# andrei-ace/EdgeStyle

Measured on AMD Instinct MI355X. Metric: 512x512 try-on images/sec @ 50 DDIM steps (6-cond ControlNet), higher is better.
Workload: dtype f16; 1 GPU; BASELINE configs[1]: full 6-cond edgestyle_multicontrolnet + controllora, 512x512, 50 DDIM steps, CFG 7.5, batch=1/GPU, hipGraph-captured step, cond embedding + VAE decode included; images_per_gpu=1, ddim_steps=50, parallelism=dp1 (independent images, one RCCL gather)

## Files before the change

### edgestyle_amd/csrc/builder.hip

```cpp
#include <hip/hip_runtime.h>
#include <math.h>
#include <stdio.h>
#include <stdlib.h>
#include <string.h>

#include <algorithm>
#include <deque>
#include <functional>
#include <map>
#include <memory>
#include <stdexcept>
#include <string>
#include <thread>
#include <unordered_map>
#include <vector>

#include "../../include/edgestyle_hip.h"
#include "plan.h"

extern "C" void es_set_error(const char* msg);
extern "C" int es_plan_set_dry(int on);

namespace {

[[noreturn]] void fail(const std::string& m) { throw std::runtime_error(m); }
inline int cdiv(long long a, long long b) { return (int)((a + b - 1) / b); }
inline int round_up(int a, int b) { return (a + b - 1) / b * b; }
constexpr int BK = 64, BM = 128;
constexpr unsigned long long FAKE_HEAP = 1ull << 44, FAKE_WS = 1ull << 45;

void parallel_for(long long n, const std::function<void(long long, long long)>& fn) {
  unsigned nt = std::thread::hardware_concurrency();
  nt = nt < 1 ? 1 : (nt > 16 ? 16 : nt);
  if (n < 64 || nt == 1) { fn(0, n); return; }
  std::vector<std::thread> th;
  const long long step = (n + nt - 1) / nt;
  for (long long a = 0; a < n; a += step) th.emplace_back(fn, a, std::min(n, a + step));
  for (auto& t : th) t.join();
}

inline uint16_t f32_to_f16(float f) { _Float16 h = (_Float16)f; uint16_t u; memcpy(&u, &h, 2); return u; }
inline float f16_to_f32(uint16_t u) { _Float16 h; memcpy(&h, &u, 2); return (float)h; }
inline uint16_t f32_to_bf16(float f) {
  uint32_t u; memcpy(&u, &f, 4);
  if ((u & 0x7FFFFFFFu) > 0x7F800000u) return (uint16_t)((u >> 16) | 0x40);
  return (uint16_t)((u + 0x7FFFu + ((u >> 16) & 1u)) >> 16);
}
inline float bf16_to_f32(uint16_t h) { uint32_t u = (uint32_t)h << 16; float f; memcpy(&f, &u, 4); return f; }

struct Dict {
  std::unordered_map<std::string, const es_tensor*> m;
  std::string name;
  void init(const es_state_dict& sd, const char* nm) {
    name = nm;
    if (sd.count < 0 || (sd.count > 0 && !sd.tensors)) fail(std::string("es_load_weights: the ") + nm + " state dict has a count but no tensors");
    for (int i = 0; i < sd.count; ++i) {
      const es_tensor& t = sd.tensors[i];
      if (!t.key || !t.data || t.ndim < 1 || t.ndim > 4 || t.dtype < 0 || t.dtype > ES_F32) fail("es_load_weights: malformed tensor descriptor #" + std::to_string(i) + " in the " + name + " state dict");
      long long n = 1;
      for (int d = 0; d < t.ndim; ++d) { if (t.shape[d] < 1 || t.shape[d] > (1ll << 31)) n = -1; else if (n > 0) n *= t.shape[d]; if (n > (1ll << 33)) n = -1; }
      if (n < 0) fail(std::string("es_load_weights: implausible shape of '") + t.key + "' in the " + name + " state dict");
      m[t.key] = &t;
    }
  }
  const es_tensor* find(const std::string& k) const { auto it = m.find(k); return it == m.end() ? nullptr : it->second; }
};
long long numel(const es_tensor* t) { long long n = 1; for (int i = 0; i < t->ndim; ++i) n *= t->shape[i]; return n; }
bool on_device(const void* p) {
  hipPointerAttribute_t a;
  const bool dev = hipPointerGetAttributes(&a, p) == hipSuccess && a.type == hipMemoryTypeDevice;
  (void)hipGetLastError();
  return dev;
}
std::vector<float> to_f32(const es_tensor* t) {
// ... 125 lines not shown
  ~Blk() { if (heap) heap->release(off, bytes); }
};

struct T {
  unsigned long long p = 0;
  int n = 0, h = 0, w = 0, c = 0;
  long long ld = 0;
  int es = 2;
  std::shared_ptr<Blk> b;
  unsigned long long lo = 0;
  std::shared_ptr<Blk> lo_b;
  unsigned long long gnp = 0;
  std::shared_ptr<Blk> gnp_b;
  int gnp_groups = 0;
  explicit operator bool() const { return p != 0; }
  long long hw() const { return (long long)h * w; }
  long long numel() const { return (long long)n * h * w * c; }
  bool contig() const { return ld == c; }
  long long bstride() const { return hw() * ld; }
  size_t bytes() const { return (size_t)numel() * es; }
  T batch(int a, int cnt = -1) const {
    T t = *this;
    t.p += (unsigned long long)a * (unsigned long long)bstride() * es;
    if (t.lo) t.lo += (unsigned long long)a * (unsigned long long)bstride() * es;
    t.gnp = 0; t.gnp_b.reset(); t.gnp_groups = 0;
    t.n = cnt < 0 ? n - a : cnt;
    if (a < 0 || t.n < 0 || a + t.n > n) fail("builder: batch slice out of range");
    return t;
  }
  T chan(int c0, int cn) const {
    T t = *this;
    if (c0 < 0 || c0 + cn > c) fail("builder: channel slice out of range");
    t.p += (unsigned long long)c0 * es;
    t.lo = 0; t.lo_b.reset();
    t.gnp = 0; t.gnp_b.reset(); t.gnp_groups = 0;
    t.c = cn;
    return t;
  }
  T view(int n2, int h2, int w2, int c2) const {
    if (!contig() || (long long)n2 * h2 * w2 * c2 != numel()) fail("builder: view of a non-contiguous or differently sized tensor");
    T t = *this;
    t.n = n2; t.h = h2; t.w = w2; t.c = c2; t.ld = c2;
    return t;
  }
  void* ptr() const { return (void*)p; }
};

struct PW {
  unsigned long long w = 0, bias = 0, ln_colsum = 0;
  int cout = 0, cin = 0, ksize = 1, bn = 128, rows_padded = 0, kpad = 0, ctail = 0, korder = 0;
  bool geglu = false;
  float ln_eps = 1e-5f;
  const uint16_t* host_w = nullptr;
  long long w_numel() const { return (long long)rows_padded * kpad; }
};
using PWs = std::vector<const PW*>;
struct Norm { unsigned long long g = 0, b = 0; };

struct CA {
  int stride = 1, pad = -1;
  bool upsample = false;
  T x2, temb, residual, out, out_scale_dev;
  long long temb_stride = 0;
  int act = ES_ACT_NONE;
  float out_scale = 1.f;
  int out_h = 0, out_w = 0;
  std::vector<int> group_n;
  std::vector<T> tails;
  int x_rep = 1;
  bool wide = false;
  int gn_groups = 0;
};

#pragma clang fp contract(off)
constexpr double PLAN_T160 = 1.25, PLAN_ALONE = 0.9, PLAN_TFIX = 2.0, PLAN_RED_FIX = 12.0, PLAN_SLAB_BYTES_PER_UNIT = 4.0e6;
constexpr double PLAN_T320 = 2.3, PLAN_T320_FIX = 3.0;
constexpr double PLAN_T256 = 2.6, PLAN_T256_FIX = 6.0, PLAN_T256_GEGLU = 7.0, PLAN_LN_TK = 1.55, PLAN_T256_MARGIN = 0.93;
constexpr int PLAN_BIG_MIN_M = 2048, PLAN_BIG_MIN_NK = 16;
constexpr double PLAN_T64_ALONE = 0.5, PLAN_T64 = 0.16, PLAN_T64_LONG = 1.5;
constexpr int PLAN_SMALL_MAX_M = 16384, PLAN_MIN_SLICE = 12, PLAN_NK_NOSPLIT = 10, PLAN_RESIDENT = 512;

double plan_env(const char* name, double dflt) { const char* e = getenv(name); return e && *e ? atof(e) : dflt; }
bool plan_gemm(long long M, int rows_padded, int kpad, bool geglu, const int* bns, int nb, bool allow_split, int* o_bn, int* o_sk, int* o_st) {
  static const double PLAN_T320 = plan_env("ES_PLAN_T320", ::PLAN_T320), PLAN_T256_MARGIN = plan_env("ES_PLAN_T256_MARGIN", ::PLAN_T256_MARGIN);
  static const int PLAN_BIG_MIN_NK = (int)plan_env("ES_PLAN_BIG_MIN_NK", ::PLAN_BIG_MIN_NK);
  int others[8], no = 0;
  bool has256 = false;
  for (int bi = 0; bi < nb; ++bi) { if (bns[bi] == 256) has256 = true; else if (no < 8) others[no++] = bns[bi]; }
  if (has256) {
    const int nk = kpad / BK;
    int obn = 0, osk = 1, ost = 2;
    const bool have_other = no > 0 && plan_gemm(M, rows_padded, kpad, geglu, others, no, allow_split, &obn, &osk, &ost);
    if (rows_padded % 256) { if (!have_other) return false; *o_bn = obn; *o_sk = osk; *o_st = ost; return true; }
    const long long t256 = ((M + 255) / 256) * (rows_padded / 256);
    const double c256 = (double)((t256 + 255) / 256) * ((double)nk * PLAN_T256 + PLAN_T256_FIX + (geglu ? PLAN_T256_GEGLU : 0.0));
    bool take = !have_other;
    if (have_other && M >= PLAN_BIG_MIN_M && nk >= PLAN_BIG_MIN_NK && osk == 1 && obn != 64) {
      const long long to = ((M + BM - 1) / BM) * (rows_padded / obn);
      const double co = (double)((to + PLAN_RESIDENT - 1) / PLAN_RESIDENT) * ((double)nk * PLAN_LN_TK * (obn == 160 ? PLAN_T160 : 1.0) + PLAN_T256_FIX);
      take = c256 < PLAN_T256_MARGIN * co;
    }
    if (take) { *o_bn = 256; *o_sk = 1; *o_st = 2; } else { *o_bn = obn; *o_sk = osk; *o_st = ost; }
    return true;
  }
  if (geglu) { *o_bn = 128; *o_sk = 1; *o_st = 2; return true; }
  const int nk = kpad / BK;
// ... 16 lines not shown
      else if (bn == 64) {
        if (sk > 1 && wgs > PLAN_RESIDENT) continue;
        const double w = (double)wgs / (double)(PLAN_RESIDENT / 2);
        const double ex = std::max(0.0, w - 1.0);
        tk = (PLAN_T64_ALONE + PLAN_T64 * (ex * ex)) * (nk <= 40 ? 1.0 : PLAN_T64_LONG);
      } else tk = (bn == 160 ? PLAN_T160 : 1.0) * (wgs <= PLAN_RESIDENT / 2 ? PLAN_ALONE : 1.0);
      const double rounds = bn == 320 ? std::max((double)wgs / 256.0, 0.9) : (double)((wgs + resident - 1) / resident);
      double t = rounds * (((double)nk / (double)sk) * tk + (bn == 320 ? PLAN_T320_FIX : PLAN_TFIX));
      if (sk > 1) t += PLAN_RED_FIX + (double)sk * (double)M * (double)rows_padded * 8.0 / PLAN_SLAB_BYTES_PER_UNIT;
      if (!have || t < bt) { have = true; bt = t; bbn = bn; bsk = sk; bwgs = wgs; }
    }
  }
  if (!have) return false;
  *o_bn = bbn; *o_sk = bsk;
  if (bbn == 64) *o_st = (bwgs <= PLAN_RESIDENT && nk / bsk >= 6) ? 4 : 2;
  else *o_st = (bbn != 320 && bwgs <= PLAN_RESIDENT / 2 && nk / bsk >= 6) ? 4 : 2;
  return true;
}

constexpr int XS_TARGET_WGS = 256, XS_MIN_M = 8192;
bool xs_shape_fits(int ksize, int kpad, int cin, int ctail, int cout, bool geglu) {
  if (ksize != 1 || (kpad != 320 && kpad != 640) || cin != kpad || ctail) return false;
  const int ch = kpad == 320 ? 64 : 32;
  const int line = ch * (128 / (geglu ? ch : 2 * ch));
  return !(cout % line || cout < 4 * line);
}
bool xs_shape_ok(long long M, int ksize, int kpad, int cin, int ctail, int cout, bool geglu, long long min_m) {
  if (!xs_shape_fits(ksize, kpad, cin, ctail, cout, geglu)) return false;
  if (min_m && (M < min_m || (M < 4 * min_m && cout < (kpad == 320 ? 960 : 1920)))) return false;
  return true;
}
int choose_bn(int cout) { return (cout % 160 == 0 && cout % 128 != 0) ? 160 : 128; }

bool wide_stream(int dtype, const es_launch_knobs& k) { return k.wide_stream == 1 || (k.wide_stream < 0 && dtype == ES_BF16); }
bool gn_handover(long long hw, int c, int groups, const es_launch_knobs& k) {
  if (!k.gn_handover || groups < 1 || c % 8 || hw % 64 || c % groups || c / groups > 64) return false;
  return k.gn_handover == 2 || !es_group_norm_is_slab((int)hw, c, groups);
}
bool groups_tile_256(const es_launch_query& q) {
  for (int g = 0; g < std::min(q.n_counts, 4); ++g) if ((q.group_n[g] * q.hw) % 256) return false;
  return true;
}
bool launch_takes_xs(const es_launch_query& q, const es_launch_knobs& k) {
  const bool xs_res = !q.has_residual || (k.xs_residual && q.kpad == 320 && !q.geglu && !q.has_ln && q.residual_dense && !(q.wide && wide_stream(q.dtype, k)));
  if (!(q.ksize == 1 && q.stride == 1 && !q.upsample && !q.C2 && !q.has_temb && xs_res && !q.n_tails && q.x_rep == 1 && q.act == ES_ACT_NONE &&
        q.unit_scale && !q.force_splitk && !k.force_bn && k.xs_enabled)) return false;
  if (q.ngroups > 1 && (q.ngroups > 4 || !groups_tile_256(q) || !q.groups_agree)) return false;
  return xs_shape_ok(q.M, q.ksize, q.kpad, q.cin, q.ctail, q.cout, q.geglu != 0, k.xs_min_m);
}
bool launch_choose(const es_launch_query& q, const es_launch_knobs& k, es_launch_choice* o) {
  memset(o, 0, sizeof(*o));
  if (launch_takes_xs(q, k)) { o->route = ES_ROUTE_LINEAR_XS; return true; }
  const bool aligned = q.C1 % BK == 0 && q.C2 % BK == 0;
  const bool big_ok = k.big_tile && aligned && !q.geglu && !q.has_ln && groups_tile_256(q);
  const bool small_ok = k.small_tile && aligned && !q.geglu && k.force_waves != 8;
  const bool ln256_ok = k.big_tile_256 && (q.geglu || q.has_ln) && q.ksize == 1 && q.stride == 1 && !q.upsample && !q.C2 && !q.n_tails && !q.has_temb &&
                        q.x_rep == 1 && q.C1 % BK == 0 && q.rows_padded % 256 == 0 && q.cout % 8 == 0 && !(q.geglu && q.has_residual) && !q.wide &&
                        q.gn_groups == 0 && k.force_waves != 8 && groups_tile_256(q);
  int cand[5], nc = 0;
  if (ln256_ok) cand[nc++] = 256;
  if (big_ok) cand[nc++] = 320;
  cand[nc++] = 160; cand[nc++] = 128;
  if (small_ok) cand[nc++] = 64;
  if (k.force_bn) { cand[0] = k.force_bn; nc = 1; }
  const bool geglu = q.geglu != 0, allow_split = !q.has_ln;
  int bn, splitk, stages;
  if (!plan_gemm(q.M, q.rows_padded, q.kpad, geglu, cand, nc, allow_split, &bn, &splitk, &stages)) return false;
  if (bn == 320 && !k.force_bn && (q.force_splitk ? q.force_splitk : splitk) == 1 &&
      !es_conv_gemm8p_form_ok(geglu ? ES_ACT_GEGLU : q.act, q.cout, q.has_temb, q.hw, q.has_residual)) {
    const int at = (int)(std::find(cand, cand + nc, 320) - cand);
    std::copy(cand + at + 1, cand + nc, cand + at);
    if (!plan_gemm(q.M, q.rows_padded, q.kpad, geglu, cand, nc - 1, allow_split, &bn, &splitk, &stages)) return false;
  }
  if (stages == 4 && !k.deep_ring) stages = 2;
  if (q.force_splitk) { splitk = q.force_splitk; stages = q.stages; }
  else if (q.stages) stages = q.stages;
  if (!stages) stages = k.force_stages;
  o->bn = bn; o->splitk = splitk; o->stages = stages;
  if (k.force_waves) o->waves = k.force_waves;
  else if (k.eight_waves && q.ksize == 1 && q.M <= 65536 && aligned && bn != 64 && bn != 320 && bn != 256 && !(stages == 4 && bn != 128) && stages != 3) o->waves = 8;
  o->xcd_m_fastest = k.xcd_order < 0 ? (q.ngroups <= 1 && splitk == 1 && q.M <= 2048 && q.w_numel > q.src_numel) : k.xcd_order;
  const int cstore = geglu ? q.cout / 2 : q.cout;
  o->gn_partials = q.gn_groups > 0 && gn_handover(q.hw, cstore, q.gn_groups, k) && !geglu && !q.has_ln && q.cout / q.gn_groups <= (bn == 320 ? 160 : bn);
  o->wide = q.wide && q.has_residual && wide_stream(q.dtype, k) && cstore % 8 == 0 && !geglu;
  return true;
}
bool launch_gn_fold(const es_launch_query& q, int groups, const es_launch_knobs& k) {
  if (!(k.gn_fold && k.xs_enabled) || k.gn_handover || q.hw % 256 || groups < 1 || groups > 32) return false;
  if (q.geglu || q.has_ln || q.kpad % groups || !xs_shape_fits(q.ksize, q.kpad, q.cin, q.ctail, q.cout, false)) return false;
  if (q.M < (q.kpad == 320 ? 8192 : 32768)) return false;
  return !(q.ngroups > 1 && (q.ngroups > 4 || !groups_tile_256(q) || !q.groups_agree));
}
struct BuildEnv { es_launch_knobs knobs; bool chunk_major; };
BuildEnv read_build_env() {
  auto env = [](const char* name, const char* dflt) { const char* e = getenv(name); return std::string(e ? e : dflt); };
  const std::string ho = env("ES_GN_HANDOVER", "0"), ws = env("ES_WIDE_STREAM", "auto");
  BuildEnv b;
  b.chunk_major = env("ES_CHUNK_MAJOR", "0") == "1";
  es_launch_knobs& k = b.knobs;
  memset(&k, 0, sizeof(k));
  k.xs_enabled = k.big_tile = k.small_tile = k.eight_waves = k.deep_ring = 1; k.xs_min_m = XS_MIN_M; k.xcd_order = -1;
  k.xs_residual = env("ES_XS_RESIDUAL", "1") == "1"; k.big_tile_256 = env("ES_BIG_TILE_256", "1")[0] != '0'; k.gn_fold = env("ES_GN_FOLD", "1") == "1";
  k.gn_handover = ho == "all" ? 2 : ho == "1"; k.wide_stream = ws == "auto" ? -1 : ws == "1";
  return b;
}

struct Builder {
  Heap heap;
  unsigned long long ws_bytes = 0;
  int dt = ES_F16;
  const BuildEnv env = read_build_env();
  std::vector<std::pair<unsigned long long, std::vector<char>>> uploads;
  std::deque<PW> pws;
  std::map<std::string, const PW*> pack_cache;
  std::map<const void*, unsigned long long> vec_cache;
  std::map<std::pair<int, int>, unsigned long long> gn_partials, fusion_scratch;
  std::map<int, unsigned long long> zero_bias;

  T empty(int n, int h, int w, int c, int es = 2) {
    T t; t.n = n; t.h = h; t.w = w; t.c = c; t.ld = c; t.es = es;
    auto blk = std::make_shared<Blk>();
    blk->heap = &heap; blk->bytes = std::max<size_t>(t.bytes(), 1); blk->off = heap.alloc(blk->bytes);
    t.b = blk; t.p = FAKE_HEAP + blk->off;
    return t;
  }
  unsigned long long persistent(size_t bytes) { return FAKE_HEAP + heap.alloc(std::max<size_t>(bytes, 1)); }
  T persistent_t(int n, int h, int w, int c, int es = 2) {
    T t; t.n = n; t.h = h; t.w = w; t.c = c; t.ld = c; t.es = es;
    t.p = persistent(t.bytes());
    return t;
  }
  char* staged(unsigned long long addr, size_t bytes) {
    uploads.emplace_back(addr, std::vector<char>(bytes, 0));
    return uploads.back().second.data();
  }
  unsigned long long upload_f32(const std::vector<float>& v) {
    const unsigned long long a = persistent(v.size() * 4);
    memcpy(staged(a, v.size() * 4), v.data(), v.size() * 4);
    return a;
  }
  unsigned long long workspace(unsigned long long bytes) { ws_bytes = std::max(ws_bytes, bytes); return FAKE_WS; }
  void add_into(const T& a, const T& b, const T& out) {
    if (!a.contig() || !b.contig() || !out.contig() || a.numel() != b.numel() || a.numel() != out.numel()) fail("builder: add of non-contiguous or differently sized tensors");
    ok(es_add(a.ptr(), b.ptr(), out.ptr(), a.numel(), dt, nullptr), "es_add");
  }
  T add(const T& a, const T& b) {
    if (!a.contig() || !b.contig() || a.numel() != b.numel()) fail("builder: add of non-contiguous or differently sized tensors");
    T out = empty(a.n, a.h, a.w, a.c);
    ok(es_add(a.ptr(), b.ptr(), out.ptr(), a.numel(), dt, nullptr), "es_add");
    return out;
  }
  uint16_t enc(float f) const { return dt == ES_F16 ? f32_to_f16(f) : f32_to_bf16(f); }
  float dec(uint16_t u) const { return dt == ES_F16 ? f16_to_f32(u) : bf16_to_f32(u); }

  const PW* pack(const std::vector<float>& w, int cout, int cin, int k, const std::vector<float>* bias, bool geglu = false, int cin_pad = 0, int cout_pad = 0,
                 const std::vector<float>* tail = nullptr, int ctail = 0) {
    if ((long long)w.size() != (long long)cout * cin * k * k) fail("builder: weight size does not match its shape");
    const int cp = cin_pad ? cin_pad : round_up(cin, 8);
    if (cp < cin || cp % 8 || (cout_pad && cout_pad < cout)) fail("builder: channel padding smaller than the tensor");
    const int ktrue = k * k * cp + ctail;
    const int cout_eff = cout_pad ? cout_pad : cout;
    const int bn = geglu ? 128 : choose_bn(cout_eff);
    const int rows = round_up(cout_eff, bn);
    const int kpad = round_up(ktrue, BK);
    const int inner = cout / 2;
    if (geglu && inner % 16) fail("builder: GEGLU inner width must be a multiple of 16");
    pws.emplace_back();
    PW& p = pws.back();
    p.cout = cout_eff; p.cin = cp; p.ksize = k; p.bn = bn; p.rows_padded = rows; p.kpad = kpad; p.geglu = geglu; p.ctail = ctail;
    const bool chunk_major = env.chunk_major && k == 3 && cp % BK == 0;
    p.korder = chunk_major ? 1 : 0;
    p.w = persistent((size_t)rows * kpad * 2);
    uint16_t* dst = (uint16_t*)staged(p.w, (size_t)rows * kpad * 2);
    p.host_w = dst;
    auto src_row = [&](int r) { if (!geglu) return r; const int blk = r / 32, within = r % 32; return within < 16 ? blk * 16 + within : inner + blk * 16 + (within - 16); };
    parallel_for(cout, [&](long long a, long long b) {
      for (long long r = a; r < b; ++r) {
        const float* s = w.data() + (size_t)src_row((int)r) * cin * k * k;
        uint16_t* d = dst + (size_t)r * kpad;
        for (int t = 0; t < k * k; ++t)
          for (int ci = 0; ci < cin; ++ci)
            d[chunk_major ? ((ci / BK) * k * k + t) * BK + ci % BK : t * cp + ci] = enc(s[(size_t)ci * k * k + t]);
        if (tail) for (int j = 0; j < ctail; ++j) d[k * k * cp + j] = enc((*tail)[(size_t)r * ctail + j]);
      }
    });
    if (bias) {
      if ((int)bias->size() != cout) fail("builder: bias size does not match the weight");
      p.bias = persistent((size_t)rows * 4);
      float* bd = (float*)staged(p.bias, (size_t)rows * 4);
      for (int r = 0; r < cout; ++r) bd[r] = (*bias)[src_row(r)];
    }
    return &p;
  }
  const PW* pack_ln(const std::vector<float>& w, int rows, int C, const std::vector<float>* bias, const std::vector<float>& gamma, const std::vector<float>& beta,
                    float eps, bool geglu) {
    std::vector<float> wg((size_t)rows * C), fb((size_t)rows);
    parallel_for(rows, [&](long long a, long long b) {
      for (long long r = a; r < b; ++r) {
        double acc = 0.0;
        for (int j = 0; j < C; ++j) { wg[r * C + j] = w[r * C + j] * gamma[j]; acc += (double)w[r * C + j] * (double)beta[j]; }
        if (bias) acc += (double)(*bias)[r];
        fb[r] = (float)acc;
      }
    });
    PW* p = const_cast<PW*>(pack(wg, rows, C, 1, &fb, geglu));
    const uint16_t* pk = p->host_w;
    std::vector<float> cs((size_t)p->rows_padded);
    for (int r = 0; r < p->rows_padded; ++r) {
      double acc = 0.0;
      for (int j = 0; j < p->kpad; ++j) acc += (double)dec(pk[(size_t)r * p->kpad + j]);
      cs[r] = (float)acc;
    }
    p->ln_colsum = upload_f32(cs);
    p->ln_eps = eps;
    return p;
  }
  unsigned long long norm_vec(const Weights& W, const std::string& key, long long n) {
    const es_tensor* id = nullptr;
    std::vector<float> v = W.vec(key, n, &id);
    auto it = vec_cache.find(id->data);
    if (it != vec_cache.end()) return it->second;
    return vec_cache[id->data] = upload_f32(v);
  }
  Norm norm(const Weights& W, const std::string& p, long long n) { return {norm_vec(W, p + ".weight", n), norm_vec(W, p + ".bias", n)}; }

  const PW* conv(const Weights& W, const std::string& p, int cin_pad = 0, bool geglu = false, int cout_pad = 0) {
    const es_tensor* wt = W.get(p + ".weight");
    if (wt->ndim != 2 && wt->ndim != 4) fail("es_load_weights: '" + p + ".weight' is neither a Linear nor a Conv2d weight");
    const int cout = (int)wt->shape[0], cin = (int)wt->shape[1], k = wt->ndim == 4 ? (int)wt->shape[2] : 1;
    if (wt->ndim == 4 && (wt->shape[3] != k || (k != 1 && k != 3))) fail("es_load_weights: '" + p + ".weight': only 1x1 and 3x3 kernels");
    const es_tensor* bt = W.find(p + ".bias");
    std::string key;
    if (!W.lora(p)) {
      char buf[128];
      snprintf(buf, sizeof(buf), "%p|%p|%d|%d|%d", wt->data, bt ? bt->data : nullptr, (int)geglu, cin_pad, cout_pad);
      key = buf;
      auto it = pack_cache.find(key);
      if (it != pack_cache.end()) return it->second;
    }
    std::vector<float> w = W.matrix(p), b;
    if (bt) b = W.vec(p + ".bias", cout);
    const PW* pw = pack(w, cout, cin, k, bt ? &b : nullptr, geglu, cin_pad, cout_pad);
    if (!key.empty()) pack_cache[key] = pw;
    return pw;
  }
  void stack(const Weights& W, const std::vector<std::string>& ps, bool bias, std::vector<float>& w, std::vector<float>& b, int& rows, int& cols) {
    rows = 0; cols = -1;
    for (const auto& p : ps) {
      const es_tensor* t = W.get(p + ".weight");
      if (t->ndim != 2 || (cols >= 0 && t->shape[1] != cols)) fail("es_load_weights: '" + p + ".weight' does not stack with its neighbours");
      cols = (int)t->shape[1];
      std::vector<float> m = W.matrix(p);
      w.insert(w.end(), m.begin(), m.end());
      if (bias) { std::vector<float> v = W.vec(p + ".bias", t->shape[0]); b.insert(b.end(), v.begin(), v.end()); }
      rows += (int)t->shape[0];
    }
  }
  const PW* cat(const Weights& W, const std::vector<std::string>& ps, bool bias) {
    std::vector<float> w, b; int rows, cols;
    stack(W, ps, bias, w, b, rows, cols);
    return pack(w, rows, cols, 1, bias ? &b : nullptr);
  }
  const PW* cat_ln(const Weights& W, const std::vector<std::string>& ps, bool bias, const std::string& ln, bool geglu = false) {
    std::vector<float> w, b; int rows, cols;
    stack(W, ps, bias, w, b, rows, cols);
    return pack_ln(w, rows, cols, bias ? &b : nullptr, W.vec(ln + ".weight", cols), W.vec(ln + ".bias", cols), 1e-5f, geglu);
  }
  const PW* conv_tail(const Weights& W, const std::string& p, const std::string& pt) {
    const es_tensor* wt = W.get(p + ".weight");
    const es_tensor* tt = W.get(pt + ".weight");
    char buf[96];
    snprintf(buf, sizeof(buf), "%p|%p|tail", wt->data, tt->data);
    auto it = pack_cache.find(buf);
    if (it != pack_cache.end()) return it->second;
    const int cout = (int)wt->shape[0], cin = (int)wt->shape[1], k = (int)wt->shape[2], ct = (int)tt->shape[1];
    if (wt->ndim != 4 || cin % BK || ct % BK || tt->shape[0] != cout) fail("es_load_weights: conv2 + conv_shortcut fold needs 64-aligned channels ('" + p + "')");
    std::vector<float> w = W.matrix(p), tw = W.matrix(pt), b = W.vec(p + ".bias", cout), b2 = W.vec(pt + ".bias", cout);
    for (int i = 0; i < cout; ++i) b[i] = b[i] + b2[i];
    const PW* pw = pack(w, cout, cin, k, &b, false, 0, 0, &tw, ct);
    pack_cache[buf] = pw;
    return pw;
  }

  static void ok(int rc, const char* what) { if (rc) fail(std::string(what) + ": " + es_last_error()); }

  struct GnFront { unsigned long long part = 0; std::vector<Norm> nl; int groups = 0, nchunk = 0, hw = 0; float eps = 0.f; };
  T linear_xs(const T& x, const PWs& pl, long long M, const T& out, const std::vector<long long>& group_rows, const T& residual = T(),
              const GnFront* gn = nullptr) {
    const PW* pw = pl[0];
    const int K = pw->kpad, ch = K == 320 ? 64 : 32;
    const int pline = 128 / (pw->geglu ? ch : 2 * ch);
    const int total = pw->cout / ch, lines = total / pline;
    const long long rbs = (M + 255) / 256;
    const int want = (int)std::max<long long>(1, std::min<long long>(lines, XS_TARGET_WGS / rbs));
    const int lps = cdiv(lines, want), nslices = cdiv(lines, lps);
    es_xs_desc d;
    memset(&d, 0, sizeof(d));
    auto bias_of = [&](const PW* q) -> unsigned long long {
      if (q->bias) return q->bias;
      auto it = zero_bias.find(q->rows_padded);
      if (it != zero_bias.end()) return it->second;
      return zero_bias[q->rows_padded] = persistent((size_t)q->rows_padded * 4);
    };
    d.x = x.ptr(); d.out = out.ptr(); d.w = (const void*)pw->w; d.bias = (const float*)bias_of(pw);
    d.M = (int)M; d.K = K; d.Cout = pw->cout; d.rows_padded = pw->rows_padded; d.ldo = out.c;
    d.geglu = pw->geglu; d.ln = pw->ln_colsum != 0; d.ln_eps = pw->ln_eps;
    d.nslices = nslices; d.chunks_per_slice = lps * pline; d.dtype = dt;
    if (residual) d.residual = residual.ptr();
    if (gn) {
      d.gn_part = (const float*)gn->part; d.gn_groups = gn->groups; d.gn_nchunk = gn->nchunk; d.gn_hw = gn->hw; d.gn_eps = gn->eps;
      if (pl.size() > 1) {
        if (gn->nl.size() != pl.size()) fail("grouped linear_xs: one GroupNorm parameter set per weight group");
        for (size_t g = 0; g < pl.size(); ++g) { d.gn_gamma_g[g] = (const float*)gn->nl[g].g; d.gn_beta_g[g] = (const float*)gn->nl[g].b; }
      } else { d.gn_gamma = (const float*)gn->nl[0].g; d.gn_beta = (const float*)gn->nl[0].b; }
    }
    if (pl.size() > 1) {
      d.ngroups = (int)pl.size();
      long long acc = 0;
      for (size_t g = 0; g < pl.size(); ++g) {
        const PW* q = pl[g];
        if (q->rows_padded != pw->rows_padded || q->kpad != pw->kpad || q->cout != pw->cout || q->geglu != pw->geglu) fail("grouped linear_xs: weight geometry differs between groups");
        acc += group_rows[g] / 128;
        d.mt_end[g] = (int)acc; d.w_g[g] = (const void*)q->w; d.bias_g[g] = (const float*)bias_of(q);
      }
    }
    ok(es_linear_xs(&d, nullptr), "es_linear_xs");
    return out;
  }

  es_launch_query launch_query(const PWs& pl, long long M, long long hw, const CA& a, int C1, int C2, long long src_numel, bool residual_dense) const {
    const PW* pw = pl[0];
    es_launch_query q;
    memset(&q, 0, sizeof(q));
    q.M = M; q.hw = hw; q.w_numel = pw->w_numel(); q.src_numel = src_numel; q.ksize = pw->ksize; q.stride = a.stride; q.upsample = a.upsample; q.C1 = C1; q.C2 = C2;
    q.rows_padded = pw->rows_padded; q.kpad = pw->kpad; q.cin = pw->cin; q.ctail = pw->ctail; q.cout = pw->cout; q.geglu = pw->geglu; q.has_ln = pw->ln_colsum != 0;
    q.act = a.act; q.has_temb = (bool)a.temb; q.has_residual = (bool)a.residual; q.residual_dense = residual_dense; q.unit_scale = a.out_scale == 1.f && !a.out_scale_dev;
    q.n_tails = (int)a.tails.size(); q.x_rep = a.x_rep; q.wide = a.wide; q.dtype = dt; q.gn_groups = a.gn_groups;
    if (pl.size() > 1) {
      q.ngroups = (int)pl.size(); q.n_counts = (int)a.group_n.size(); q.groups_agree = 1;
      for (size_t g = 0; g < std::min<size_t>(a.group_n.size(), 4); ++g) q.group_n[g] = a.group_n[g];
      for (const PW* p : pl) if ((p->ln_colsum == 0) != (pw->ln_colsum == 0)) q.groups_agree = 0;
    }
    return q;
  }

  T conv_gemm(const T& x, const PWs& pl, const CA& a = CA()) {
    const PW* pw = pl[0];
    const bool grouped = pl.size() > 1;
    int N = x.n;
    const int H = x.h, Wd = x.w, C1 = x.c, nsrc = x.n;
    if (!x.contig()) fail("conv_gemm: the source must be contiguous");
    if (a.x_rep > 1) { if (a.x2 || !a.tails.empty()) fail("conv_gemm: x_rep needs a single source"); N *= a.x_rep; }
    const int C2 = a.x2 ? a.x2.c : 0;
    if (C1 + C2 != pw->cin) fail("conv_gemm: input channels " + std::to_string(C1) + "+" + std::to_string(C2) + " != packed " + std::to_string(pw->cin));
    int tsum = 0;
    for (const auto& t : a.tails) tsum += t.c;
    if (tsum != pw->ctail || a.tails.size() > 2) fail("conv_gemm: tail channels do not match the packed weights");
    const int k = pw->ksize, pad = a.pad < 0 ? (k == 3 ? 1 : 0) : a.pad;
    const int Hin = a.upsample ? H * 2 : H, Win = a.upsample ? Wd * 2 : Wd;
    const int Hout = a.out_h ? a.out_h : (Hin + 2 * pad - k) / a.stride + 1, Wout = a.out_w ? a.out_w : (Win + 2 * pad - k) / a.stride + 1;
    const int act_i = pw->geglu ? ES_ACT_GEGLU : a.act;
    const int cstore = pw->geglu ? pw->cout / 2 : pw->cout;
    T out = a.out ? a.out : empty(N, Hout, Wout, cstore);
    if (out.numel() != (long long)N * Hout * Wout * cstore || !out.contig()) fail("conv_gemm: output buffer of another size");
    const long long M = (long long)N * Hout * Wout, hw = (long long)Hout * Wout;
    const es_launch_query q = launch_query(pl, M, hw, a, C1, C2, x.numel() * a.x_rep + (a.x2 ? a.x2.numel() : 0),
                                           a.residual && a.residual.contig() && a.residual.numel() == M * cstore);
    es_launch_choice ch;
    if (!launch_choose(q, env.knobs, &ch)) fail("plan_gemm: rows_padded fits no N tile");
    if (ch.route == ES_ROUTE_LINEAR_XS) {
      std::vector<long long> rows;
      for (int n : a.group_n) rows.push_back(n * hw);
      T xo = out;
      linear_xs(x, grouped ? pl : PWs{pw}, M, xo, rows, a.residual);
      return out;
    }
    const int bn = ch.bn, splitk = ch.splitk;
    es_gemm_desc d;
    memset(&d, 0, sizeof(d));
    d.x = x.ptr(); d.x2 = a.x2 ? a.x2.ptr() : nullptr; d.w = (const void*)pw->w; d.bias = (const float*)pw->bias;
    d.temb = a.temb ? a.temb.ptr() : nullptr; d.residual = a.residual ? a.residual.ptr() : nullptr;
    d.out_scale_dev = a.out_scale_dev ? (const float*)a.out_scale_dev.ptr() : nullptr; d.out = out.ptr();
    d.N = N; d.Hsrc = H; d.Wsrc = Wd; d.C1 = C1; d.C2 = C2; d.Hout = Hout; d.Wout = Wout; d.Cout = pw->cout;
    d.rows_padded = pw->rows_padded; d.Kpad = pw->kpad; d.ksize = k; d.stride = a.stride; d.pad = pad; d.upsample = a.upsample;
    d.temb_stride = a.temb ? (int)a.temb_stride : 0;
    d.act = act_i; d.splitk = splitk; d.bn = bn; d.dtype = dt; d.out_scale = a.out_scale; d.stages = ch.stages;
    d.waves = ch.waves; d.xcd_m_fastest = ch.xcd_m_fastest;
    d.x_nmod = a.x_rep > 1 ? nsrc : 0;
    d.korder = pw->korder;
    if (ch.gn_partials) {
      T part = empty(N, (int)(2 * (hw / 64)), 1, a.gn_groups * 2, 4);
      d.gn_part = (float*)part.ptr(); d.gn_groups = a.gn_groups;
      out.gnp = part.p; out.gnp_b = part.b; out.gnp_groups = a.gn_groups;
    }
    if (ch.wide) {
      if (a.residual.lo) d.residual_lo = (const void*)a.residual.lo;
      T lo = empty(N, Hout, Wout, cstore);
      d.out_lo = lo.ptr();
      out.lo = lo.p; out.lo_b = lo.b;
    }
    if (splitk > 1) d.workspace = (float*)workspace((unsigned long long)splitk * M * pw->rows_padded * 4);
    if (pw->ln_colsum) {
      for (const PW* q : pl) if (!q->ln_colsum) fail("LayerNorm-folded weights need a plain linear launch (all groups folded)");
      if (a.x2 || k != 1) fail("LayerNorm-folded weights need a plain linear launch");
      d.ln_colsum = (const float*)pw->ln_colsum; d.ln_eps = pw->ln_eps;
    }
    if (!a.tails.empty()) {
      for (const auto& t : a.tails) if (t.n != N || t.h != Hout || t.w != Wout || !t.contig()) fail("conv_gemm: tail sources must be contiguous [N,Hout,Wout,C]");
      d.t1 = a.tails[0].ptr(); d.Ct1 = a.tails[0].c;
      if (a.tails.size() == 2) { d.t2 = a.tails[1].ptr(); d.Ct2 = a.tails[1].c; }
    }
    if (grouped) {
      const int gran = bn == 320 ? 256 : BM;
      int sum = 0;
      for (int n : a.group_n) { sum += n; if ((n * hw) % gran) fail("grouped conv_gemm: groups must cover N in whole tiles"); }
      if (pl.size() > 4 || a.group_n.size() != pl.size() || sum != N) fail("grouped conv_gemm: bad group table");
      d.ngroups = (int)pl.size();
      long long acc = 0;
      for (size_t g = 0; g < pl.size(); ++g) {
        const PW* q = pl[g];
// ... 215 lines not shown
    conv_in = B.conv(W, "conv_in", in_pad);
    t1 = B.conv(W, "time_embedding.linear_1"); t2 = B.conv(W, "time_embedding.linear_2");
    std::vector<std::string> names;
    for (int i = 0; i < c.nb; ++i) for (int j = 0; j < c.lpb; ++j) names.push_back("down_blocks." + std::to_string(i) + ".resnets." + std::to_string(j));
    names.push_back("mid_block.resnets.0"); names.push_back("mid_block.resnets.1");
    names.insert(names.end(), extra_resnets.begin(), extra_resnets.end());
    int o = 0;
    std::vector<std::string> tp;
    for (const auto& nm : names) { temb_offs[nm] = o; o += (int)W.shaped(nm + ".time_emb_proj.weight", {-1, 4 * c.ch[0]})->shape[0]; tp.push_back(nm + ".time_emb_proj"); }
    tproj = B.cat(W, tp, true);
    for (int i = 0; i < c.nb; ++i) {
      down.emplace_back();
      for (int j = 0; j < c.lpb; ++j) {
        const std::string r = "down_blocks." + std::to_string(i) + ".resnets." + std::to_string(j);
        int ti = -1;
        Resnet rs(B, W, r, c.groups, c.eps, temb_offs[r]);
        if (c.has_attn[i]) { tr.emplace_back(B, W, "down_blocks." + std::to_string(i) + ".attentions." + std::to_string(j), c.heads, c.groups); ti = (int)tr.size() - 1; }
        down.back().emplace_back(rs, ti);
      }
      downsample.push_back(i != c.nb - 1 ? B.conv(W, "down_blocks." + std::to_string(i) + ".downsamplers.0.conv") : nullptr);
    }
    mid0 = Resnet(B, W, "mid_block.resnets.0", c.groups, c.eps, temb_offs["mid_block.resnets.0"]);
    tr.emplace_back(B, W, "mid_block.attentions.0", c.heads, c.groups); mid_attn = (int)tr.size() - 1;
    mid1 = Resnet(B, W, "mid_block.resnets.1", c.groups, c.eps, temb_offs["mid_block.resnets.1"]);
    n_enc_tr = (int)tr.size();
  }
  int tproj_width() const { return tproj->cout; }
  T time_proj(Builder& B, const T& t, int n) const {
    T e = B.timestep_embedding(t, n, cfg.ch[0]);
    CA s; s.act = ES_ACT_SILU;
    e = B.linear(e, t1, s);
    e = B.linear(e, t2, s);
    return B.linear(e, tproj);
  }
};

struct UNet : Encoder {
  std::vector<std::vector<std::pair<Resnet, int>>> up;
  std::vector<const PW*> upsample;
  Norm norm_out; const PW* conv_out;
  void init(Builder& B, const Weights& W, const UCfg& c) {
    std::vector<std::string> extra;
    for (int i = 0; i < c.nb; ++i) for (int j = 0; j < c.lpb + 1; ++j) extra.push_back("up_blocks." + std::to_string(i) + ".resnets." + std::to_string(j));
    Encoder::init(B, W, c, extra);
    for (int i = 0; i < c.nb; ++i) {
      up.emplace_back();
      for (int j = 0; j < c.lpb + 1; ++j) {
        const std::string r = "up_blocks." + std::to_string(i) + ".resnets." + std::to_string(j);
        int ti = -1;
        Resnet rs(B, W, r, c.groups, c.eps, temb_offs[r]);
        if (c.has_attn[c.nb - 1 - i]) { tr.emplace_back(B, W, "up_blocks." + std::to_string(i) + ".attentions." + std::to_string(j), c.heads, c.groups); ti = (int)tr.size() - 1; }
        up.back().emplace_back(rs, ti);
      }
      upsample.push_back(i != c.nb - 1 ? B.conv(W, "up_blocks." + std::to_string(i) + ".upsamplers.0.conv") : nullptr);
    }
    W.shaped("conv_out.weight", {c.out_ch, c.ch[0], 3, 3});
    norm_out = B.norm(W, "conv_norm_out", c.ch[0]);
    conv_out = B.conv(W, "conv_out");
  }
};

struct ControlNet : Encoder {
  std::vector<const PW*> zero; const PW* zero_mid = nullptr;
  std::vector<const PW*> cond;
  bool uses_vae = false;
  void init(Builder& B, const Weights& W, const UCfg& c, bool uses_vae_) {
    Encoder::init(B, W, c, {});
    uses_vae = uses_vae_;
    std::vector<int> rc{c.ch[0]};
    for (int i = 0; i < c.nb; ++i) { for (int j = 0; j < c.lpb; ++j) rc.push_back(c.ch[i]); if (i != c.nb - 1) rc.push_back(c.ch[i]); }
    for (size_t i = 0; i < rc.size(); ++i) {
      W.shaped("controlnet_down_blocks." + std::to_string(i) + ".weight", {rc[i], rc[i], 1, 1});
      zero.push_back(B.conv(W, "controlnet_down_blocks." + std::to_string(i)));
    }
    W.shaped("controlnet_mid_block.weight", {c.ch[c.nb - 1], c.ch[c.nb - 1], 1, 1});
    zero_mid = B.conv(W, "controlnet_mid_block");
    if (!uses_vae) {
      const std::string p = "controlnet_cond_embedding";
      W.shaped(p + ".conv_in.weight", {c.ce[0], c.cond_ch, 3, 3});
      W.shaped(p + ".conv_out.weight", {c.ch[0], c.ce[c.nce - 1], 3, 3});
      cond.push_back(B.conv(W, p + ".conv_in", 8));
      for (int i = 0; i < 2 * (c.nce - 1); ++i) cond.push_back(B.conv(W, p + ".blocks." + std::to_string(i)));
      cond.push_back(B.conv(W, p + ".conv_out"));
    }
  }
  T embed_cond(Builder& B, const T& img) const {
    CA s; s.act = ES_ACT_SILU;
    T h = B.conv_gemm(img, cond[0], s);
    for (size_t i = 1; i + 1 < cond.size(); ++i) { CA a; a.act = ES_ACT_SILU; a.stride = ((i - 1) % 2 == 1) ? 2 : 1; h = B.conv_gemm(h, cond[i], a); }
    return B.conv_gemm(h, cond.back());
  }
};

struct FusionParams { unsigned long long w1, b1, g1, be1, w2, b2, g2, be2, w3, b3; int c, s; };

struct VAE {
  VCfg cfg; int lat_pad = 8;
  struct Mid { Resnet r0, r1; Norm gn; const PW *qkv, *o; };
  const PW *e_in, *e_out, *quant, *post_quant_scaled, *d_in, *d_out;
  std::vector<std::pair<std::vector<Resnet>, const PW*>> e_down, d_up;
  Mid e_mid, d_mid; Norm e_norm, d_norm;
  Mid mid(Builder& B, const Weights& W, const std::string& side) {
    const std::string a = side + ".mid_block.attentions.0";
    const int c = cfg.ch[cfg.nb - 1];
    Mid m;
    m.r0 = Resnet(B, W, side + ".mid_block.resnets.0", cfg.groups, cfg.eps, -1);
    m.gn = B.norm(W, a + ".group_norm", c);
    m.qkv = B.cat(W, {a + ".to_q", a + ".to_k", a + ".to_v"}, true);
    m.o = B.conv(W, a + ".to_out.0");
    m.r1 = Resnet(B, W, side + ".mid_block.resnets.1", cfg.groups, cfg.eps, -1);
    return m;
  }
  void init(Builder& B, const Weights& W, const VCfg& c) {
    cfg = c;
    lat_pad = round_up(c.latent, 8);
    const int n = c.nb;
    W.shaped("encoder.conv_in.weight", {c.ch[0], 3, 3, 3}); W.shaped("encoder.conv_out.weight", {2 * c.latent, c.ch[n - 1], 3, 3});
    W.shaped("quant_conv.weight", {2 * c.latent, 2 * c.latent, 1, 1}); W.shaped("post_quant_conv.weight", {c.latent, c.latent, 1, 1});
    W.shaped("decoder.conv_in.weight", {c.ch[n - 1], c.latent, 3, 3}); W.shaped("decoder.conv_out.weight", {3, c.ch[0], 3, 3});
    for (const char* side : {"encoder", "decoder"})
      for (const char* q : {".to_q", ".to_k", ".to_v", ".to_out.0"}) W.shaped(std::string(side) + ".mid_block.attentions.0" + q + ".weight", {c.ch[n - 1], c.ch[n - 1]});
    e_in = B.conv(W, "encoder.conv_in", 8);
    for (int i = 0; i < n; ++i) {
      std::vector<Resnet> rs;
      for (int j = 0; j < c.lpb; ++j) rs.emplace_back(B, W, "encoder.down_blocks." + std::to_string(i) + ".resnets." + std::to_string(j), c.groups, c.eps, -1);
      e_down.emplace_back(rs, i != n - 1 ? B.conv(W, "encoder.down_blocks." + std::to_string(i) + ".downsamplers.0.conv") : nullptr);
    }
    e_mid = mid(B, W, "encoder");
    e_norm = B.norm(W, "encoder.conv_norm_out", c.ch[n - 1]);
    e_out = B.conv(W, "encoder.conv_out");
    quant = B.conv(W, "quant_conv");
    {
      const es_tensor* wt = W.get("post_quant_conv.weight");
      std::vector<float> w = W.matrix("post_quant_conv"), b;
      for (auto& v : w) v = (float)((double)v / (double)c.scaling);
      const bool hb = W.has("post_quant_conv.bias");
      if (hb) b = W.vec("post_quant_conv.bias", wt->shape[0]);
      post_quant_scaled = B.pack(w, (int)wt->shape[0], (int)wt->shape[1], 1, hb ? &b : nullptr, false, lat_pad, 8);
    }
    d_in = B.conv(W, "decoder.conv_in", 8);
    d_mid = mid(B, W, "decoder");
    for (int i = 0; i < n; ++i) {
      std::vector<Resnet> rs;
      for (int j = 0; j < c.lpb + 1; ++j) rs.emplace_back(B, W, "decoder.up_blocks." + std::to_string(i) + ".resnets." + std::to_string(j), c.groups, c.eps, -1);
      d_up.emplace_back(rs, i != n - 1 ? B.conv(W, "decoder.up_blocks." + std::to_string(i) + ".upsamplers.0.conv") : nullptr);
    }
    d_norm = B.norm(W, "decoder.conv_norm_out", c.ch[0]);
    d_out = B.conv(W, "decoder.conv_out");
  }
  T run_mid(Builder& B, const Mid& m, T h) const {
    h = m.r0.run(B, h, T());
    const int N = h.n, H = h.h, Wd = h.w, C = h.c;
    T n = B.group_norm(h, m.gn, cfg.groups, cfg.eps, false).view(N, H * Wd, 1, C);
    T qkv = B.linear(n, m.qkv);
    T a = B.attention(qkv.chan(0, C), qkv.chan(C, C), qkv.chan(2 * C, C), 1);
    CA r; r.residual = h.view(N, H * Wd, 1, C);
    h = B.linear(a, m.o, r).view(N, H, Wd, C);
    return m.r1.run(B, h, T());
  }
  T encode_moments(Builder& B, const T& img) const {
    T h = B.conv_gemm(img, e_in);
    for (const auto& blk : e_down) {
      for (const auto& r : blk.first) h = r.run(B, h, T());
      if (blk.second) { CA a; a.stride = 2; a.pad = 0; a.out_h = h.h / 2; a.out_w = h.w / 2; h = B.conv_gemm(h, blk.second, a); }
    }
    h = run_mid(B, e_mid, h);
    h = B.group_norm(h, e_norm, cfg.groups, cfg.eps, true);
    h = B.conv_gemm(h, e_out);
    return B.conv_gemm(h, quant);
  }
  T decode(Builder& B, const T& z) const {
    T h = B.conv_gemm(z, post_quant_scaled);
    h = B.conv_gemm(h, d_in);
    h = run_mid(B, d_mid, h);
    for (const auto& blk : d_up) {
      for (const auto& r : blk.first) h = r.run(B, h, T());
      if (blk.second) { CA a; a.upsample = true; h = B.conv_gemm(h, blk.second, a); }
    }
    h = B.group_norm(h, d_norm, cfg.groups, cfg.eps, true);
    return B.conv_gemm(h, d_out);
  }
};

struct Model {
  Builder B;
  UCfg ucfg; VCfg vcfg;
  es_ctx_geometry geo;
  Dict d_unet, d_vae, d_fusion, d_cn[6];
  UNet unet;
  VAE vae;
  std::vector<std::unique_ptr<ControlNet>> nets;
  std::vector<int> net_of_cond;
  std::vector<std::pair<int, std::vector<int>>> groups;
  std::vector<FusionParams> fusion;
  std::vector<std::pair<int, int>> table;
  std::vector<const Encoder*> encs; std::vector<int> counts; int ntot = 0, width = 0, ncn = 0;
  int B_ = 1, N = 2, T_ = 50, h = 64, w = 64, nn = 6, kmax = 3;
  T latents, model_in, noise, ehs, step_idx, t_rows, scales_cur, t_table, scale_table, coef, ts_dev, image;
// ... 340 lines not shown
  void pack_fusion(const Weights& W) {
    for (size_t i = 0; i < table.size(); ++i) {
      const std::string p = i + 1 < table.size() ? "multi_controlnet_down_blocks." + std::to_string(i) : "multi_controlnet_mid_block";
      const int c = table[i].first, s = table[i].second, hw = s * s;
      FusionParams f; f.c = c; f.s = s;
      f.w1 = B.upload_f32(to_f32(W.shaped(p + ".first_conv.weight", {3 * c, 2, 1, 1})));
      f.b1 = B.upload_f32(to_f32(W.shaped(p + ".first_conv.bias", {3 * c})));
      f.w2 = B.upload_f32(to_f32(W.shaped(p + ".second_conv.weight", {c, 3, 1, 1})));
      f.b2 = B.upload_f32(to_f32(W.shaped(p + ".second_conv.bias", {c})));
      f.w3 = B.upload_f32(to_f32(W.shaped(p + ".third_conv.weight", {c, 1, 1, 1})));
      f.b3 = B.upload_f32(to_f32(W.shaped(p + ".third_conv.bias", {c})));
      auto plane = [&](const std::string& key, int per) {
        const std::vector<float> t = to_f32(W.shaped(key, {(long long)per * c, s, s}));
        const unsigned long long a = B.persistent((size_t)hw * c * per * 2);
        uint16_t* d = (uint16_t*)B.staged(a, (size_t)hw * c * per * 2);
        parallel_for(hw, [&](long long x0, long long x1) {
          for (long long px = x0; px < x1; ++px)
            for (int cc = 0; cc < c * per; ++cc) d[(size_t)px * c * per + cc] = B.enc(t[(size_t)cc * hw + px]);
        });
        return a;
      };
      f.g1 = plane(p + ".first_normalization.weight", 3); f.be1 = plane(p + ".first_normalization.bias", 3);
      f.g2 = plane(p + ".second_normalization.weight", 1); f.be2 = plane(p + ".second_normalization.bias", 1);
      fusion.push_back(f);
    }
  }
};

struct Recording {
  es_plan* p;
  explicit Recording(es_plan* pl) : p(pl) { if (es_plan_begin_record(p)) fail(std::string("es_load_weights: ") + es_last_error()); es_plan_set_dry(1); }
  ~Recording() { es_plan_set_dry(0); es_plan_end_record(p); }
};

}

extern "C" int es_plan_gemm_choice(long long M, int rows_padded, int kpad, int geglu, const int* bns, int n_bns, int allow_split, int* bn, int* splitk, int* stages) {
  if (!bns || n_bns < 1 || !bn || !splitk || !stages) { es_set_error("es_plan_gemm_choice: null argument"); return -1; }
  if (!plan_gemm(M, rows_padded, kpad, geglu != 0, bns, n_bns, allow_split != 0, bn, splitk, stages)) { es_set_error("es_plan_gemm_choice: rows_padded fits no N tile"); return -1; }
  return 0;
}
extern "C" int es_linear_xs_eligible(long long M, int ksize, int kpad, int cin, int ctail, int cout, int geglu) {
  return xs_shape_ok(M, ksize, kpad, cin, ctail, cout, geglu != 0, XS_MIN_M) ? 1 : 0;
}
extern "C" int es_launch_choose(const es_launch_query* q, const es_launch_knobs* k, es_launch_choice* out) {
  if (!q || !k || !out) { es_set_error("es_launch_choose: null argument"); return -1; }
  if (!launch_choose(*q, *k, out)) { es_set_error("es_launch_choose: rows_padded fits no N tile"); return -1; }
  return 0;
}
extern "C" int es_launch_route(const es_launch_query* q, const es_launch_knobs* k) { return q && k && launch_takes_xs(*q, *k) ? ES_ROUTE_LINEAR_XS : ES_ROUTE_CONV_GEMM; }
extern "C" int es_launch_gn_fold(const es_launch_query* q, int groups, const es_launch_knobs* k) { return q && k && launch_gn_fold(*q, groups, *k); }
extern "C" int es_launch_gn_handover(long long hw, int c, int groups, const es_launch_knobs* k) { return k && gn_handover(hw, c, groups, *k); }
extern "C" int es_launch_wide_stream(int dtype, const es_launch_knobs* k) { return k && wide_stream(dtype, *k); }

extern "C" int es_load_weights(const es_weights* wts, const es_model_config* mc, const es_ctx_geometry* g, int device, es_ctx** out) {
  if (!wts || !mc || !g || !out) { es_set_error("es_load_weights: null argument"); return -1; }
  es_ctx* ctx = nullptr;
  es_plan* plans[ES_PLAN_COUNT] = {};
  void* arena = nullptr;
  try {
    auto m = std::make_unique<Model>();
    Model& M = *m;
    Builder& B = M.B;
    if (mc->n_blocks < 2 || mc->n_blocks > 4 || mc->vae_n_blocks < 2 || mc->vae_n_blocks > 4) fail("es_load_weights: 2..4 resolution levels");
    if (g->n_conds != 6 && g->n_conds != 1) fail("es_load_weights: n_conds is 6 (the reference's fused multi-ControlNet model, MC:66-114) or 1 (a single ControlNet, PL:338-351)");
    if (g->n_conds == 1 && wts->n_controlnets != 1) fail("es_load_weights: a single-ControlNet context takes exactly one ControlNet");
    if (g->dtype != ES_F16 && g->dtype != ES_BF16) fail("es_load_weights: dtype must be ES_F16 or ES_BF16");
    if (g->B < 1 || g->h < 1 || g->w < 1 || g->n_steps < 1) fail("es_load_weights: bad geometry");
    if (wts->n_controlnets < 1 || wts->n_controlnets > 6) fail("es_load_weights: 1..6 distinct ControlNets");
    UCfg& u = M.ucfg;
    u.in_ch = mc->in_channels; u.out_ch = mc->out_channels; u.nb = mc->n_blocks; u.lpb = mc->layers_per_block; u.heads = mc->num_heads;
    u.cross = mc->cross_attention_dim; u.groups = mc->norm_num_groups; u.eps = mc->norm_eps; u.nce = mc->n_cond_embed; u.cond_ch = mc->conditioning_channels;
    for (int i = 0; i < 4; ++i) { u.ch[i] = mc->block_out_channels[i]; u.has_attn[i] = mc->down_has_attn[i]; u.ce[i] = mc->cond_embed_channels[i]; }
    VCfg& v = M.vcfg;
    v.nb = mc->vae_n_blocks; v.lpb = mc->vae_layers_per_block; v.latent = mc->vae_latent_channels; v.groups = mc->vae_norm_num_groups;
    v.eps = mc->vae_norm_eps; v.scaling = mc->vae_scaling_factor;
    for (int i = 0; i < 4; ++i) v.ch[i] = mc->vae_block_out_channels[i];
    if (u.in_ch != v.latent) fail("es_load_weights: the UNet's in_channels must equal the VAE's latent_channels");
    if (u.cond_ch != 3 || u.nce < 2 || u.nce > 4) fail("es_load_weights: conditioning embedding of 3 input channels, 2..4 widths");
    M.geo = *g;
    B.dt = g->dtype;
    M.B_ = g->B; M.N = g->cfg ? 2 * g->B : g->B; M.T_ = g->n_steps; M.h = g->h; M.w = g->w; M.nn = g->n_conds;
    M.guess = g->guess_mode != 0;
    M.Bc = M.guess ? g->B : M.N;
    const int N = M.N, TS = M.T_, h = g->h, w = g->w, Bn = g->B, NN = g->n_conds, Nc = M.Bc;
    if (!M.guess) {
      int cnt[6] = {};
      for (int p = 0; p < NN; ++p) {
        const int ni = wts->net_of_cond[p];
        if (ni < 0 || ni >= wts->n_controlnets) fail("es_load_weights: net_of_cond names a ControlNet that was not given");
        ++cnt[ni];
      }
      const int hw_min = (h >> (u.nb - 1)) * (w >> (u.nb - 1));
      for (int i = 0; i <= wts->n_controlnets; ++i) {
        const long long n = (i < wts->n_controlnets ? (long long)cnt[i] : 1) * N;
        if (n && (n * hw_min) % BM) fail("es_load_weights: the groups of the lockstep pass do not tile in 128-pixel units at this latent size (the Python host falls back to serial chains; this builder does not)");
      }
    }
    M.d_unet.init(wts->unet, "UNet"); M.d_vae.init(wts->vae, "VAE"); M.d_fusion.init(wts->fusion, "fusion");
    for (int i = 0; i < wts->n_controlnets; ++i) M.d_cn[i].init(wts->controlnet[i], ("ControlNet " + std::to_string(i)).c_str());
    Weights Wu; Wu.own = &M.d_unet; Wu.who = "UNet";
    Weights Wv; Wv.own = &M.d_vae; Wv.who = "VAE";
    Weights Wf; Wf.own = &M.d_fusion; Wf.who = "fusion";
    M.unet.init(B, Wu, u);
    M.vae.init(B, Wv, v);
    for (int i = 0; i < wts->n_controlnets; ++i) {
// ... 198 lines not shown
```

### edgestyle_amd/csrc/gemm_conv.hip

```cpp
#ifndef ES_WT_STORES
#define ES_WT_STORES 1
#endif
#include "common.h"
#include "../../include/edgestyle_hip.h"
#include "plan.h"

#ifndef ES_W_AUX
#define ES_W_AUX 0
#endif

int es_conv_gemm8p_launch(const es_gemm_desc& d, hipStream_t st);
bool es_conv_gemm8p_takes(const es_gemm_desc& d);

unsigned long long es_operand_limit_v = 0x7FFFFFFFull;

namespace {

constexpr int BK = 64;

#ifndef ES_ABLATE
#define ES_ABLATE 0
#endif
#ifndef ES_STAMPS
#define ES_STAMPS 0
#endif

typedef __attribute__((address_space(3))) void* lptr_t;

template <typename T>
ES_DEVICE void store_elems(T* o, const float* v, int n) {
  for (int r = 0; r < n; ++r) o[r] = from_f32<T>(v[r]);
}

template <int XI>
ES_DEVICE void row_offsets_fn(unsigned (&voff)[XI], const int (&iy0)[XI], const int (&ix0)[XI], const int (&nb)[XI],
                              const int tp, const int cs, const int chan, const int ksize, const int KK, const int pad,
                              const int Hin, const int Win, const int upsample, const int Wsrc) {
  int ky = 0, kx = 0;
  if (ksize == 3) { ky = (tp * 11) >> 5; kx = tp - ky * 3; }
  if (tp >= KK) { ky = pad; kx = pad; }
#pragma unroll
  for (int i = 0; i < XI; ++i) {
    const int iy = iy0[i] + ky, ix = ix0[i] + kx;
    const bool ok = (unsigned)iy < (unsigned)Hin && (unsigned)ix < (unsigned)Win;
    const int pix = nb[i] + (iy >> upsample) * Wsrc + (ix >> upsample);
    voff[i] = ok ? (unsigned)(((size_t)pix * cs + chan) * 2) : 0xFFFFFF00u;
  }
}

template <typename T, int BM, int BN, bool ALIGNED, int STAGES, int FM = 4 ,
          bool LN = false ,
          bool KO = false >
__global__ __launch_bounds__(BM * 8 / FM, (STAGES == 2 && BM == 128) ? (FM == 2 ? 4 : 2) : 1) void conv_gemm_kernel(
    const es_gemm_desc p, const int M, const int nk, const void* const tail1, const void* const tail2, const int tailC1,
    const int tailC2) {
  constexpr int BKT = BK;
  constexpr int RB = BKT * 2;
  constexpr int CPR = BKT / 8;
  constexpr int RPP = 1024 / RB;
  constexpr int WM = BM / (16 * FM);
  constexpr int NW = WM * 2;
  constexpr int NT = NW * 64;
  constexpr int XI = (BM / RPP) / NW;
  constexpr int FN = BN / 32;
  constexpr int WP = BN / RPP;
  constexpr int WI = (WP + NW - 1) / NW;
  constexpr int XT = BM * RB;
  constexpr int WT = BN * RB;
  static_assert((size_t)BM * (BN * 2 + 16) <= (size_t)STAGES * (BM + BN) * RB, "the epilogue tile must fit the stage ring");
  static_assert(LN || (size_t)BM * (BN * 2 + 16) + (size_t)(BM / 8 + BM / 64) * BN * 8 <= (size_t)STAGES * (BM + BN) * RB,
                "the GroupNorm-statistics scratch (gn_emit_partials) must fit behind the epilogue tile");
  constexpr int BNP = BN;
  constexpr int EROW = BNP * 2 + 16;
  constexpr int NI = XI + WI;
  extern __shared__ __attribute__((aligned(16))) char smem[];

  const int tid = threadIdx.x;
  const int lane = tid & 63;
  const int wave = __builtin_amdgcn_readfirstlane(tid >> 6);
  const int wm = wave % WM, wn = wave / WM;
  int tile_m, tile_n, z;
  {
    const int tm = (M + BM - 1) / BM, tn = p.rows_padded / BN;
    const int nwg = gridDim.x, b = blockIdx.x;
    const int q = nwg >> 3, r = nwg & 7, xcd = b & 7;
    const int w = (xcd < r ? xcd * (q + 1) : r * (q + 1) + (xcd - r) * q) + (b >> 3);
    const float inv_tm = __builtin_amdgcn_rcpf((float)tm), inv_tn = __builtin_amdgcn_rcpf((float)tn);
    if (p.xcd_m_fastest) { const int t = fast_div(w, tm, inv_tm); tile_m = w - t * tm; z = fast_div(t, tn, inv_tn); tile_n = t - z * tn; }
    else                 { const int t = fast_div(w, tn, inv_tn); tile_n = w - t * tn; z = fast_div(t, tm, inv_tm); tile_m = t - z * tm; }
  }
#if ES_STAMPS
  const int sblk = blockIdx.x == 40 ? 0 : (blockIdx.x == 333 ? 1 : -1);
  auto stamp = [&](int ks, int what) __attribute__((always_inline)) {
    if (p.prof && sblk >= 0 && lane == 0 && wave < 4 && ks >= 8 && ks < 16)
      p.prof[((sblk * 4 + wave) * 8 + (ks - 8)) * 4 + what] = __builtin_amdgcn_s_memtime();
  };
  auto pstamp = [&](int what) __attribute__((always_inline)) {
    if (p.prof && tid == 0 && (blockIdx.x == 0 || blockIdx.x == gridDim.x - 1))
      p.prof[256 + (blockIdx.x == 0 ? 0 : 1) * 8 + what] = __builtin_amdgcn_s_memtime();
  };
  pstamp(0);
#else
  if (p.prof && tid == 0) atomicMin(p.prof, (unsigned long long)__builtin_amdgcn_s_memrealtime());
#endif

  int ks0 = 0, ks1 = nk;
  if (p.splitk > 1) {
    const float inv_sk = __builtin_amdgcn_rcpf((float)p.splitk);
    ks0 = fast_div(nk * z, p.splitk, inv_sk);
    ks1 = fast_div(nk * (z + 1), p.splitk, inv_sk);
  }

  const int lrow = lane / CPR;
  const int lslot = lane % CPR;
  const int kc = lslot ^ (lrow & 7);
  const int Ctot = p.C1 + p.C2;
  const int KK = p.ksize * p.ksize;
  const int pC1 = p.C1, pC2 = p.C2, pCt1 = tailC1, pCt2 = tailC2;
  const bool has_tail = tail1 != nullptr;
  const int Ctail = has_tail ? pCt1 + pCt2 : 0;
  const int Ktrue = KK * Ctot + Ctail;
  const int Hin = p.Hsrc << p.upsample, Win = p.Wsrc << p.upsample;
  const int HWout = p.Hout * p.Wout;

  constexpr unsigned OOB = 0xFFFFFF00u;
  int iy0[XI], ix0[XI], nb[XI];
  const bool small_m = M < (1 << 24);
  const float inv_hw = __builtin_amdgcn_rcpf((float)HWout), inv_w = __builtin_amdgcn_rcpf((float)p.Wout);
#pragma unroll
  for (int i = 0; i < XI; ++i) {
    const int m = tile_m * BM + RPP * (wave * XI + i) + lrow;
    iy0[i] = -(1 << 20); ix0[i] = -(1 << 20); nb[i] = 0;
    if (m < M) {
      int n, oy, ox;
      if (HWout == 1) {
        n = m; oy = 0; ox = 0;
      } else if (small_m) {
        n = fast_div(m, HWout, inv_hw);
        const int rem = m - n * HWout;
        oy = fast_div(rem, p.Wout, inv_w);
        ox = rem - oy * p.Wout;
      } else {
        n = m / HWout;
        const int rem = m - n * HWout;
        oy = rem / p.Wout; ox = rem - oy * p.Wout;
      }
      iy0[i] = oy * p.stride - p.pad;
      ix0[i] = ox * p.stride - p.pad;
      if (p.x_nmod) n -= (n / p.x_nmod) * p.x_nmod;
      nb[i] = n * p.Hsrc * p.Wsrc;
    }
  }
  int pix0[KO ? XI : 1];
  unsigned tmask[KO ? XI : 1];
  if constexpr (KO) {
#pragma unroll
    for (int i = 0; i < XI; ++i) {
      const int ay = iy0[i], ax = ix0[i];
      unsigned vy = 0, vx = 0;
#pragma unroll
      for (int k = 0; k < 3; ++k) {
        vy |= ((unsigned)(ay + k) < (unsigned)Hin ? 1u : 0u) << k;
        vx |= ((unsigned)(ax + k) < (unsigned)Win ? 1u : 0u) << k;
      }
      unsigned mk = ((vy & 1) ? vx : 0u) | ((vy & 2) ? vx << 3 : 0u) | ((vy & 4) ? vx << 6 : 0u);
      mk |= ay > -(1 << 19) ? 1u << 9 : 0u;
      mk |= (unsigned)(ay & p.upsample) << 10 | (unsigned)(ax & p.upsample) << 11;
      tmask[i] = mk;
      pix0[i] = nb[i] + (ay >> p.upsample) * p.Wsrc + (ax >> p.upsample);
    }
  }
  int grp = 0;
  if (p.ngroups > 1) {
    const int t128 = (tile_m * BM) / 128;
    grp = (t128 >= p.mt_end[0]) + (t128 >= p.mt_end[1]) + (t128 >= p.mt_end[2]);
  }
  const void* wsel = p.ngroups > 1 ? p.w_g[grp] : p.w;
  const float* bsel = p.ngroups > 1 ? p.bias_g[grp] : p.bias;
  const float* lnsel = LN ? (p.ngroups > 1 ? p.ln_colsum_g[grp] : p.ln_colsum) : nullptr;
  const auto rW = __builtin_amdgcn_make_buffer_rsrc(
      (void*)wsel, (short)0, (int)((size_t)p.rows_padded * p.Kpad * 2), 0x00020000);
  const int Nsrc = p.x_nmod ? p.x_nmod : p.N;
  const auto rX1 = __builtin_amdgcn_make_buffer_rsrc(
      (void*)p.x, (short)0, (int)((size_t)Nsrc * p.Hsrc * p.Wsrc * p.C1 * 2), 0x00020000);
  const void* const pt1 = tail1 ? tail1 : p.x;
  const void* const pt2 = tail2 ? tail2 : p.x;
  const void* const px = p.x;
  const void* const px2 = p.x2 ? p.x2 : p.x;
  const int nX1 = (int)((size_t)Nsrc * p.Hsrc * p.Wsrc * pC1 * 2);
  const int nX2 = (int)((size_t)Nsrc * p.Hsrc * p.Wsrc * (p.x2 ? pC2 : pC1) * 2);
  const int nT1 = has_tail ? (int)((size_t)p.N * p.Hout * p.Wout * pCt1 * 2) : 0;
  const int nT2 = tail2 ? (int)((size_t)p.N * p.Hout * p.Wout * pCt2 * 2) : 0;
  unsigned woff[WI];
#pragma unroll
  for (int i = 0; i < WI; ++i) {
    const int piece = wave * WI + i;
    woff[i] = piece < WP ? (unsigned)(((size_t)(tile_n * BN + RPP * piece + lrow) * p.Kpad + kc * 8) * 2) : OOB;
  }

  int tap, cpos;
  {
    const int kg = ks0 * BKT + (ALIGNED ? 0 : kc * 8);
    tap = kg == 0 ? 0 : fast_div(kg, Ctot, __builtin_amdgcn_rcpf((float)Ctot));
    cpos = kg - tap * Ctot;
    if (ALIGNED && tap >= KK) { tap = KK; cpos = kg - KK * Ctot; }
    if constexpr (KO) {
      const int kt = (KK * Ctot) / BKT;
      if (ks0 >= kt) { tap = KK; cpos = (ks0 - kt) * BKT; }
      else { const int ch = fast_div(ks0, 9, 1.0f / 9.0f); tap = ks0 - ch * 9; cpos = ch * BKT; }
    }
  }
  unsigned voff[XI];
#pragma unroll
  for (int i = 0; i < XI; ++i) voff[i] = OOB;
  const void* xbase = p.x;
  int xrec = 0, soff_x = 0, seg_left = 0;
  const int ks_tail = (KK * Ctot) / BKT;
  const int pk_ksize = p.ksize, pk_pad = p.pad, pk_up = p.upsample, pk_wsrc = p.Wsrc;
#define row_offsets(tp, cs, chan) \
  row_offsets_fn<XI>(voff, iy0, ix0, nb, (tp), (cs), (chan), pk_ksize, KK, pk_pad, Hin, Win, pk_up, pk_wsrc)
  auto issue_tile = [&](int ks, int stage) __attribute__((always_inline)) {
    char* xs = smem + stage * (XT + WT);
    char* ws = xs + XT;
    const int soff_w = ks * RB;
#pragma unroll
    for (int i = 0; i < WI; ++i)
      if (!(ES_ABLATE & 32) && wave * WI + i < WP)
        __builtin_amdgcn_raw_ptr_buffer_load_lds(rW, (lptr_t)(ws + (wave * WI + i) * 1024), 16,
                                                 (ES_ABLATE & 64) ? (int)OOB : (int)woff[i], soff_w, 0, ES_W_AUX);
    if constexpr ((ES_ABLATE & 16) != 0) {
    } else if constexpr (ALIGNED) {
      bool fast = false;
      if constexpr (!KO) fast = seg_left > 0;
      if (fast) {
        soff_x += 128; --seg_left;
      } else {
      const bool tail = KO ? ks >= ks_tail : tap >= KK;
      int q0 = pC1, q1 = pC2, q2 = pCt1, q3 = pCt2;
      asm("" : "+s"(q0), "+s"(q1), "+s"(q2), "+s"(q3));
      const int c1 = tail ? q2 : q0;
      const int second = cpos >= c1 ? 1 : 0;
      const int cs = second ? (tail ? q3 : q1) : c1;
      const int cc = second ? cpos - c1 : cpos;
      if constexpr (KO) {
        int ky = (tap * 11) >> 5, kx = tap - ky * 3;
        if (tail) { ky = pk_pad; kx = pk_pad; }
        const unsigned tb = 1u << tap, cs2 = (unsigned)cs * 2u;
        const int dsc = ky * pk_wsrc + kx;
#pragma unroll
        for (int i = 0; i < XI; ++i) {
          int pix = pix0[i] + dsc;
          if (pk_up) pix = pix0[i] + ((int)(((tmask[i] >> 10) & 1) + ky) >> 1) * pk_wsrc + ((int)(((tmask[i] >> 11) & 1) + kx) >> 1);
          voff[i] = (tmask[i] & tb) ? __umul24((unsigned)pix, cs2) + (unsigned)(kc * 16) : 0xFFFFFF00u;
        }
      } else {
        row_offsets(tap, cs, kc * 8);
      }
#if ES_ABLATE & 64
#pragma unroll
      for (int i = 0; i < XI; ++i) voff[i] = OOB;
#endif
      const void *b0 = px, *b1 = px2, *b2 = pt1, *b3 = pt2;
      int n0 = nX1, n1 = nX2, n2 = nT1, n3 = nT2;
      asm("" : "+s"(b0), "+s"(b1), "+s"(b2), "+s"(b3), "+s"(n0), "+s"(n1), "+s"(n2), "+s"(n3));
      xbase = tail ? (second ? b3 : b2) : (second ? b1 : b0);
      xrec = tail ? (second ? n3 : n2) : (second ? n1 : n0);
      soff_x = cc * 2;
      if constexpr (KO) {
        if (tap < KK) {
          if (++tap == KK) { cpos += BKT; if (cpos >= Ctot) cpos = 0; else tap = 0; }
        } else {
          cpos += BKT;
        }
// ... 122 lines not shown
      wa1[i] = as_vec8<T>(*(const u32x4*)(ws + row * 128 + (((4 + fq) ^ (row & 7)) << 4)));
    }
    }
#ifndef ES_LN_NOGRAM
#define ES_LN_NOGRAM 0
#endif
    if constexpr (LN && !ES_LN_NOGRAM) {
#pragma unroll
      for (int jj = 0; jj < LNH; ++jj) {
        const auto f0 = wn ? xa0[LNH + jj] : xa0[jj];
        const auto f1 = wn ? xa1[LNH + jj] : xa1[jj];
        ln_gram[jj] = mfma16(f0, f0, ln_gram[jj]);
        ln_gram[jj] = mfma16(f1, f1, ln_gram[jj]);
        ln_sum[jj] = mfma16(ln_ones, f0, ln_sum[jj]);
        ln_sum[jj] = mfma16(ln_ones, f1, ln_sum[jj]);
      }
    }
    do_mfmas();
#if ES_STAMPS
    stamp(ks - ks0, 3);
#endif
    istage = istage + 1 == STAGES ? 0 : istage + 1;
    stage = stage + 1 == STAGES ? 0 : stage + 1;
  }

#if ES_STAMPS
  pstamp(3);
#endif
  const int prow = wm * (16 * FM) + frow;
  const int pcol = wn * (BN / 2) + fq * 4;
  if (p.splitk > 1) {
    float* wsp = p.workspace + (size_t)z * M * p.rows_padded;
#pragma unroll
    for (int j = 0; j < FM; ++j) {
      const int m = tile_m * BM + prow + j * 16;
      if (m < M) {
#pragma unroll
        for (int i = 0; i < FN; ++i)
          store16(wsp + (size_t)m * p.rows_padded + tile_n * BN + pcol + i * 16, __builtin_bit_cast(u32x4, acc[i][j]));
      }
    }
#if !ES_STAMPS
    if (p.prof && tid == 0) atomicMax(p.prof + 1, (unsigned long long)__builtin_amdgcn_s_memrealtime());
#endif
    return;
  }

  const bool geglu = p.act == ES_ACT_GEGLU;
  const int Cstore = geglu ? p.Cout / 2 : p.Cout;
  float scale = p.out_scale;
  if (p.out_scale_dev) scale *= *p.out_scale_dev;
  char* et = smem;
  T* outp = (T*)p.out;
  const T* resp = (const T*)p.residual;
  constexpr int RPF = (BM * (BN / 8) + NT - 1) / NT;
  u32x4 rpre[RPF];
  const bool vec_store = (Cstore & 7) == 0;
  {
    if (resp && vec_store) {
      const int CH = (geglu ? BN / 2 : BN) / 8;
      const float inv_ch = __builtin_amdgcn_rcpf((float)CH);
      const int c_tile = tile_n * (geglu ? BN / 2 : BN);
#pragma unroll
      for (int k = 0; k < RPF; ++k) {
        const int idx = tid + k * NT;
        const int row = fast_div(idx, CH, inv_ch), ch = idx - row * CH;
        const int m = tile_m * BM + row, c = c_tile + ch * 8;
        rpre[k] = u32x4{0u, 0u, 0u, 0u};
        if (idx < BM * CH && m < M && c < Cstore) rpre[k] = *(const u32x4*)(resp + (size_t)m * Cstore + c);
      }
    }
  }
  float* rowstat = (float*)(smem + (size_t)STAGES * (XT + WT) - BM * 8);
  {
    __syncthreads();
    if constexpr (LN) {
#pragma unroll
      for (int i = 0; i < FN; ++i) lncs[i] = *(const f32x4*)(lnsel + tile_n * BN + wn * (BN / 2) + fq * 4 + i * 16);
#pragma unroll
      for (int jj = 0; jj < LNH; ++jj) {
        const float dq = fq == (frow >> 2) ? ln_gram[jj][frow & 3] : 0.f;
        const float q_ = xor32_sum(xor16_sum(dq));
        if (fq == 0) {
          const int row = wm * (16 * FM) + ((wn ? LNH : 0) + jj) * 16 + frow;
          const float inv_c = 1.0f / (float)p.C1;
          const float mean = ln_sum[jj][0] * inv_c;
          float var = q_ * inv_c - mean * mean;
          var = var < 0.f ? 0.f : var;
          rowstat[row * 2] = mean;
          rowstat[row * 2 + 1] = rsqrtf(var + p.ln_eps);
        }
      }
      __syncthreads();
    }
    const bool tuni = !LN && p.temb && (HWout % BM) == 0;
    if (!geglu && p.act == ES_ACT_NONE && (!p.temb || tuni)) {
      f32x4 tvv[LN ? 1 : FN];
#pragma unroll
      for (int i = 0; i < (LN ? 1 : FN); ++i) tvv[i] = f32x4{0.f, 0.f, 0.f, 0.f};
      if (tuni) {
        const int m0 = tile_m * BM < M ? tile_m * BM : M - 1;
        const T* trow = (const T*)p.temb + (size_t)(m0 / HWout) * p.temb_stride;
#pragma unroll
        for (int i = 0; i < (LN ? 0 : FN); ++i) {
          const int c = tile_n * BN + pcol + i * 16;
          if (c + 3 < p.Cout) {
// ... 42 lines not shown
                  ag = ln_rstd * (ag - ln_mean * lncs[i + 1][r]);
                }
                const float hv = ah + bias[i][r], gv = ag + bias[i + 1][r];
                pk[r] = from_f32<T>(hv * gelu_f(gv) * scale);
              }
              *(typename Traits<T>::vec4*)(et + (prow + j * 16) * EROW + ((wn * (BN / 2) + i * 16) / 2 + fq * 4) * 2) = pk;
            }
          }
        } else {
#pragma unroll
          for (int i = 0; i < FN; ++i) {
            const int c = tile_n * BN + pcol + i * 16;
            float tv[4] = {0.f, 0.f, 0.f, 0.f};
            if (p.temb && c < p.Cout) {
              const T* tp = (const T*)p.temb + (size_t)n * p.temb_stride + c;
              if (c + 3 < p.Cout) {
                const auto t4 = *(const typename Traits<T>::vec4*)tp;
#pragma unroll
                for (int r = 0; r < 4; ++r) tv[r] = to_f32(t4[r]);
              } else {
                for (int r = 0; r < 4 && c + r < p.Cout; ++r) tv[r] = to_f32(tp[r]);
              }
            }
            typename Traits<T>::vec4 pk;
#pragma unroll
            for (int r = 0; r < 4; ++r) {
              float a = acc[i][j][r];
              if constexpr (LN) a = ln_rstd * (a - ln_mean * lncs[i][r]);
              float x = a + bias[i][r] + tv[r];
              if (p.act == ES_ACT_SILU) x = silu_f(x);
              pk[r] = from_f32<T>(x * scale);
            }
            *(typename Traits<T>::vec4*)(et + (prow + j * 16) * EROW + (pcol + i * 16) * 2) = pk;
          }
        }
      }
    }
    __syncthreads();

    const int BNo = geglu ? BN / 2 : BNP;
    const int c_tile = tile_n * (geglu ? BN / 2 : BN);
    if (vec_store) {
      const int CH = BNo / 8;
      const float inv_ch = __builtin_amdgcn_rcpf((float)CH);
      auto store_rows = [&](auto mode_c) __attribute__((always_inline)) {
        constexpr int MODE = decltype(mode_c)::value;
#pragma unroll
        for (int k = 0; k < RPF; ++k) {
          const int idx = tid + k * NT;
          const int row = fast_div(idx, CH, inv_ch), ch = idx - row * CH;
          const int m = tile_m * BM + row, c = c_tile + ch * 8;
          if (idx < BM * CH && m < M && c < Cstore) {
            auto v = as_vec8<T>(*(const u32x4*)(et + row * EROW + ch * 16));
            const size_t o = (size_t)m * Cstore + c;
            if constexpr (MODE >= 2) {
              const auto rv = as_vec8<T>(rpre[k]);
              typename Traits<T>::vec8 lv, lo;
              if constexpr (MODE == 3) lv = as_vec8<T>(*(const u32x4*)((const T*)p.residual_lo + o));
#pragma unroll
              for (int e = 0; e < 8; ++e) {
                float sum = to_f32(v[e]) + to_f32(rv[e]);
                if constexpr (MODE == 3) sum += to_f32(lv[e]);
                v[e] = from_f32<T>(sum);
                lo[e] = from_f32<T>(sum - to_f32(v[e]));
              }
              store16((T*)p.out_lo + o, __builtin_bit_cast(u32x4, lo));
            } else if constexpr (MODE == 1) {
              const auto rv = as_vec8<T>(rpre[k]);
#pragma unroll
              for (int e = 0; e < 8; ++e) v[e] = from_f32<T>(to_f32(v[e]) + to_f32(rv[e]));
            }
            store16(outp + o, __builtin_bit_cast(u32x4, v));
            if (p.gn_part) *(u32x4*)(et + row * EROW + ch * 16) = __builtin_bit_cast(u32x4, v);
          }
        }
      };
      if (p.out_lo) { if (p.residual_lo) store_rows(std::integral_constant<int, 3>{}); else store_rows(std::integral_constant<int, 2>{}); }
      else if (resp) store_rows(std::integral_constant<int, 1>{});
      else store_rows(std::integral_constant<int, 0>{});
      if (p.gn_part) {
        __syncthreads();
        gn_emit_partials<T, NT>(et, EROW, BM, BNo, (float*)(et + BM * EROW), p.gn_part, tile_m * BM, M, c_tile, Cstore, HWout, p.gn_groups, tid);
      }
    } else {
      const float inv_bno = __builtin_amdgcn_rcpf((float)BNo);
      for (int idx = tid; idx < BM * BNo; idx += NT) {
        const int row = fast_div(idx, BNo, inv_bno), cc = idx - row * BNo;
        const int m = tile_m * BM + row, c = c_tile + cc;
        if (m < M && c < Cstore) {
          float x = to_f32(*(const T*)(et + row * EROW + cc * 2));
          if (resp) x += to_f32(resp[(size_t)m * Cstore + c]);
          outp[(size_t)m * Cstore + c] = from_f32<T>(x);
        }
      }
    }
  }
#if !ES_STAMPS
  if (p.prof && tid == 0) atomicMax(p.prof + 1, (unsigned long long)__builtin_amdgcn_s_memrealtime());
#else
  pstamp(4);
#endif
}

template <typename T>
__global__ __launch_bounds__(256) void splitk_reduce_kernel(const es_gemm_desc p, const int M) {
  const int oct = p.rows_padded / 8;
  const int idx = blockIdx.x * 256 + threadIdx.x;
  if (idx >= M * oct) return;
  const bool small = M * oct < (1 << 24);
  const int m = div_any(idx, oct, 1.0f / (float)oct, small);
  const int c0 = (idx - m * oct) * 8;
  if (c0 >= p.Cout) return;
  const int nv = p.Cout - c0 < 8 ? p.Cout - c0 : 8;
  const bool full = nv == 8 && (p.Cout & 7) == 0;
  const int n = div_any(m, p.Hout * p.Wout, 1.0f / (float)(p.Hout * p.Wout), small);
  const float* bsel = p.bias;
  if (p.ngroups > 1) {
    const int tm = m >> 7;
    bsel = p.bias_g[(tm >= p.mt_end[0]) + (tm >= p.mt_end[1]) + (tm >= p.mt_end[2])];
  }
  float bv[8] = {0.f, 0.f, 0.f, 0.f, 0.f, 0.f, 0.f, 0.f}, tv[8] = {0.f, 0.f, 0.f, 0.f, 0.f, 0.f, 0.f, 0.f};
  float rv[8] = {0.f, 0.f, 0.f, 0.f, 0.f, 0.f, 0.f, 0.f};
  if (bsel) {
    const f32x4 b0 = *(const f32x4*)(bsel + c0), b1 = *(const f32x4*)(bsel + c0 + 4);
#pragma unroll
    for (int r = 0; r < 4; ++r) { bv[r] = b0[r]; bv[4 + r] = b1[r]; }
  }
  if (p.temb) {
    const T* tp = (const T*)p.temb + (size_t)n * p.temb_stride + c0;
    if (full && (p.temb_stride & 7) == 0 && (((size_t)p.temb) & 15) == 0) {
      const auto t8 = as_vec8<T>(*(const u32x4*)tp);
#pragma unroll
      for (int r = 0; r < 8; ++r) tv[r] = to_f32(t8[r]);
    } else {
      for (int r = 0; r < nv; ++r) tv[r] = to_f32(tp[r]);
    }
  }
  if (p.residual) {
    const T* rp = (const T*)p.residual + (size_t)m * p.Cout + c0;
    if (full) {
      const auto r8 = as_vec8<T>(*(const u32x4*)rp);
#pragma unroll
      for (int r = 0; r < 8; ++r) rv[r] = to_f32(r8[r]);
    } else {
      for (int r = 0; r < nv; ++r) rv[r] = to_f32(rp[r]);
    }
  }
  float scale = p.out_scale;
  if (p.out_scale_dev) scale *= *p.out_scale_dev;
  f32x4 s0 = {0.f, 0.f, 0.f, 0.f}, s1 = {0.f, 0.f, 0.f, 0.f};
  const size_t zstride = (size_t)M * p.rows_padded;
  const float* w = p.workspace + (size_t)m * p.rows_padded + c0;
  int z = 0;
  for (; z + 4 <= p.splitk; z += 4) {
    f32x4 a[4], b[4];
#pragma unroll
    for (int u = 0; u < 4; ++u) { a[u] = *(const f32x4*)(w + (z + u) * zstride); b[u] = *(const f32x4*)(w + (z + u) * zstride + 4); }
#pragma unroll
    for (int u = 0; u < 4; ++u) { s0 += a[u]; s1 += b[u]; }
  }
  for (; z < p.splitk; ++z) {
    s0 += *(const f32x4*)(w + z * zstride);
    s1 += *(const f32x4*)(w + z * zstride + 4);
  }
  float v[8] = {s0[0], s0[1], s0[2], s0[3], s1[0], s1[1], s1[2], s1[3]};
#pragma unroll
  for (int r = 0; r < 8; ++r) {
    float x = v[r] + bv[r] + tv[r];
    if (p.act == ES_ACT_SILU) x = silu_f(x);
    x = to_f32(from_f32<T>(x * scale));
    v[r] = x + rv[r];
  }
  T* o = (T*)p.out + (size_t)m * p.Cout + c0;
  if (full && p.out_lo) {
    typename Traits<T>::vec8 pk, lo;
    if (p.residual_lo) {
      const auto l8 = as_vec8<T>(*(const u32x4*)((const T*)p.residual_lo + (size_t)m * p.Cout + c0));
#pragma unroll
      for (int r = 0; r < 8; ++r) v[r] += to_f32(l8[r]);
    }
#pragma unroll
    for (int r = 0; r < 8; ++r) { pk[r] = from_f32<T>(v[r]); lo[r] = from_f32<T>(v[r] - to_f32(pk[r])); }
    store16(o, __builtin_bit_cast(u32x4, pk));
    store16((T*)p.out_lo + (size_t)m * p.Cout + c0, __builtin_bit_cast(u32x4, lo));
  } else if (full) {
    typename Traits<T>::vec8 pk;
#pragma unroll
    for (int r = 0; r < 8; ++r) pk[r] = from_f32<T>(v[r]);
    store16(o, __builtin_bit_cast(u32x4, pk));
  } else {
    store_elems<T>(o, v, nv);
  }
}

template <typename T, int CB>
__global__ __launch_bounds__(64 * (CB / 8)) void splitk_reduce_gn_kernel(const es_gemm_desc p, const int M) {
  constexpr int OCT = CB / 8, NTH = 64 * OCT, ITEMS = 1, EROW = CB * 2 + 16;
  __shared__ __attribute__((aligned(16))) char smem[64 * EROW + (8 + 1) * CB * 8];
  const int tid = threadIdx.x;
  const int nct = p.rows_padded / CB;
  const int mb = blockIdx.x / nct, ct = blockIdx.x - mb * nct;
  const int HW = p.Hout * p.Wout;
  float scale = p.out_scale;
  if (p.out_scale_dev) scale *= *p.out_scale_dev;
  const size_t zstride = (size_t)M * p.rows_padded;
#pragma unroll
  for (int it = 0; it < ITEMS; ++it) {
    const int idx = tid + it * NTH;
    const int row = idx / OCT, o = idx - row * OCT;
    const int m = mb * 64 + row, c0 = ct * CB + o * 8;
    u32x4 res = {0u, 0u, 0u, 0u};
    if (c0 < p.Cout) {
      const int n = m / HW;
      const float* bsel = p.bias;
      if (p.ngroups > 1) {
        const int tm = m >> 7;
        bsel = p.bias_g[(tm >= p.mt_end[0]) + (tm >= p.mt_end[1]) + (tm >= p.mt_end[2])];
      }
      float bv[8] = {0.f, 0.f, 0.f, 0.f, 0.f, 0.f, 0.f, 0.f}, tv[8] = {0.f, 0.f, 0.f, 0.f, 0.f, 0.f, 0.f, 0.f};
      float rv[8] = {0.f, 0.f, 0.f, 0.f, 0.f, 0.f, 0.f, 0.f};
      if (bsel) {
        const f32x4 b0 = *(const f32x4*)(bsel + c0), b1 = *(const f32x4*)(bsel + c0 + 4);
#pragma unroll
        for (int r = 0; r < 4; ++r) { bv[r] = b0[r]; bv[4 + r] = b1[r]; }
      }
      if (p.temb) {
// ... 20 lines not shown
        for (int u = 0; u < 4; ++u) { a[u] = *(const f32x4*)(w + (z + u) * zstride); b[u] = *(const f32x4*)(w + (z + u) * zstride + 4); }
#pragma unroll
        for (int u = 0; u < 4; ++u) { s0 += a[u]; s1 += b[u]; }
      }
      for (; z < p.splitk; ++z) {
        s0 += *(const f32x4*)(w + z * zstride);
        s1 += *(const f32x4*)(w + z * zstride + 4);
      }
      float v[8] = {s0[0], s0[1], s0[2], s0[3], s1[0], s1[1], s1[2], s1[3]};
#pragma unroll
      for (int r = 0; r < 8; ++r) {
        float x = v[r] + bv[r] + tv[r];
        if (p.act == ES_ACT_SILU) x = silu_f(x);
        x = to_f32(from_f32<T>(x * scale));
        v[r] = x + rv[r];
      }
      typename Traits<T>::vec8 pk, lo;
      if (p.out_lo) {
        if (p.residual_lo) {
          const auto l8 = as_vec8<T>(*(const u32x4*)((const T*)p.residual_lo + (size_t)m * p.Cout + c0));
#pragma unroll
          for (int r = 0; r < 8; ++r) v[r] += to_f32(l8[r]);
        }
#pragma unroll
        for (int r = 0; r < 8; ++r) { pk[r] = from_f32<T>(v[r]); lo[r] = from_f32<T>(v[r] - to_f32(pk[r])); }
        store16((T*)p.out_lo + (size_t)m * p.Cout + c0, __builtin_bit_cast(u32x4, lo));
      } else {
#pragma unroll
        for (int r = 0; r < 8; ++r) pk[r] = from_f32<T>(v[r]);
      }
      res = __builtin_bit_cast(u32x4, pk);
      store16((T*)p.out + (size_t)m * p.Cout + c0, res);
    }
    *(u32x4*)(smem + row * EROW + o * 16) = res;
  }
  __syncthreads();
  gn_emit_partials<T, NTH>(smem, EROW, 64, CB, (float*)(smem + 64 * EROW), p.gn_part, mb * 64, M, ct * CB, p.Cout, HW, p.gn_groups, tid);
}

template <typename T>
int launch(const es_gemm_desc& d0, hipStream_t st) {
  es_gemm_desc d = d0;
  if (d.bn == 320 && !es_conv_gemm8p_takes(d)) { d.bn = 160; d.stages = 2; }
  if (d.bn == 256 && !es_conv_gemm8p_takes(d)) { d.bn = 128; d.stages = 2; }
  const int M = d.N * d.Hout * d.Wout;
  const int nk = d.Kpad / BK;
  const int Ctot = d.C1 + d.C2;
  const bool aligned = (Ctot % BK == 0) && (d.C1 % BK == 0);
  const int tn = d.rows_padded / d.bn;
  const int bm = d.bn == 64 ? 64 : 128;
  dim3 grid(((M + bm - 1) / bm) * tn * d.splitk);
  int stages = d.stages;
  if (stages == 0) stages = 2;
#define ES_LAUNCH_F(BMV, BNV, AL, ST, FMV)                                                                  \
  do {                                                                                                      \
    if (AL && d.korder) ES_LAUNCH_K(BMV, BNV, AL, ST, FMV, AL);                                             \
    else ES_LAUNCH_K(BMV, BNV, AL, ST, FMV, false);                                                         \
  } while (0)
#define ES_LAUNCH_K(BMV, BNV, AL, ST, FMV, KOV)                                                             \
  do {                                                                                                      \
    auto kfn = conv_gemm_kernel<T, BMV, BNV, AL, ST, FMV, false, KOV>;                                      \
    const size_t lds = (size_t)ST * (BMV + BNV) * BK * 2;                                                   \
    static bool attr_set = false;                                                                           \
    if (!attr_set) {                                                                                        \
      (void)hipFuncSetAttribute((const void*)kfn, hipFuncAttributeMaxDynamicSharedMemorySize, (int)lds);    \
      attr_set = true;                                                                                      \
    }                                                                                                       \
    hipLaunchKernelGGL(kfn, grid, dim3(BMV * 8 / FMV), lds, st, d, M, nk, d.t1, d.t2, d.Ct1, d.Ct2);                                  \
  } while (0)
#define ES_LAUNCH_LN(BMV, BNV, ST, FMV)                                                                      \
  do {                                                                                                      \
    auto kfn = conv_gemm_kernel<T, BMV, BNV, true, ST, FMV, true>;                                          \
    const size_t lds = (size_t)ST * (BMV + BNV) * BK * 2;                                                   \
    static bool attr_set = false;                                                                           \
    if (!attr_set) {                                                                                        \
      (void)hipFuncSetAttribute((const void*)kfn, hipFuncAttributeMaxDynamicSharedMemorySize, (int)lds);    \
      attr_set = true;                                                                                      \
    }                                                                                                       \
    hipLaunchKernelGGL(kfn, grid, dim3(BMV * 8 / FMV), lds, st, d, M, nk, d.t1, d.t2, d.Ct1, d.Ct2);                                  \
  } while (0)
#define ES_LAUNCH(BMV, BNV, AL, ST) ES_LAUNCH_F(BMV, BNV, AL, ST, 4)
#define ES_LAUNCH_ST(BNV)                                                                                   \
  do {                                                                                                      \
    if (d.waves == 8 && stages == 4 && BNV == 128) ES_LAUNCH_F(128, 128, true, 4, 2);                       \
    else if (d.waves == 8) ES_LAUNCH_F(128, BNV, true, 2, 2);                                               \
    else if (stages == 2) ES_LAUNCH(128, BNV, true, 2);                                                     \
    else if (stages == 3) ES_LAUNCH(128, BNV, true, 3);                                                     \
    else ES_LAUNCH(128, BNV, true, 4);                                                                      \
  } while (0)
  if (d.bn == 256) { if (es_conv_gemm8p_launch(d, st)) return -2; }
  else if (d.ln_colsum) {
    const bool w8 = d.waves == 8;
    if (d.bn == 64)            { if (stages == 4) ES_LAUNCH_LN(64, 64, 4, 2); else ES_LAUNCH_LN(64, 64, 2, 2); }
    else if (d.bn == 128 && w8) { if (stages == 4) ES_LAUNCH_LN(128, 128, 4, 2); else ES_LAUNCH_LN(128, 128, 2, 2); }
    else if (d.bn == 128)       { if (stages == 4) ES_LAUNCH_LN(128, 128, 4, 4); else ES_LAUNCH_LN(128, 128, 2, 4); }
    else if (w8)                { ES_LAUNCH_LN(128, 160, 2, 2); }
    else                        { if (stages == 4) ES_LAUNCH_LN(128, 160, 4, 4); else ES_LAUNCH_LN(128, 160, 2, 4); }
  }
  else if (d.bn == 64)  { if (stages == 4) ES_LAUNCH_F(64, 64, true, 4, 2); else ES_LAUNCH_F(64, 64, true, 2, 2); }
  else if (d.bn == 320) { if (es_conv_gemm8p_launch(d, st)) return -2; }
  else if (d.bn == 128) { if (aligned) ES_LAUNCH_ST(128); else ES_LAUNCH(128, 128, false, 2); }
  else                  { if (aligned) ES_LAUNCH_ST(160); else ES_LAUNCH(128, 160, false, 2); }
#undef ES_LAUNCH_ST
#undef ES_LAUNCH
#undef ES_LAUNCH_F
#undef ES_LAUNCH_K
#undef ES_LAUNCH_LN
  if (d.splitk > 1 && d.gn_part) {
    const int cb = (d.bn == 320 || d.bn == 160) ? 80 : (d.bn == 128 ? 128 : 64);
    dim3 grid((unsigned)((M / 64) * (d.rows_padded / cb)));
    if (cb == 80) hipLaunchKernelGGL((splitk_reduce_gn_kernel<T, 80>), grid, dim3(64 * 10), 0, st, d, M);
    else if (cb == 128) hipLaunchKernelGGL((splitk_reduce_gn_kernel<T, 128>), grid, dim3(64 * 16), 0, st, d, M);
    else hipLaunchKernelGGL((splitk_reduce_gn_kernel<T, 64>), grid, dim3(64 * 8), 0, st, d, M);
  } else if (d.splitk > 1) {
// ... 67 lines not shown
    }
    g0 = g1;
  }
  return 0;
}

}

extern "C" void es_set_error(const char* msg);

extern "C" unsigned long long es_set_operand_limit(unsigned long long bytes) {
  const unsigned long long prev = es_operand_limit_v;
  es_operand_limit_v = bytes && bytes < 0x7FFFFFFFull ? bytes : 0x7FFFFFFFull;
  return prev;
}

extern "C" size_t es_conv_gemm_workspace_bytes(const es_gemm_desc* d) {
  if (d->splitk <= 1) return 0;
  return (size_t)d->splitk * d->N * d->Hout * d->Wout * d->rows_padded * sizeof(float);
}

extern "C" int es_conv_gemm(const es_gemm_desc* d, void* stream) {
  const int Ctot = d->C1 + d->C2;
  const int Ktrue = d->ksize * d->ksize * Ctot + (d->t1 ? d->Ct1 + d->Ct2 : 0);
  if (!d->x || !d->out || (d->ngroups <= 1 && !d->w)) { es_set_error("es_conv_gemm: null pointer"); return -1; }
  if (d->ngroups > 4) { es_set_error("es_conv_gemm: at most 4 groups"); return -1; }
  if (d->ngroups > 1) {
    const int tm = (d->N * d->Hout * d->Wout + 127) / 128;
    for (int g = 0; g < d->ngroups; ++g)
      if (!d->w_g[g] || d->mt_end[g] <= (g ? d->mt_end[g - 1] : 0)) { es_set_error("es_conv_gemm: bad group table"); return -1; }
    if (d->mt_end[d->ngroups - 1] != tm || (d->N * d->Hout * d->Wout) % 128) { es_set_error("es_conv_gemm: groups must tile M in whole 128-pixel tiles"); return -1; }
    if (d->bn == 320 || d->bn == 256)
      for (int g = 0; g < d->ngroups; ++g)
        if (d->mt_end[g] & 1) { es_set_error("es_conv_gemm: 256-pixel tiles need groups of whole 256-pixel tiles"); return -1; }
  }
  if (d->bn != 64 && d->bn != 128 && d->bn != 160 && d->bn != 320 && d->bn != 256) { es_set_error("es_conv_gemm: bn must be 64, 128, 160, 256 or 320"); return -1; }
  if (d->bn == 256 && (d->C1 % BK || d->C2 % BK || (d->stages != 0 && d->stages != 2) || d->waves == 8 || d->korder || d->temb)) {
    es_set_error("es_conv_gemm: bn=256 is the 256-pixel phase-interleaved tile of the LayerNorm-folded / GEGLU linear layers: 64-aligned channels, 2 stages, tap-major K, no time embedding"); return -1; }
  if (d->bn == 64 && (d->C1 % BK || d->C2 % BK || d->stages == 3 || d->waves == 8 || d->act == ES_ACT_GEGLU)) {
    es_set_error("es_conv_gemm: bn=64 is the 64x64 tile: 64-aligned channels, 2 or 4 stages, no GEGLU"); return -1; }
  if (d->bn == 320 && (d->C1 % BK || d->C2 % BK || (d->stages != 0 && d->stages != 2) || d->act == ES_ACT_GEGLU || d->waves == 8)) {
    es_set_error("es_conv_gemm: bn=320 is the 256-pixel phase-interleaved tile: 64-aligned channels, 2 stages, no GEGLU"); return -1; }
  if (d->rows_padded % d->bn || d->rows_padded < d->Cout) { es_set_error("es_conv_gemm: bad rows_padded"); return -1; }
  if (d->Kpad % BK || d->Kpad < Ktrue) { es_set_error("es_conv_gemm: bad Kpad"); return -1; }
  if (d->C1 % 8 || d->C2 % 8 || (d->C2 && !d->x2)) { es_set_error("es_conv_gemm: channels must be multiples of 8"); return -1; }
  if (d->C2 && (d->C1 % BK || d->C2 % BK)) { es_set_error("es_conv_gemm: concatenated sources need C1, C2 multiples of 64"); return -1; }
  if ((size_t)d->rows_padded * d->Kpad * 2 >= 0x7FFFFFFFull) { es_set_error("es_conv_gemm: weights larger than 2 GiB (32-bit buffer offsets)"); return -1; }
  if (d->N < 1 || d->Hout < 1 || d->Wout < 1 || d->Cout < 1) { es_set_error("es_conv_gemm: empty problem"); return -1; }
  const bool chunked = oversize(*d);
  if (chunked) {
    const char* why = nullptr;
    if (launch_in_chunks(*d, nullptr, &why, true)) { es_set_error(why); return -1; }
  }
  if (d->ksize != 1 && d->ksize != 3) { es_set_error("es_conv_gemm: ksize must be 1 or 3"); return -1; }
  if (d->t1 && (d->stride != 1 || d->upsample || d->C1 % BK || d->C2 % BK || d->Ct1 % BK || d->Ct2 % BK || d->Ct1 < BK ||
                (d->Ct2 && !d->t2) || d->ln_colsum || d->Hout != d->Hsrc || d->Wout != d->Wsrc ||
                false)) {
    es_set_error("es_conv_gemm: 1x1 tail sources need stride 1, no upsample, same-size output, 64-aligned channels"); return -1; }
  if (!d->t1 && (d->t2 || d->Ct1 || d->Ct2)) { es_set_error("es_conv_gemm: tail fields set without t1"); return -1; }
  if (d->x_nmod < 0 || (d->x_nmod && (d->x2 || d->t1 || d->x_nmod > d->N))) { es_set_error("es_conv_gemm: x_nmod needs a single source and 0 < x_nmod <= N"); return -1; }
  if (d->out_lo && (!d->residual || (d->Cout & 7) || d->act == ES_ACT_GEGLU)) {
    es_set_error("es_conv_gemm: out_lo (wide residual stream) needs a residual and an output width that is a multiple of 8"); return -1; }
  if (d->residual_lo && !d->out_lo) { es_set_error("es_conv_gemm: residual_lo without out_lo"); return -1; }
  if (d->gn_part) {
    const int hw = d->Hout * d->Wout;
    if (d->gn_groups < 1 || d->Cout % d->gn_groups || (d->Cout & 7) || hw % 64 || d->act == ES_ACT_GEGLU || d->ln_colsum ||
        d->Cout / d->gn_groups > (d->bn == 320 ? 160 : d->bn) || (d->splitk > 1 && d->Cout / d->gn_groups > 64)) {
      es_set_error("es_conv_gemm: gn_part needs H*W % 64 == 0, Cout % 8 == 0 and whole GroupNorm groups no wider than the N tile"); return -1; }
  }
  if (d->korder != 0 && (d->korder != 1 || d->ksize != 3 || d->C1 % BK || d->C2 % BK || d->ln_colsum)) {
    es_set_error("es_conv_gemm: korder 1 (chunk-major K) needs ksize 3 and 64-aligned C1, C2"); return -1; }
  if (d->splitk < 1 || d->splitk > d->Kpad / BK) { es_set_error("es_conv_gemm: bad splitk"); return -1; }
  if (d->splitk > 1 && (!d->workspace || d->act == ES_ACT_GEGLU)) { es_set_error("es_conv_gemm: splitk needs workspace and no GEGLU"); return -1; }
  if (d->act == ES_ACT_GEGLU && ((d->bn != 128 && d->bn != 256) || d->Cout % 32)) { es_set_error("es_conv_gemm: GEGLU needs bn=128 | 256, Cout%32==0"); return -1; }
  if (d->stages != 0 && (d->stages < 2 || d->stages > 4)) { es_set_error("es_conv_gemm: stages must be 0 (auto), 2, 3 or 4"); return -1; }
  if (d->waves != 0 && d->waves != 4 && d->waves != 8) { es_set_error("es_conv_gemm: waves must be 0 (auto), 4 or 8"); return -1; }
  if (d->ln_colsum && (d->ksize != 1 || d->stride != 1 || d->C2 || d->C1 % BK || d->Kpad != d->C1 || d->splitk != 1 ||
                       d->bn == 320 || d->upsample || d->temb || d->stages == 3)) {
    es_set_error("es_conv_gemm: LayerNorm fold needs a plain linear layer: ksize 1, one source, K = C1 (multiple of 64), splitk 1, bn 64|128|160"); return -1; }
  if (d->ln_colsum && d->ngroups > 1)
    for (int g = 0; g < d->ngroups; ++g)
      if (!d->ln_colsum_g[g]) { es_set_error("es_conv_gemm: grouped LayerNorm fold needs ln_colsum_g for every group"); return -1; }
  if (d->waves == 8 && (d->bn == 320 || d->C1 % BK || d->C2 % BK || d->stages == 3 ||
                        (d->stages == 4 && d->bn != 128))) {
    es_set_error("es_conv_gemm: waves=8 is the 128-pixel tile on 8 waves: 64-aligned channels, 2 stages (4 with bn=128)"); return -1; }
  ES_PLAN_RECORD(ES_OP_CONV_GEMM, d, sizeof(*d));
  hipStream_t st = (hipStream_t)stream;
  es_gemm_desc dd = *d;
  for (int g = dd.ngroups > 1 ? dd.ngroups : 0; g < 4; ++g) dd.mt_end[g] = 0x7FFFFFFF;
  if (chunked) {
    const char* why = "es_conv_gemm: launch failed";
    const int rc = launch_in_chunks(*d, st, &why, false);
    if (rc) es_set_error(why);
    return rc;
  }
  int rc = dd.dtype == ES_F16 ? launch<f16>(dd, st) : launch<bf16>(dd, st);
  if (rc) es_set_error("es_conv_gemm: launch failed");
  return rc;
}
```

### edgestyle_amd/engine.py

```python
import os
import weakref
from typing import Dict, List, Optional, Sequence, Tuple

import torch

from . import lib as L
from . import ops
from .config import UNetConfig, VAEConfig

SD = Dict[str, torch.Tensor]


def fold_lora(sd: SD) -> SD:
    out = {k: v for k, v in sd.items() if ".lora_layer." not in k}
    for k in sd:
        if k.endswith(".lora_layer.down.weight"):
            base = k[: -len(".lora_layer.down.weight")]
            up = sd[base + ".lora_layer.up.weight"].double()
            out[base + ".weight"] = (sd[base + ".weight"].double() + up @ sd[k].double()).float()
    return out


_PACK_CACHE = {}


class _Packer:

    def __init__(self, sd: SD, dtype, device):
        self.sd, self.dtype, self.device = sd, dtype, device

    def t(self, key):
        return self.sd[key].to(self.device, torch.float32)

    def conv(self, p: str, cin_pad: Optional[int] = None, geglu=False, cout_pad=None) -> ops.PackedWeight:
        w = self.sd[p + ".weight"]
        b = self.sd.get(p + ".bias")
        key = (id(w), None if b is None else id(b), str(self.dtype), str(self.device), geglu, cin_pad, cout_pad)
        hit = _PACK_CACHE.get(key)
        if hit is not None and hit[0]() is w and (b is None or hit[1]() is b):
            return hit[2]
        pw = ops.pack_weight(self.t(p + ".weight"), None if b is None else b.to(self.device), self.dtype,
                             self.device, geglu=geglu, cin_pad=cin_pad, cout_pad=cout_pad)
        _PACK_CACHE[key] = (weakref.ref(w), None if b is None else weakref.ref(b), pw)
        return pw

    def conv_tail(self, p: str, pt: str) -> ops.PackedWeight:
        w, wt = self.sd[p + ".weight"], self.sd[pt + ".weight"]
        key = (id(w), id(wt), str(self.dtype), str(self.device), "tail")
        hit = _PACK_CACHE.get(key)
        if hit is not None and hit[0]() is w and hit[1]() is wt:
            return hit[2]
        pw = ops.pack_weight_tail(self.t(p + ".weight"), self.t(pt + ".weight"), self.t(p + ".bias") + self.t(pt + ".bias"),
                                  self.dtype, self.device)
        _PACK_CACHE[key] = (weakref.ref(w), weakref.ref(wt), pw)
        return pw

    def cat(self, ps: Sequence[str], bias: bool) -> ops.PackedWeight:
        w = torch.cat([self.t(p + ".weight") for p in ps], 0)
        b = torch.cat([self.t(p + ".bias") for p in ps], 0) if bias else None
        return ops.pack_weight(w, b, self.dtype, self.device)

    def norm(self, p: str) -> Tuple[torch.Tensor, torch.Tensor]:
        return self.t(p + ".weight").contiguous(), self.t(p + ".bias").contiguous()

    def cat_ln(self, ps: Sequence[str], bias: bool, ln: str, geglu: bool = False) -> ops.PackedWeight:
        w = torch.cat([self.t(p + ".weight") for p in ps], 0)
        b = torch.cat([self.t(p + ".bias") for p in ps], 0) if bias else None
        return ops.pack_weight_ln(w, b, self.t(ln + ".weight"), self.t(ln + ".bias"), 1e-5, self.dtype, self.device,
                                  geglu=geglu)


SHORTCUT_FOLD = os.environ.get("ES_SHORTCUT_FOLD", "1") == "1"
FFO_FOLD = os.environ.get("ES_FFO_FOLD", "1") == "1"
LN_FOLD = os.environ.get("ES_LN_FOLD", "1") in ("1", "qk")
LN_FOLD_FF = os.environ.get("ES_LN_FOLD", "1") == "1"


class Resnet:
    def __init__(self, pk: _Packer, p: str, groups: int, eps: float, temb_off: Optional[int]):
        self.n1, self.n2 = pk.norm(p + ".norm1"), pk.norm(p + ".norm2")
        self.conv1, self.conv2 = pk.conv(p + ".conv1"), pk.conv(p + ".conv2")
        self.short = pk.conv(p + ".conv_shortcut") if (p + ".conv_shortcut.weight") in pk.sd else None
        self.groups, self.eps, self.temb_off = groups, eps, temb_off
        self.cout = self.conv1.cout
        self.conv2s = None
        w2, ws_ = pk.sd[p + ".conv2.weight"], pk.sd.get(p + ".conv_shortcut.weight")
        if SHORTCUT_FOLD and ws_ is not None and w2.shape[1] % 64 == 0 and ws_.shape[1] % 64 == 0:
            self.conv2s = pk.conv_tail(p + ".conv2", p + ".conv_shortcut")

    def __call__(self, x, tproj, x2=None):
        h = ops.group_norm(x, self.n1[0], self.n1[1], self.groups, self.eps, True, x2=x2)
        temb = None if self.temb_off is None else tproj[:, self.temb_off:]
        h = ops.conv_gemm(h, self.conv1, temb=temb, gn_groups=self.groups)
        h = ops.group_norm(h, self.n2[0], self.n2[1], self.groups, self.eps, True)
        if self.conv2s is not None and (x2 is None or (x.shape[3] % 64 == 0 and x2.shape[3] % 64 == 0)):
            return ops.conv_gemm(h, self.conv2s, tail=(x, x2), gn_groups=self.groups)
# ... 89 lines not shown
        out = [a for blk in self.down for (_, a) in blk if a is not None]
        return out + [self.mid_attn]

    def context(self, ehs, outs: Optional[List[torch.Tensor]] = None) -> List[torch.Tensor]:
        tr = self.transformers()
        if outs is not None and outs[0].shape[0] == ehs.shape[0]:
            return [t.context(ehs, o) for t, o in zip(tr, outs)]
        return [t.context(ehs) for t in tr]

    def time_proj(self, t_dev: torch.Tensor, step_idx: Optional[torch.Tensor] = None) -> torch.Tensor:
        e = ops.timestep_embedding(t_dev, self.cfg.block_out_channels[0], self.dtype)
        e = ops.linear(e, self.t1, act=L.ACT_SILU)
        e = ops.linear(e, self.t2, act=L.ACT_SILU)
        return ops.linear(e, self.tproj)

    @property
    def tproj_width(self) -> int:
        return self.tproj.cout

    def run(self, h, tproj, ctx: List[torch.Tensor]):
        skips = [h]
        ci = 0
        for i, blk in enumerate(self.down):
            for r, a in blk:
                h = r(h, tproj)
                if a is not None:
                    h = a(h, ctx[ci]); ci += 1
                skips.append(h)
            if self.downsample[i] is not None:
                h = ops.conv_gemm(h, self.downsample[i], stride=2, gn_groups=self.cfg.norm_num_groups)
                skips.append(h)
        h = self.mid0(h, tproj)
        h = self.mid_attn(h, ctx[ci])
        h = self.mid1(h, tproj)
        return skips, h


class UNet(Encoder):
    def __init__(self, sd: SD, cfg: UNetConfig, dtype, device):
        n = len(cfg.block_out_channels)
        extra = [f"up_blocks.{i}.resnets.{j}" for i in range(n) for j in range(cfg.layers_per_block + 1)]
        super().__init__(sd, cfg, dtype, device, extra_resnets=extra)
        pk, g, eps, heads = self.pk, cfg.norm_num_groups, cfg.norm_eps, cfg.num_heads
        self.up: List[List[Tuple[Resnet, Optional[Transformer]]]] = []
        self.upsample: List[Optional[ops.PackedWeight]] = []
        for i in range(n):
            blk = []
            for j in range(cfg.layers_per_block + 1):
                nm = f"up_blocks.{i}.resnets.{j}"
                r = Resnet(pk, nm, g, eps, self.temb_offs[nm])
                a = Transformer(pk, f"up_blocks.{i}.attentions.{j}", heads, g) if cfg.up_has_attn[i] else None
                blk.append((r, a))
            self.up.append(blk)
            self.upsample.append(pk.conv(f"up_blocks.{i}.upsamplers.0.conv") if i != n - 1 else None)
        self.norm_out = pk.norm("conv_norm_out")
        self.conv_out = pk.conv("conv_out")
        del self.pk

    def transformers(self):
        return super().transformers() + [a for blk in self.up for (_, a) in blk if a is not None]

    def encode(self, x, tproj, ctx):
        h = ops.conv_gemm(x, self.conv_in, gn_groups=self.cfg.norm_num_groups)
        return self.run(h, tproj, ctx)

    def forward(self, x, tproj, ctx, down_res: Optional[Sequence] = None, mid_res=None, out=None, encoded=None,
                presummed: bool = False):
        skips, h = encoded if encoded is not None else self.encode(x, tproj, ctx)
        skips = list(skips)
        if presummed:
            skips = [r.reshape(s.shape) for s, r in zip(skips, down_res)]
            h = mid_res.reshape(h.shape)
        else:
            if down_res is not None:
                skips = [ops.add(s, r.reshape(s.shape)) for s, r in zip(skips, down_res)]
            if mid_res is not None:
                h = ops.add(h, mid_res.reshape(h.shape))
        ci = len(super().transformers())
        cfg = self.cfg
        for i, blk in enumerate(self.up):
            for r, a in blk:
                h = r(h, tproj, x2=skips.pop())
                if a is not None:
                    h = a(h, ctx[ci]); ci += 1
            if self.upsample[i] is not None:
                h = ops.conv_gemm(h, self.upsample[i], upsample=True)
        h = ops.group_norm(h, self.norm_out[0], self.norm_out[1], cfg.norm_num_groups, cfg.norm_eps, True)
        return ops.conv_gemm(h, self.conv_out, out=out)


class ControlNet(Encoder):

    def __init__(self, sd: SD, cfg: UNetConfig, dtype, device, uses_vae: bool = False):
        super().__init__(sd, cfg, dtype, device)
        pk = self.pk
        table = cfg.residual_table()
        self.zero = [pk.conv(f"controlnet_down_blocks.{i}") for i in range(len(table) - 1)]
        self.zero_mid = pk.conv("controlnet_mid_block")
        self.uses_vae = uses_vae
        self.cond = None
        if not uses_vae and "controlnet_cond_embedding.conv_in.weight" in pk.sd:
            ce = cfg.conditioning_embedding_out_channels
            p = "controlnet_cond_embedding"
            self.cond = [pk.conv(p + ".conv_in", cin_pad=8)]
            self.cond += [pk.conv(f"{p}.blocks.{i}") for i in range(2 * (len(ce) - 1))]
            self.cond.append(pk.conv(p + ".conv_out"))
        del self.pk
# ... 32 lines not shown
            p = f"multi_controlnet_down_blocks.{i}" if i < len(self.table) - 1 else "multi_controlnet_mid_block"
            self.params.append(ops.pack_fusion_params(sd, p, dtype, device))

    def forward(self, res_per_net: Sequence[Sequence[torch.Tensor]], bs: Sequence[Sequence[int]], N: int,
                scales: Sequence[float], scales_dev=None, addends=None, first_level: int = 0):
        nl = len(res_per_net[0])
        table = self.table[first_level:first_level + nl]
        blocks = [([res_per_net[i][k] for i in range(6)], [bs[i][k] for i in range(6)], self.params[first_level + k], s * s, c)
                  for k, (c, s) in enumerate(table)]
        outs = ops.fusion_blocks(blocks, N, scales, scales_dev, addends=addends, first_block=first_level)
        return [o.reshape(N, s, s, c) for o, (c, s) in zip(outs, table)]


class VAE:
    def __init__(self, sd: SD, cfg: VAEConfig, dtype, device, decoder: bool = True, encoder: bool = True):
        self.cfg, self.dtype, self.device = cfg, dtype, device
        pk = _Packer(sd, dtype, device)
        g, eps = cfg.norm_num_groups, cfg.norm_eps
        ch = cfg.block_out_channels
        n = len(ch)
        self.lat_pad = (cfg.latent_channels + 7) // 8 * 8

        def mid(side):
            a = f"{side}.mid_block.attentions.0"
            return dict(r0=Resnet(pk, f"{side}.mid_block.resnets.0", g, eps, None),
                        gn=pk.norm(a + ".group_norm"),
                        qkv=pk.cat([a + ".to_q", a + ".to_k", a + ".to_v"], bias=True),
                        o=pk.conv(a + ".to_out.0"),
                        r1=Resnet(pk, f"{side}.mid_block.resnets.1", g, eps, None))
        if encoder:
            self.e_in = pk.conv("encoder.conv_in", cin_pad=8)
            self.e_down = []
            for i in range(n):
                rs = [Resnet(pk, f"encoder.down_blocks.{i}.resnets.{j}", g, eps, None)
                      for j in range(cfg.layers_per_block)]
                ds = pk.conv(f"encoder.down_blocks.{i}.downsamplers.0.conv") if i != n - 1 else None
                self.e_down.append((rs, ds))
            self.e_mid = mid("encoder")
            self.e_norm = pk.norm("encoder.conv_norm_out")
            self.e_out = pk.conv("encoder.conv_out")
            self.quant = pk.conv("quant_conv")
        if decoder:
            self.post_quant = pk.conv("post_quant_conv", cin_pad=self.lat_pad, cout_pad=8)
            b = sd.get("post_quant_conv.bias")
            self.post_quant_scaled = ops.pack_weight(
                (pk.t("post_quant_conv.weight").double() / cfg.scaling_factor).float(), None if b is None else b.to(device), dtype,
                device, cin_pad=self.lat_pad, cout_pad=8)
            self.d_in = pk.conv("decoder.conv_in", cin_pad=8)
            self.d_mid = mid("decoder")
            self.d_up = []
            for i in range(n):
                rs = [Resnet(pk, f"decoder.up_blocks.{i}.resnets.{j}", g, eps, None)
                      for j in range(cfg.layers_per_block + 1)]
                us = pk.conv(f"decoder.up_blocks.{i}.upsamplers.0.conv") if i != n - 1 else None
                self.d_up.append((rs, us))
            self.d_norm = pk.norm("decoder.conv_norm_out")
            self.d_out = pk.conv("decoder.conv_out")

    def _mid(self, m, h):
        cfg = self.cfg
        h = m["r0"](h, None)
        N, H, W, C = h.shape
        n = ops.group_norm(h, m["gn"][0], m["gn"][1], cfg.norm_num_groups, cfg.norm_eps, False).reshape(N, H * W, C)
        qkv = ops.linear(n, m["qkv"])
        a = ops.attention(qkv[:, :, :C], qkv[:, :, C:2 * C], qkv[:, :, 2 * C:], 1)
        h = ops.linear(a, m["o"], residual=h.reshape(N, H * W, C)).reshape(N, H, W, C)
        return m["r1"](h, None)

    def encode_moments(self, img):
        cfg = self.cfg
        h = ops.conv_gemm(img, self.e_in)
        for rs, ds in self.e_down:
            for r in rs:
                h = r(h, None)
            if ds is not None:
                h = ops.conv_gemm(h, ds, stride=2, pad=0, out_hw=(h.shape[1] // 2, h.shape[2] // 2))
        h = self._mid(self.e_mid, h)
        h = ops.group_norm(h, self.e_norm[0], self.e_norm[1], cfg.norm_num_groups, cfg.norm_eps, True)
        h = ops.conv_gemm(h, self.e_out)
        return ops.conv_gemm(h, self.quant)

    def decode(self, z, unscaled_latents: bool = False):
        cfg = self.cfg
        h = ops.conv_gemm(z, self.post_quant_scaled if unscaled_latents else self.post_quant)
        h = ops.conv_gemm(h, self.d_in)
        h = self._mid(self.d_mid, h)
        for rs, us in self.d_up:
            for r in rs:
                h = r(h, None)
            if us is not None:
                h = ops.conv_gemm(h, us, upsample=True)
        h = ops.group_norm(h, self.d_norm[0], self.d_norm[1], cfg.norm_num_groups, cfg.norm_eps, True)
        return ops.conv_gemm(h, self.d_out)


class GroupedEncoder:

    def __init__(self, encoders: Sequence[Encoder], counts: Sequence[int]):
        self.encs, self.counts = list(encoders), list(counts)
        e0 = self.encs[0]
        self.cfg = e0.cfg
        for e in self.encs[1:]:
            if e.cfg.block_out_channels != e0.cfg.block_out_channels or e.cfg.layers_per_block != e0.cfg.layers_per_block:
                raise L.EdgeStyleHipError("grouped encoders must share the architecture")
        self.ntot = sum(self.counts)
        self.width = max(e.tproj_width for e in self.encs)

# ... 69 lines not shown
```

### edgestyle_amd/lib.py

```python
import ctypes as C
import os

_HERE = os.path.dirname(os.path.abspath(__file__))
LIB_PATH = os.environ.get("ES_HIP_LIB") or os.path.join(_HERE, "lib", "libedgestyle_hip.so")

ES_F16, ES_BF16, ES_F32 = 0, 1, 2
ABI_VERSION = 7
ACT_NONE, ACT_SILU, ACT_GEGLU = 0, 1, 2


class GemmDesc(C.Structure):
    _fields_ = [
        ("x", C.c_void_p), ("x2", C.c_void_p), ("w", C.c_void_p), ("bias", C.c_void_p), ("temb", C.c_void_p),
        ("residual", C.c_void_p), ("out_scale_dev", C.c_void_p), ("out", C.c_void_p), ("workspace", C.c_void_p),
        ("prof", C.c_void_p),
        ("N", C.c_int32), ("Hsrc", C.c_int32), ("Wsrc", C.c_int32), ("C1", C.c_int32), ("C2", C.c_int32),
        ("Hout", C.c_int32), ("Wout", C.c_int32), ("Cout", C.c_int32),
        ("rows_padded", C.c_int32), ("Kpad", C.c_int32),
        ("ksize", C.c_int32), ("stride", C.c_int32), ("pad", C.c_int32),
        ("upsample", C.c_int32), ("temb_stride", C.c_int32), ("act", C.c_int32), ("splitk", C.c_int32),
        ("bn", C.c_int32), ("dtype", C.c_int32),
        ("ngroups", C.c_int32), ("mt_end", C.c_int32 * 4), ("w_g", C.c_void_p * 4), ("bias_g", C.c_void_p * 4),
        ("stages", C.c_int32), ("xcd_m_fastest", C.c_int32), ("waves", C.c_int32),
        ("out_scale", C.c_float),
        ("ln_colsum", C.c_void_p), ("ln_colsum_g", C.c_void_p * 4), ("ln_eps", C.c_float),
        ("t1", C.c_void_p), ("t2", C.c_void_p), ("Ct1", C.c_int32), ("Ct2", C.c_int32),
        ("x_nmod", C.c_int32), ("korder", C.c_int32), ("residual_lo", C.c_void_p), ("out_lo", C.c_void_p),
        ("gn_part", C.c_void_p), ("gn_groups", C.c_int32),
    ]


class XsDesc(C.Structure):
    _fields_ = [
        ("x", C.c_void_p), ("out", C.c_void_p), ("w", C.c_void_p), ("bias", C.c_void_p),
        ("w_g", C.c_void_p * 4), ("bias_g", C.c_void_p * 4), ("prof", C.c_void_p),
        ("mt_end", C.c_int32 * 4), ("ngroups", C.c_int32),
        ("M", C.c_int32), ("K", C.c_int32), ("Cout", C.c_int32), ("rows_padded", C.c_int32),
        ("ldo", C.c_int32), ("geglu", C.c_int32), ("ln", C.c_int32), ("ln_eps", C.c_float),
        ("nslices", C.c_int32), ("chunks_per_slice", C.c_int32), ("dtype", C.c_int32),
        ("residual", C.c_void_p),
        ("gn_part", C.c_void_p), ("gn_gamma", C.c_void_p), ("gn_beta", C.c_void_p), ("gn_gamma_g", C.c_void_p * 4), ("gn_beta_g", C.c_void_p * 4),
        ("gn_groups", C.c_int32), ("gn_nchunk", C.c_int32), ("gn_hw", C.c_int32), ("gn_eps", C.c_float),
    ]


class CtxGeometry(C.Structure):
    _fields_ = [("B", C.c_int32), ("cfg", C.c_int32), ("h", C.c_int32), ("w", C.c_int32),
                ("latent_channels", C.c_int32), ("latent_pad", C.c_int32), ("n_conds", C.c_int32),
                ("n_steps", C.c_int32), ("dtype", C.c_int32), ("guess_mode", C.c_int32)]


PLAN_STEP_GENERIC, PLAN_PREP, PLAN_STEP, PLAN_DECODE, PLAN_CONDS, PLAN_STEP_UNET = 0, 1, 2, 3, 4, 5
PLAN_COUNT = 6
(BUF_SAMPLE, BUF_T_ROWS, BUF_EHS, BUF_COND0, BUF_COND1, BUF_COND2, BUF_COND3, BUF_COND4, BUF_COND5, BUF_SCALES, BUF_NOISE,
 BUF_LATENTS, BUF_STEP_IDX, BUF_T_TABLE, BUF_SCALE_TABLE, BUF_COEF, BUF_TIMESTEPS, BUF_IMAGE) = range(18)
BUF_COND_IMG0, BUF_COND_NOISE0 = 18, 24
BUF_HIST0, BUF_COUNT = 30, 33
SCHED_DDIM, SCHED_UNIPC = 0, 1
OP_CONV_GEMM, OP_LINEAR_XS, OP_ATTENTION = 1, 2, 3


class AttnDesc(C.Structure):
    _fields_ = [
        ("q", C.c_void_p), ("k", C.c_void_p), ("v", C.c_void_p), ("o", C.c_void_p),
        ("N", C.c_int32), ("heads", C.c_int32), ("Sq", C.c_int32), ("Skv", C.c_int32), ("d", C.c_int32),
        ("ldq", C.c_int32), ("ldk", C.c_int32), ("ldv", C.c_int32), ("ldo", C.c_int32),
        ("bsq", C.c_int64), ("bsk", C.c_int64), ("bsv", C.c_int64), ("bso", C.c_int64),
        ("scale", C.c_float), ("dtype", C.c_int32),
    ]


class GnDesc(C.Structure):
    _fields_ = [
        ("x", C.c_void_p), ("x2", C.c_void_p), ("out", C.c_void_p),
        ("gamma", C.c_void_p), ("beta", C.c_void_p), ("partials", C.c_void_p),
        ("N", C.c_int32), ("HW", C.c_int32), ("C1", C.c_int32), ("C2", C.c_int32), ("groups", C.c_int32),
        ("eps", C.c_float), ("silu", C.c_int32), ("dtype", C.c_int32),
        ("ngroups", C.c_int32), ("n_end", C.c_int32 * 4), ("gamma_g", C.c_void_p * 4), ("beta_g", C.c_void_p * 4),
        ("ext_chunks", C.c_int32), ("stats_only", C.c_int32),
    ]

# ... 23 lines not shown
class ImageU8(C.Structure):
    _fields_ = [("data", C.c_void_p), ("height", C.c_int32), ("width", C.c_int32), ("channels", C.c_int32), ("row_stride", C.c_int64)]


class Philox(C.Structure):
    _fields_ = [("seed", C.c_uint64), ("offset", C.c_uint64)]


class RandnDesc(C.Structure):
    _fields_ = [("seed", C.c_uint64), ("offset", C.c_uint64), ("numel", C.c_int64), ("blocks", C.c_int32), ("scale", C.c_float),
                ("round_dtype", C.c_int32), ("N", C.c_int64), ("C", C.c_int64), ("HW", C.c_int64), ("Cstride", C.c_int64)]


class TextConfig(C.Structure):
    _fields_ = [(n, C.c_int32) for n in ("vocab_size", "hidden", "heads", "layers", "intermediate", "max_positions")] + \
        [("ln_eps", C.c_float), ("act", C.c_int32)]


class Tensor(C.Structure):
    _fields_ = [("key", C.c_char_p), ("data", C.c_void_p), ("shape", C.c_int64 * 4), ("ndim", C.c_int32), ("dtype", C.c_int32)]


class StateDict(C.Structure):
    _fields_ = [("tensors", C.POINTER(Tensor)), ("count", C.c_int32)]


NET_CONTROLNET, NET_CONTROL_LORA_VAE, NET_CONTROL_LORA = 0, 1, 2


class Weights(C.Structure):
    _fields_ = [("unet", StateDict), ("vae", StateDict), ("fusion", StateDict), ("controlnet", StateDict * 6),
                ("controlnet_kind", C.c_int32 * 6), ("n_controlnets", C.c_int32), ("net_of_cond", C.c_int32 * 6)]


class ModelConfig(C.Structure):
    _fields_ = [("in_channels", C.c_int32), ("out_channels", C.c_int32),
                ("n_blocks", C.c_int32), ("block_out_channels", C.c_int32 * 4), ("down_has_attn", C.c_int32 * 4),
                ("layers_per_block", C.c_int32), ("num_heads", C.c_int32), ("cross_attention_dim", C.c_int32),
                ("norm_num_groups", C.c_int32), ("norm_eps", C.c_float),
                ("n_cond_embed", C.c_int32), ("cond_embed_channels", C.c_int32 * 4), ("conditioning_channels", C.c_int32),
                ("text_tokens", C.c_int32),
                ("vae_n_blocks", C.c_int32), ("vae_block_out_channels", C.c_int32 * 4), ("vae_layers_per_block", C.c_int32),
                ("vae_latent_channels", C.c_int32), ("vae_norm_num_groups", C.c_int32),
                ("vae_norm_eps", C.c_float), ("vae_scaling_factor", C.c_float)]


_I32 = C.c_int32


class LaunchQuery(C.Structure):
    _fields_ = [(n, C.c_longlong) for n in ("M", "hw", "w_numel", "src_numel")] + \
        [(n, _I32) for n in ("ksize", "stride", "upsample", "C1", "C2", "rows_padded", "kpad", "cin", "ctail", "cout", "geglu", "has_ln", "act",
                             "has_temb", "has_residual", "residual_dense", "unit_scale", "n_tails", "x_rep", "wide", "dtype", "gn_groups",
                             "ngroups", "n_counts")] + [("group_n", _I32 * 4)] + [(n, _I32) for n in ("groups_agree", "force_splitk", "stages")]


class LaunchKnobs(C.Structure):
    _fields_ = [(n, _I32) for n in ("xs_enabled", "xs_residual", "xs_min_m", "big_tile", "big_tile_256", "small_tile", "eight_waves", "deep_ring",
                                    "gn_handover", "wide_stream", "gn_fold", "force_bn", "force_waves", "force_stages", "xcd_order")]


class LaunchChoice(C.Structure):
    _fields_ = [(n, _I32) for n in ("route", "bn", "splitk", "stages", "waves", "xcd_m_fastest", "gn_partials", "wide")]


ROUTE_CONV_GEMM, ROUTE_LINEAR_XS = 0, 1
XS_FORM_KC_MASK, XS_FORM_GEGLU, XS_FORM_LN, XS_FORM_RES, XS_FORM_PP, XS_FORM_GN = 0xFF, 0x100, 0x200, 0x400, 0x800, 0x1000
GN_FORM_SLAB, GN_FORM_TWO_LAUNCHES = 1, 2
GN_ROUTE_FIELDS = ("form", "gpb", "slots", "cpt", "ppb", "nchunk", "ps", "lanes", "blocks", "ipt", "general", "lds")

_P, _I, _F, _L = C.c_void_p, C.c_int, C.c_float, C.c_int64
SYMBOLS = {
    "es_abi_version": (C.c_int, []),
    "es_set_operand_limit": (C.c_ulonglong, [C.c_ulonglong]),
    "es_last_error": (C.c_char_p, []),
    "es_sizeof_desc": (C.c_size_t, [_I]),
    "es_conv_gemm": (C.c_int, [C.POINTER(GemmDesc), _P]),
    "es_conv_gemm_workspace_bytes": (C.c_size_t, [C.POINTER(GemmDesc)]),
    "es_linear_xs": (C.c_int, [C.POINTER(XsDesc), _P]),
    "es_linear_xs_set_pp": (C.c_int, [_I]),
    "es_linear_xs_last_form": (C.c_int, []),
    "es_attention": (C.c_int, [C.POINTER(AttnDesc), _P]),
    "es_attention_set_kvres": (C.c_int, [_I]),
    "es_attention_last_kernel": (C.c_int, []),
    "es_group_norm": (C.c_int, [C.POINTER(GnDesc), _P]),
    "es_group_norm_partials_bytes": (C.c_size_t, [_I, _I]),
    "es_group_norm_is_slab": (C.c_int, [_I, _I, _I]),
    "es_group_norm_chunks": (C.c_int, [_I]),
    "es_group_norm_route": (C.c_int, [C.POINTER(GnDesc), C.POINTER(C.c_int32)]),
    "es_layer_norm_route": (C.c_int, [_I]),
    "es_layer_norm": (C.c_int, [_P, _P, _P, _P, _I, _I, _F, _I, _P]),
    "es_fusion_block": (C.c_int, [C.POINTER(FusionDesc), _P]),
    "es_fusion_scratch_bytes": (C.c_size_t, [_I]),
    "es_fusion_blocks": (C.c_int, [C.POINTER(FusionDesc), _I, _P]),
    "es_timestep_embedding": (C.c_int, [_P, _P, _I, _I, _I, _P]),
    "es_cfg_ddim_step": (C.c_int, [_P, _P, _P, _P, _P, _F, _I, _I, _I, _I, _I, _I, _I, _P]),
    "es_cfg_unipc_step": (C.c_int, [_P, _P, _P, _P, _P, _P, _P, _P, _F, _I, _I, _I, _I, _I, _I, _I, _P]),
    "es_nchw_f32_to_nhwc": (C.c_int, [_P, _P, _I, _I, _I, _I, _I, _P]),
    "es_nhwc_to_nchw_f32": (C.c_int, [_P, _P, _I, _I, _I, _I, _F, _F, _I, _I, _P]),
    "es_add": (C.c_int, [_P, _P, _P, _L, _I, _P]),
    "es_vae_sample": (C.c_int, [_P, _P, _P, _I, _I, _I, _I, _F, _I, _P]),
    "es_incr": (C.c_int, [_P, _P]),
    "es_clock_probe": (C.c_int, [_P, C.c_uint, _P]),
    "es_gather_row": (C.c_int, [_P, _P, _P, _I, _I, _P]),
    "es_layer_norm_grouped": (C.c_int, [C.POINTER(LnDesc), _P]),
    "es_latents_to_input": (C.c_int, [_P, _P, _I, _I, _I, _I, _I, _I, _P]),
    "es_memcpy": (C.c_int, [_P, _P, C.c_size_t, _P]),
    "es_memcpy2d": (C.c_int, [_P, C.c_size_t, _P, C.c_size_t, C.c_size_t, C.c_size_t, _P]),
    "es_fill_f32": (C.c_int, [_P, _F, C.c_size_t, _P]),
    "es_plan_create": (_P, []),
    "es_plan_destroy": (None, [_P]),
    "es_plan_begin_record": (C.c_int, [_P]),
    "es_plan_end_record": (C.c_int, [_P]),
    "es_plan_size": (C.c_int, [_P]),
    "es_plan_count": (C.c_int, [_P, _I]),
    "es_plan_launch": (C.c_int, [_P, _P]),
    "es_ctx_create": (C.c_int, [_I, C.POINTER(_P)]),
    "es_ctx_destroy": (None, [_P]),
    "es_ctx_set_geometry": (C.c_int, [_P, C.POINTER(CtxGeometry)]),
    "es_ctx_set_plan": (C.c_int, [_P, _I, _P]),
    "es_ctx_bind": (C.c_int, [_P, _I, _P, C.c_size_t]),
    "es_ctx_buffer": (_P, [_P, _I, C.POINTER(C.c_size_t)]),
    "es_ctx_arena_bytes": (C.c_size_t, [_P]),
    "es_ctx_set_options": (C.c_int, [_P, C.POINTER(C.c_float), _F, _F, _I]),
    "es_ctx_set_scheduler": (C.c_int, [_P, _I]),
    "es_ctx_set_alphas_cumprod_f64": (C.c_int, [_P, C.POINTER(C.c_double), _I]),
    "es_unipc_coef_table": (C.c_int, [C.POINTER(C.c_double), _I, C.POINTER(C.c_float), _I, C.POINTER(C.c_float)]),
    "es_ctx_set_alphas_cumprod": (C.c_int, [_P, C.POINTER(C.c_float), _I]),
    "es_ctx_plan_size": (C.c_int, [_P, _I]),
    "es_ctx_plan": (_P, [_P, _I]),
    "es_ctx_load": (C.c_int, [C.c_char_p, _I, C.POINTER(_P)]),
    "es_ctx_save": (C.c_int, [_P, C.c_char_p]),
    "es_plan_export": (C.c_size_t, [_P, _P, C.c_size_t]),
    "es_plan_import": (_P, [_P, C.c_size_t]),
    "es_plan_pointer_fields": (C.c_int, [_I, C.POINTER(C.c_int32), C.POINTER(C.c_int32), _I, C.POINTER(C.c_int32)]),
    "es_ctx_launch_plan": (C.c_int, [_P, _I, C.POINTER(C.c_float), _P]),
    "es_ddim_coef_table": (C.c_int, [C.POINTER(C.c_float), _I, C.POINTER(C.c_float), _I, C.POINTER(C.c_float)]),
    "es_denoise_step": (C.c_int, [_P, _P, _F, _P, C.POINTER(_P), C.POINTER(C.c_float), _P, _P]),
    "es_denoise_loop": (C.c_int, [_P, _P, _P, _F, C.POINTER(C.c_float), _I, _P]),
    "es_vae_decode": (C.c_int, [_P, _P, _P, _P]),
    "es_prepare_conds": (C.c_int, [_P, C.POINTER(_P), C.POINTER(_P), _P]),
    "es_load_weights": (C.c_int, [C.POINTER(Weights), C.POINTER(ModelConfig), C.POINTER(CtxGeometry), _I, C.POINTER(_P)]),
    "es_plan_gemm_choice": (C.c_int, [C.c_longlong, _I, _I, _I, C.POINTER(C.c_int), _I, _I, C.POINTER(C.c_int), C.POINTER(C.c_int),
                                      C.POINTER(C.c_int)]),
    "es_linear_xs_eligible": (C.c_int, [C.c_longlong, _I, _I, _I, _I, _I, _I]),
    "es_launch_choose": (C.c_int, [C.POINTER(LaunchQuery), C.POINTER(LaunchKnobs), C.POINTER(LaunchChoice)]),
    "es_launch_route": (C.c_int, [C.POINTER(LaunchQuery), C.POINTER(LaunchKnobs)]),
    "es_launch_gn_fold": (C.c_int, [C.POINTER(LaunchQuery), _I, C.POINTER(LaunchKnobs)]),
    "es_launch_gn_handover": (C.c_int, [C.c_longlong, _I, _I, C.POINTER(LaunchKnobs)]),
    "es_launch_wide_stream": (C.c_int, [_I, C.POINTER(LaunchKnobs)]),
    "es_conv_gemm8p_form_ok": (C.c_int, [_I, _I, _I, C.c_longlong, _I]),
    "es_ctx_graph_hazard": (C.c_int, []),
    "es_plan_set_dry": (C.c_int, [_I]),
    "es_image_fit": (C.c_int, [_I, _I, _I, C.POINTER(C.c_int32)]),
    "es_image_resize_coeffs": (C.c_int, [_I, _I, C.POINTER(C.c_int32), C.POINTER(C.c_int32), C.POINTER(C.c_int32), _I]),
    "es_image_resize_workspace_bytes": (C.c_size_t, [C.POINTER(ImageU8), _I, _I]),
    "es_image_resize_u8": (C.c_int, [C.POINTER(ImageU8), _I, _P, _I, _P, C.c_size_t, _P]),
    "es_image_u8_to_f32": (C.c_int, [_P, _P, _I, _I, _I, _I, _P]),
    "es_image_f32_to_u8": (C.c_int, [_P, _P, _I, _I, _I, _P]),
    "es_prepare_conds_u8": (C.c_int, [_P, C.POINTER(ImageU8), C.POINTER(C.c_int32), C.POINTER(_P), _P, C.c_size_t, _P]),
    "es_vae_decode_u8": (C.c_int, [_P, _P, _P, _P]),
    "es_philox4x32_10": (C.c_int, [C.POINTER(C.c_uint32), C.POINTER(C.c_uint32), C.POINTER(C.c_uint32)]),
    "es_philox_block_cap": (C.c_int, [_I]),
    "es_philox_blocks": (C.c_int, [_L, _I]),
    "es_philox_advance": (_L, [_L, _I]),
    "es_randn": (C.c_int, [_P, C.POINTER(RandnDesc), _P]),
    "es_randn_host": (C.c_int, [_P, C.POINTER(RandnDesc)]),
    "es_ctx_draw_latents": (C.c_int, [_P, C.POINTER(Philox), _I, _F, _I, _P, _P]),
    "es_ctx_draw_cond_noise": (C.c_int, [_P, C.POINTER(Philox), _I, _P]),
    "es_attention_causal": (C.c_int, [C.POINTER(AttnDesc), _P]),
    "es_text_embed": (C.c_int, [_P, _P, _P, _P, _I, _I, _I, _I, _I, _P]),
    "es_text_encoder_create": (C.c_int, [C.POINTER(StateDict), C.POINTER(TextConfig), _I, _I, _I, C.POINTER(_P)]),
    "es_text_encoder_destroy": (None, [_P]),
    "es_text_encoder_arena_bytes": (C.c_size_t, [_P]),
    "es_text_encode": (C.c_int, [_P, _P, _I, _P, _P]),
}

_lib = None


FUSION_MAX_BATCH = 13


class EdgeStyleHipError(RuntimeError):
    pass


def load():
    global _lib
    if _lib is not None:
        return _lib
    if not os.path.exists(LIB_PATH):
        raise EdgeStyleHipError(
            f"{LIB_PATH} not found: build it with `python -c 'import __graft_entry__ as g; g.build()'` "
            "(hipcc --offload-arch=gfx950). There is no CPU fallback for the product path.")
    lib = C.CDLL(LIB_PATH)
    for name, (res, args) in SYMBOLS.items():
        fn = getattr(lib, name)
        fn.restype = res
        fn.argtypes = args
    if lib.es_abi_version() != ABI_VERSION:
# ... 22 lines not shown
```

### edgestyle_amd/ops.py

```python
import ctypes as C
import math
import os as _os
from dataclasses import dataclass
from typing import Optional, Sequence

import torch

from . import lib as L

_DT = {torch.float16: L.ES_F16, torch.bfloat16: L.ES_BF16}
LANE = 0


class lane:

    def __init__(self, i: int):
        self.i = i

    def __enter__(self):
        global LANE
        self.prev, LANE = LANE, self.i

    def __exit__(self, *a):
        global LANE
        LANE = self.prev


XCD_ORDER = -1
DEEP_RING = _os.environ.get("ES_DEEP_RING", "1") == "1"
FORCE_BN = 0
FORCE_STAGES = 0
FORCE_WAVES = 0
EIGHT_WAVES = _os.environ.get("ES_EIGHT_WAVES", "1") == "1"
SMALL_TILE = _os.environ.get("ES_SMALL_TILE", "1") == "1"
PROFILE = None


class Profiler:

    def __init__(self, device, capacity: int = 8192, stamps: bool = True):
        self.slots = torch.empty((capacity, 2), dtype=torch.int64, device=device)
        self.meta = []
        self.stamps = stamps
        self.descs = []
        self.reset()

    def reset(self):
        self.slots[:, 0] = 1 << 62
        self.slots[:, 1] = 0

    def next(self, meta) -> int:
        i = len(self.meta)
        if i >= self.slots.shape[0]:
            raise L.EdgeStyleHipError("Profiler capacity exceeded")
        self.meta.append(meta)
        return self.slots[i].data_ptr() if self.stamps else 0

    def replay_gemms(self, only_ksize: int = 0):
        lib = L.load()
        for d in self.descs:
            if only_ksize and (isinstance(d, L.XsDesc) or int(d.ksize) != only_ksize):
                continue
            fn = lib.es_linear_xs if isinstance(d, L.XsDesc) else lib.es_conv_gemm
            L.check(fn(C.byref(d), _stream()), "GEMM replay")

    def results(self, first: int = 0):
        s = self.slots[first:len(self.meta)].cpu().tolist()
        return [(m, (e - b) * 1e-8) for m, (b, e) in zip(self.meta[first:], s) if e > 0]
BK = 64
BM = 128


def _stream():
    return C.c_void_p(torch.cuda.current_stream().cuda_stream)


def _ptr(t: Optional[torch.Tensor]):
    return None if t is None else C.c_void_p(t.data_ptr())


def _dt(t: torch.Tensor) -> int:
    try:
        return _DT[t.dtype]
    except KeyError:
        raise L.EdgeStyleHipError(f"unsupported dtype {t.dtype}: the HIP path computes in fp16 or bf16")


@dataclass
class PackedWeight:
    w: torch.Tensor
    bias: Optional[torch.Tensor]
    cout: int
    cin: int
    ksize: int
    bn: int
    geglu: bool = False
    ln_colsum: Optional[torch.Tensor] = None
    ln_eps: float = 1e-5
    ctail: int = 0
    korder: int = 0

    @property
    def rows_padded(self):
        return self.w.shape[0]

    @property
    def kpad(self):
        return self.w.shape[1]


def choose_bn(cout: int) -> int:
    return 160 if (cout % 160 == 0 and cout % 128 != 0) else 128


CHUNK_MAJOR = _os.environ.get("ES_CHUNK_MAJOR", "0") == "1"


def choose_korder(k: int, cin_padded: int) -> int:
    return 1 if (CHUNK_MAJOR and k == 3 and cin_padded % BK == 0) else 0


def _chunk_major(w: torch.Tensor, k: int, cin: int) -> torch.Tensor:
    cout = w.shape[0]
    return w.reshape(cout, k * k, cin // BK, BK).permute(0, 2, 1, 3).reshape(cout, k * k * cin)


def pack_weight(weight: torch.Tensor, bias: Optional[torch.Tensor], dtype, device, geglu: bool = False,
                cin_pad: Optional[int] = None, cout_pad: Optional[int] = None) -> PackedWeight:
    if weight.dim() == 2:
        weight = weight[:, :, None, None]
    weight = weight.to(device=device, dtype=torch.float32)
    cout, cin, k, _ = weight.shape
    cp = cin_pad or ((cin + 7) // 8 * 8)
    w = weight.permute(0, 2, 3, 1)
    if cp != cin:
        w = torch.nn.functional.pad(w, (0, cp - cin))
    w = w.reshape(cout, k * k * cp)
    korder = choose_korder(k, cp)
    if korder:
        w = _chunk_major(w, k, cp)
    b = None if bias is None else bias.to(device=device, dtype=torch.float32)
    if geglu:
        inner = cout // 2
        assert inner % 16 == 0
        idx = torch.arange(cout, device=device)
        blk, within = idx // 32, idx % 32
        src = torch.where(within < 16, blk * 16 + within, inner + blk * 16 + (within - 16))
        w = w[src]
        if b is not None:
            b = b[src]
    cout_eff = cout_pad or cout
    bn = 128 if geglu else choose_bn(cout_eff)
    rows = (cout_eff + bn - 1) // bn * bn
    ktrue = w.shape[1]
    kpad = (ktrue + BK - 1) // BK * BK
    wp = torch.zeros(rows, kpad, dtype=dtype, device=device)
    wp[:cout, :ktrue] = w.to(dtype)
    bp = None
    if b is not None:
        bp = torch.zeros(rows, dtype=torch.float32, device=device)
        bp[:cout] = b
    return PackedWeight(wp, bp, cout_eff, cp, k, bn, geglu, korder=korder)


def pack_weight_tail(weight: torch.Tensor, tail_weight: torch.Tensor, bias: Optional[torch.Tensor], dtype, device) -> PackedWeight:
    weight = weight.to(device=device, dtype=torch.float32)
    tw = tail_weight.to(device=device, dtype=torch.float32).reshape(tail_weight.shape[0], -1)
    cout, cin, k, _ = weight.shape
    if cin % BK or tw.shape[1] % BK or tw.shape[0] != cout:
        raise L.EdgeStyleHipError("pack_weight_tail: conv and tail channels must be multiples of 64, equal Cout")
    korder = choose_korder(k, cin)
    wm = weight.permute(0, 2, 3, 1).reshape(cout, k * k * cin)
    w = torch.cat([_chunk_major(wm, k, cin) if korder else wm, tw], 1)
    bn = choose_bn(cout)
    rows = (cout + bn - 1) // bn * bn
    wp = torch.zeros(rows, w.shape[1], dtype=dtype, device=device)
    wp[:cout] = w.to(dtype)
    bp = None
    if bias is not None:
        bp = torch.zeros(rows, dtype=torch.float32, device=device)
        bp[:cout] = bias.to(device=device, dtype=torch.float32)
    return PackedWeight(wp, bp, cout, cin, k, bn, False, ctail=tw.shape[1], korder=korder)


def pack_weight_ln(weight: torch.Tensor, bias: Optional[torch.Tensor], gamma: torch.Tensor, beta: torch.Tensor,
                   eps: float, dtype, device, geglu: bool = False) -> PackedWeight:
    w = weight.to(device=device, dtype=torch.float32)
    if w.dim() == 4:
        w = w[:, :, 0, 0]
    g = gamma.to(device=device, dtype=torch.float32)
    b = beta.to(device=device, dtype=torch.float32)
    fb = w.double() @ b.double()
    if bias is not None:
        fb = fb + bias.to(device=device, dtype=torch.float64)
    pw = pack_weight(w * g[None, :], fb.float(), dtype, device, geglu=geglu)
    pw.ln_colsum = pw.w.double().sum(dim=1).float().contiguous()
    pw.ln_eps = float(eps)
    return pw


_workspace = {}
_workspace_retired = []


def _get_workspace(nbytes: int, device) -> torch.Tensor:
    device = (device, LANE)
    ws = _workspace.get(device)
    if ws is None or ws.numel() * 4 < nbytes:
        if torch.cuda.is_current_stream_capturing():
            raise L.EdgeStyleHipError("split-K workspace too small during graph capture; run one eager warm-up first")
        if ws is not None:
            _workspace_retired.append(ws)
        ws = torch.empty(max(nbytes // 4, 1 << 22), dtype=torch.float32, device=device[0])
        _workspace[device] = ws
    return ws


PLAN_T160, PLAN_ALONE, PLAN_TFIX, PLAN_RED_FIX, PLAN_SLAB_BYTES_PER_UNIT = 1.25, 0.9, 2.0, 12.0, 4.0e6
PLAN_T320, PLAN_BIG_MIN_M, PLAN_T320_FIX, PLAN_BIG_MIN_NK = 2.3, 2048, 3.0, 16
PLAN_T256, PLAN_T256_FIX, PLAN_T256_GEGLU, PLAN_LN_TK, PLAN_T256_MARGIN = 2.6, 6.0, 7.0, 1.55, 0.93
PLAN_T64_ALONE, PLAN_T64, PLAN_T64_LONG, PLAN_SMALL_MAX_M = 0.5, 0.16, 1.5, 16384
BIG_TILE = _os.environ.get("ES_BIG_TILE", "1") == "1"
BIG_TILE_256 = _os.environ.get("ES_BIG_TILE_256", "1") != "0"
PLAN_MIN_SLICE, PLAN_NK_NOSPLIT, PLAN_RESIDENT = 12, 10, 512


def plan_gemm(M: int, rows_padded: int, kpad: int, geglu: bool = False, bns=(160, 128, 64), allow_split: bool = True):
    arr = (C.c_int * len(bns))(*[int(b) for b in bns])
    bn, sk, st = C.c_int(), C.c_int(), C.c_int()
    if L.load().es_plan_gemm_choice(int(M), int(rows_padded), int(kpad), int(bool(geglu)), arr, len(bns), int(bool(allow_split)),
                                    C.byref(bn), C.byref(sk), C.byref(st)) != 0:
        raise L.EdgeStyleHipError(f"plan_gemm: rows_padded {rows_padded} fits no N tile")
    stages = st.value
    if stages == 4 and not (DEEP_RING and LANE == 0):
        stages = 2
# ... 53 lines not shown
            rounds = max(wgs / 256.0, 0.9) if bn == 320 else float(-(-wgs // resident))
            t = rounds * ((nk / sk) * tk + (PLAN_T320_FIX if bn == 320 else PLAN_TFIX))
            if sk > 1:
                t += PLAN_RED_FIX + sk * M * rows_padded * 8.0 / PLAN_SLAB_BYTES_PER_UNIT
            if best is None or t < best[0]:
                best = (t, bn, sk, wgs)
    if best is None:
        raise L.EdgeStyleHipError(f"plan_gemm: rows_padded {rows_padded} fits no N tile")
    _, bn, sk, wgs = best
    if bn == 64:
        stages = 4 if (DEEP_RING and LANE == 0 and wgs <= PLAN_RESIDENT and nk // sk >= 6) else 2
    else:
        stages = 4 if (bn != 320 and DEEP_RING and LANE == 0 and wgs <= PLAN_RESIDENT // 2 and nk // sk >= 6) else 2
    return bn, sk, stages


def choose_launch_bn(M: int, pw: "PackedWeight") -> int:
    return plan_gemm(M, pw.rows_padded, pw.kpad, pw.geglu)[0]


def choose_splitk(M: int, rows_padded: int, bn: int, kpad: int) -> int:
    return plan_gemm(M, rows_padded, kpad, bns=(bn,))[1]


def plan_launch(M: int, pw: "PackedWeight", bn: int):
    _, sk, st = plan_gemm(M, pw.rows_padded, pw.kpad, pw.geglu, bns=(bn,))
    return sk, st


XS_ENABLED = _os.environ.get("ES_XS", "1") == "1"
XS_RESIDUAL = _os.environ.get("ES_XS_RESIDUAL", "1") == "1"
XS_TARGET_WGS = 256
XS_FORCE_SLICES = 0
XS_MIN_M = int(_os.environ.get("ES_XS_MIN_M", "8192"))
_zero_bias = {}


def xs_shape_reference(M: int, pw: "PackedWeight", min_m: int) -> bool:
    if pw.ksize != 1 or pw.kpad not in (320, 640) or pw.cin != pw.kpad or pw.ctail:
        return False
    ch = 64 if pw.kpad == 320 else 32
    line = ch * (128 // (ch if pw.geglu else 2 * ch))
    if pw.cout % line or pw.cout < 4 * line:
        return False
    if min_m and (M < min_m or (M < 4 * min_m and pw.cout < (960 if pw.kpad == 320 else 1920))):
        return False
    return True


def launch_knobs(**over) -> "L.LaunchKnobs":
    kn = dict(xs_enabled=XS_ENABLED, xs_residual=XS_RESIDUAL, xs_min_m=XS_MIN_M, big_tile=BIG_TILE, big_tile_256=BIG_TILE_256,
              small_tile=SMALL_TILE, eight_waves=EIGHT_WAVES, deep_ring=DEEP_RING and LANE == 0,
              gn_handover=(2 if GN_HANDOVER_ALL else 1) if GN_HANDOVER else 0, wide_stream={"auto": -1, "1": 1}.get(WIDE_STREAM, 0),
              gn_fold=GN_FOLD, force_bn=FORCE_BN, force_waves=FORCE_WAVES, force_stages=FORCE_STAGES, xcd_order=XCD_ORDER)
    return L.LaunchKnobs(**{k: int(v) for k, v in dict(kn, **over).items()})


def launch_query(M: int, hw: int, pw: "PackedWeight", pws=None, group_n=None, **facts) -> "L.LaunchQuery":
    q = L.LaunchQuery(M=M, hw=hw, w_numel=pw.w.numel(), ksize=pw.ksize, stride=1, rows_padded=pw.rows_padded, kpad=pw.kpad, cin=pw.cin,
                      ctail=pw.ctail, cout=pw.cout, geglu=pw.geglu, has_ln=pw.ln_colsum is not None, residual_dense=1, unit_scale=1, x_rep=1)
    for name, v in facts.items():
        setattr(q, name, int(v))
    if pws is not None:
        q.ngroups, q.groups_agree = len(pws), all((p.ln_colsum is None) == (pw.ln_colsum is None) for p in pws)
    if group_n is not None:
        q.n_counts = len(group_n)
        q.group_n[:] = (list(group_n) + [0] * 4)[:4]
    return q


def xs_eligible(M: int, pw: "PackedWeight", pws, group_n, hw: int) -> bool:
    return L.load().es_launch_route(C.byref(launch_query(M, hw, pw, pws, group_n)), C.byref(launch_knobs(force_bn=0))) == L.ROUTE_LINEAR_XS


def linear_xs(x: torch.Tensor, pw, M: int, out: torch.Tensor, group_rows=None, residual: Optional[torch.Tensor] = None,
              gn: Optional[dict] = None) -> torch.Tensor:
    def bad(msg):
        return L.EdgeStyleHipError("linear_xs: " + msg)
    pws = None
    if isinstance(pw, (list, tuple)):
        pws = list(pw) if len(pw) > 1 else None
        pw = pw[0]
    cstore = pw.cout // 2 if pw.geglu else pw.cout
    if x.dtype not in (torch.float16, torch.bfloat16):
        raise bad(f"x must be fp16 or bf16, not {x.dtype}")
    for name, t in (("out", out), ("residual", residual)):
        if t is not None and (t.dtype != x.dtype or t.device != x.device):
            raise bad(f"{name} is {t.dtype} on {t.device}, x is {x.dtype} on {x.device}")
    if M < 1 or x.dim() != 2 or tuple(x.shape) != (M, pw.kpad) or not x.is_contiguous():
        raise bad(f"x must be a contiguous [M, K] = [{M}, {pw.kpad}] (got shape {tuple(x.shape)}, strides {x.stride()})")
    if x.device.type != "meta" and x.data_ptr() % 16:
        raise bad("x must start at a multiple of 16 bytes (16-byte vector loads)")
    for name, t in (("out", out), ("residual", residual)):
        if t is None:
            continue
        if t.dim() != 2 or tuple(t.shape) != (M, cstore):
            raise bad(f"{name} must be [M, cstore] = [{M}, {cstore}], not {tuple(t.shape)}")
        if t.stride(1) != 1:
            raise bad(f"{name}: innermost stride must be 1")
    ldo = out.stride(0) if M > 1 else cstore
    if ldo < cstore or ldo % 8:
        raise bad(f"out: row pitch {ldo} must be a multiple of 8 elements and at least the width {cstore}")
    if residual is not None and M > 1 and residual.stride(0) != ldo:
        raise bad(f"residual: row pitch {residual.stride(0)} differs from out's {ldo} (the kernel reads it with out's)")
    for name, t in (("out", out), ("residual", residual)):
        if t is not None and t.device.type != "meta" and t.data_ptr() % 16:
            raise bad(f"{name} must start at a multiple of 16 bytes (16-byte vector accesses)")
# ... 91 lines not shown


def conv_gemm(x: torch.Tensor, pw: PackedWeight, *, stride: int = 1, pad: Optional[int] = None,
              upsample: bool = False, x2: Optional[torch.Tensor] = None, temb: Optional[torch.Tensor] = None,
              residual: Optional[torch.Tensor] = None, act: int = L.ACT_NONE, out_scale: float = 1.0,
              out_scale_dev: Optional[torch.Tensor] = None, out: Optional[torch.Tensor] = None,
              out_hw=None, splitk: Optional[int] = None, stages: int = 0,
              group_n: Optional[Sequence[int]] = None, tail: Optional[Sequence[torch.Tensor]] = None,
              x_rep: int = 1, wide: bool = False, out_lo: Optional[torch.Tensor] = None, gn_groups: int = 0,
              gn_part: Optional[torch.Tensor] = None):
    pws = None
    if isinstance(pw, (list, tuple)):
        pws = list(pw)
        pw = pws[0]
        if len(pws) == 1:
            pws = None
    N, H, W, C1 = x.shape
    nsrc = N
    if x_rep > 1:
        if x2 is not None or tail:
            raise L.EdgeStyleHipError("conv_gemm: x_rep needs a single source")
        N = N * x_rep
    C2 = 0 if x2 is None else x2.shape[3]
    if C1 + C2 != pw.cin:
        raise L.EdgeStyleHipError(f"conv_gemm: input channels {C1}+{C2} != packed {pw.cin}")
    tails = [t for t in (tail or ()) if t is not None]
    if sum(t.shape[3] for t in tails) != pw.ctail or len(tails) > 2:
        raise L.EdgeStyleHipError(f"conv_gemm: tail channels {[t.shape[3] for t in tails]} != packed {pw.ctail}")
    k = pw.ksize
    if pad is None:
        pad = 1 if k == 3 else 0
    Hin, Win = (H * 2, W * 2) if upsample else (H, W)
    if out_hw is None:
        Hout = (Hin + 2 * pad - k) // stride + 1
        Wout = (Win + 2 * pad - k) // stride + 1
    else:
        Hout, Wout = out_hw
    act_i = L.ACT_GEGLU if pw.geglu else act
    cstore = pw.cout // 2 if pw.geglu else pw.cout
    if out is None:
        out = torch.empty((N, Hout, Wout, cstore), dtype=x.dtype, device=x.device)
    M = N * Hout * Wout
    for what, t, numel in (("x", x, None), ("x2", x2, nsrc * H * W * C2), ("residual", residual, M * cstore), ("out", out, M * cstore)):
        if t is None:
            continue
        if not t.is_contiguous():
            raise L.EdgeStyleHipError(f"conv_gemm: {what} must be contiguous (got shape {tuple(t.shape)}, strides {t.stride()})")
        if t.dtype != x.dtype or (numel is not None and t.numel() != numel):
            raise L.EdgeStyleHipError(f"conv_gemm: {what} has {t.numel()} {t.dtype} elements, the launch needs {numel} {x.dtype}")
    q = launch_query(M, Hout * Wout, pw, pws, group_n, src_numel=x.numel() * x_rep + (x2.numel() if x2 is not None else 0), stride=stride,
                     upsample=upsample, C1=C1, C2=C2, act=act, has_temb=temb is not None, has_residual=residual is not None,
                     unit_scale=out_scale == 1.0 and out_scale_dev is None, n_tails=len(tails), x_rep=x_rep, wide=wide, dtype=_dt(x),
                     gn_groups=gn_groups, force_splitk=splitk or 0, stages=stages)
    ch = L.LaunchChoice()
    if L.load().es_launch_choose(C.byref(q), C.byref(launch_knobs()), C.byref(ch)) != 0:
        raise L.EdgeStyleHipError(f"plan_gemm: rows_padded {pw.rows_padded} fits no N tile")
    if ch.route == L.ROUTE_LINEAR_XS:
        linear_xs(x.reshape(M, C1), pws if pws is not None else pw, M, out.reshape(M, cstore),
                  None if pws is None else [n * Hout * Wout for n in group_n],
                  residual=None if residual is None else residual.reshape(M, cstore))
        return out
    bn, splitk = ch.bn, ch.splitk
    d = L.GemmDesc()
    d.x, d.x2, d.w = x.data_ptr(), (x2.data_ptr() if x2 is not None else None), pw.w.data_ptr()
    d.bias = pw.bias.data_ptr() if pw.bias is not None else None
    d.temb = temb.data_ptr() if temb is not None else None
    d.residual = residual.data_ptr() if residual is not None else None
    d.out_scale_dev = out_scale_dev.data_ptr() if out_scale_dev is not None else None
    d.out = out.data_ptr()
    d.N, d.Hsrc, d.Wsrc, d.C1, d.C2 = N, H, W, C1, C2
    d.Hout, d.Wout, d.Cout = Hout, Wout, pw.cout
    d.rows_padded, d.Kpad = pw.rows_padded, pw.kpad
    d.ksize, d.stride, d.pad = k, stride, pad
    d.upsample = 1 if upsample else 0
    d.temb_stride = temb.stride(0) if temb is not None else 0
    d.act, d.splitk, d.bn, d.dtype, d.out_scale = act_i, splitk, bn, _dt(x), out_scale
    d.stages, d.waves, d.xcd_m_fastest = ch.stages, ch.waves, ch.xcd_m_fastest
    d.korder = pw.korder
    if ch.gn_partials:
        shape = (N, 2 * (Hout * Wout // 64), gn_groups, 2)
        part = gn_part if gn_part is not None else torch.empty(shape, dtype=torch.float32, device=x.device)
        if tuple(part.shape) != shape or part.dtype != torch.float32 or not part.is_contiguous():
            raise L.EdgeStyleHipError(f"conv_gemm: gn_part must be a contiguous fp32 {shape}")
        d.gn_part, d.gn_groups = part.data_ptr(), gn_groups
        out._gnp = (part, gn_groups)
    if ch.wide:
        lo_in = getattr(residual, "_lo", None)
        if lo_in is not None:
            if lo_in.numel() != residual.numel() or not lo_in.is_contiguous():
                raise L.EdgeStyleHipError("conv_gemm: the residual's low part does not match it")
            d.residual_lo = lo_in.data_ptr()
        if out_lo is None:
            out_lo = torch.empty_like(out)
        elif out_lo.shape != out.shape or out_lo.dtype != out.dtype or not out_lo.is_contiguous():
            raise L.EdgeStyleHipError("conv_gemm: out_lo must match out")
        d.out_lo = out_lo.data_ptr()
        out._lo = out_lo
    d.x_nmod = nsrc if x_rep > 1 else 0
    if splitk > 1:
        ws = _get_workspace(splitk * M * pw.rows_padded * 4, x.device)
        d.workspace = ws.data_ptr()
    if pw.ln_colsum is not None:
        if (pws is not None and any(q.ln_colsum is None for q in pws)) or x2 is not None or k != 1:
            raise L.EdgeStyleHipError("LayerNorm-folded weights need a plain linear launch (all groups folded)")
        d.ln_colsum, d.ln_eps = pw.ln_colsum.data_ptr(), pw.ln_eps
    if tails:
        if any(t.shape[:3] != (N, Hout, Wout) or not t.is_contiguous() for t in tails):
            raise L.EdgeStyleHipError("conv_gemm: tail sources must be contiguous [N,Hout,Wout,C]")
        d.t1, d.Ct1 = tails[0].data_ptr(), tails[0].shape[3]
        if len(tails) == 2:
            d.t2, d.Ct2 = tails[1].data_ptr(), tails[1].shape[3]
    if pws is not None:
        hw = Hout * Wout
        gran = 256 if bn in (320, 256) else BM
        if len(pws) > 4 or len(group_n) != len(pws) or sum(group_n) != N or any((n * hw) % gran for n in group_n):
            raise L.EdgeStyleHipError(f"grouped conv_gemm: groups must cover N in whole {gran}-pixel tiles (<= 4 groups)")
        d.ngroups = len(pws)
        acc = 0
        for g, (q, n) in enumerate(zip(pws, group_n)):
            if (q.rows_padded, q.kpad, q.cout, q.cin, q.ksize, q.geglu, q.ctail, q.korder) != \
                    (pw.rows_padded, pw.kpad, pw.cout, pw.cin, pw.ksize, pw.geglu, pw.ctail, pw.korder):
                raise L.EdgeStyleHipError("grouped conv_gemm: weight geometry differs between groups")
            acc += n * hw // BM
            d.mt_end[g] = acc
            d.w_g[g] = q.w.data_ptr()
            d.bias_g[g] = q.bias.data_ptr() if q.bias is not None else None
            d.ln_colsum_g[g] = q.ln_colsum.data_ptr() if q.ln_colsum is not None else None
    if PROFILE is not None:
        d.prof = PROFILE.next((2.0 * M * pw.cout * (k * k * (C1 + C2) + pw.ctail), k,
                               (M, pw.cout, k * k * (C1 + C2) + pw.ctail, stride, splitk, bn),
                               dict(N=N, H=H, W=W, C1=C1, C2=C2, cout=pw.cout, k=k, stride=stride, pad=pad,
                                    upsample=bool(upsample), geglu=pw.geglu, splitk=splitk, Hout=Hout, Wout=Wout,
                                    residual=residual is not None, temb=temb is not None, bn=bn,
                                    stages=int(d.stages), group_n=list(group_n) if pws is not None else None,
                                    ctail=pw.ctail,
                                    algorithmic_bytes=_algorithmic_bytes(x, x2, pw, pws, out, residual)
                                    + sum(t.numel() * t.element_size() for t in tails))))
        dd = L.GemmDesc()
        C.memmove(C.byref(dd), C.byref(d), C.sizeof(L.GemmDesc))
        dd.prof = None
        PROFILE.descs.append(dd)
    L.check(L.load().es_conv_gemm(C.byref(d), _stream()), "es_conv_gemm")
    return out


def _algorithmic_bytes(x, x2, pw, pws, out, residual) -> int:
    n = x.numel() * x.element_size() + (x2.numel() * x2.element_size() if x2 is not None else 0)
    n += sum(q.w.numel() * q.w.element_size() for q in (pws if pws is not None else [pw]))
    n += out.numel() * out.element_size()
    if residual is not None:
        n += residual.numel() * residual.element_size()
    return int(n)


def linear(x: torch.Tensor, pw: PackedWeight, **kw) -> torch.Tensor:
    shp = x.shape
    M = x.numel() // shp[-1]
    out = kw.pop("out", None)
    res = kw.pop("residual", None)
    rep = kw.get("x_rep", 1)
    p0 = pw[0] if isinstance(pw, (list, tuple)) else pw
    cstore = p0.cout // 2 if p0.geglu else p0.cout
    y = conv_gemm(x.reshape(M, 1, 1, shp[-1]), pw,
                  residual=None if res is None else carry_lo(res.reshape(M * rep, 1, 1, cstore), res),
                  out=None if out is None else out.reshape(M * rep, 1, 1, cstore), **kw)
    if rep > 1:
        return carry_lo(y.reshape(shp[0] * rep, *shp[1:-1], cstore), y)
    return carry_lo(y.reshape(*shp[:-1], cstore), y)


def attention(q: torch.Tensor, k: torch.Tensor, v: torch.Tensor, heads: int, scale: Optional[float] = None,
              out: Optional[torch.Tensor] = None) -> torch.Tensor:
    def bad(msg):
        return L.EdgeStyleHipError("attention: " + msg)
    if q.dtype not in (torch.float16, torch.bfloat16):
        raise bad(f"q must be fp16 or bf16, not {q.dtype}")
    if q.dim() != 3 or k.dim() != 3 or v.dim() != 3:
        raise bad("q, k, v must be [N, S, heads * d]")
    N, Sq, Cq = q.shape
    Skv = k.shape[1]
    if heads < 1 or Cq % heads != 0:
        raise bad(f"width {Cq} is not a multiple of heads {heads}")
    dh = Cq // heads
    if out is None:
        out = torch.empty((N, Sq, Cq), dtype=q.dtype, device=q.device)
    for name, t in (("k", k), ("v", v), ("out", out)):
        if t.dtype != q.dtype or t.device != q.device:
            raise bad(f"{name} is {t.dtype} on {t.device}, q is {q.dtype} on {q.device}")
    if k.shape != v.shape:
        raise bad(f"k {tuple(k.shape)} and v {tuple(v.shape)} differ")
    if k.shape[0] != N or k.shape[2] != Cq:
        raise bad(f"k / v {tuple(k.shape)} do not match q {tuple(q.shape)} in N or width")
    if out.dim() != 3 or out.shape != q.shape:
        raise bad(f"out {tuple(out.shape)} is not q's shape {tuple(q.shape)}")
    for name, t in (("q", q), ("k", k), ("v", v), ("out", out)):
        if t.stride(2) != 1:
            raise bad("innermost stride must be 1")
        if t.stride(1) < Cq:
# ... 533 lines not shown
```

### include/edgestyle_hip.h

```cpp
#ifndef EDGESTYLE_HIP_H
#define EDGESTYLE_HIP_H
#include <stddef.h>
#include <stdint.h>

#ifdef __cplusplus
extern "C" {
#endif

enum { ES_F16 = 0, ES_BF16 = 1, ES_F32 = 2  };
enum { ES_ACT_NONE = 0, ES_ACT_SILU = 1, ES_ACT_GEGLU = 2 };

#define ES_ABI_VERSION 7
int es_abi_version(void);
size_t es_sizeof_desc(int which);
const char* es_last_error(void);

typedef struct {
  const void* x;
  const void* x2;
  const void* w;
  const float* bias;
  const void* temb;
  const void* residual;
  const float* out_scale_dev;
  void* out;
  float* workspace;
  unsigned long long* prof;
  int32_t N, Hsrc, Wsrc, C1, C2;
  int32_t Hout, Wout, Cout;
  int32_t rows_padded, Kpad;
  int32_t ksize, stride, pad;
  int32_t upsample;
  int32_t temb_stride;
  int32_t act;
  int32_t splitk;
  int32_t bn;
  int32_t dtype;
  int32_t ngroups;
  int32_t mt_end[4];
  const void* w_g[4];
  const float* bias_g[4];
  int32_t stages;
  int32_t xcd_m_fastest;
  int32_t waves;
  float out_scale;
  const float* ln_colsum;
  const float* ln_colsum_g[4];
  float ln_eps;
  const void* t1;
  const void* t2;
  int32_t Ct1, Ct2;
  int32_t x_nmod;
  int32_t korder;
  const void* residual_lo;
  void* out_lo;
  float* gn_part;
  int32_t gn_groups;
} es_gemm_desc;
int es_conv_gemm(const es_gemm_desc* d, void* stream);
unsigned long long es_set_operand_limit(unsigned long long bytes);
size_t es_conv_gemm_workspace_bytes(const es_gemm_desc* d);

typedef struct {
  const void* x; void* out;
  const void* w; const float* bias;
  const void* w_g[4]; const float* bias_g[4];
  unsigned long long* prof;
  int32_t mt_end[4];
  int32_t ngroups;
  int32_t M, K, Cout, rows_padded;
  int32_t ldo;
  int32_t geglu, ln;
  float ln_eps;
  int32_t nslices, chunks_per_slice;
  int32_t dtype;
  const void* residual;
  const float* gn_part;
  const float* gn_gamma; const float* gn_beta;
  const float* gn_gamma_g[4]; const float* gn_beta_g[4];
  int32_t gn_groups, gn_nchunk, gn_hw;
  float gn_eps;
} es_xs_desc;
int es_linear_xs(const es_xs_desc* d, void* stream);
int es_linear_xs_set_pp(int on);
enum { ES_XS_FORM_KC_MASK = 0xFF, ES_XS_FORM_GEGLU = 0x100, ES_XS_FORM_LN = 0x200, ES_XS_FORM_RES = 0x400, ES_XS_FORM_PP = 0x800,
       ES_XS_FORM_GN = 0x1000 };
int es_linear_xs_last_form(void);

typedef struct {
  const void* q; const void* k; const void* v; void* o;
  int32_t N, heads, Sq, Skv, d;
  int32_t ldq, ldk, ldv, ldo;
  int64_t bsq, bsk, bsv, bso;
  float scale;
  int32_t dtype;
} es_attn_desc;
int es_attention(const es_attn_desc* d, void* stream);
int es_attention_set_kvres(int on);
int es_attention_last_kernel(void);

typedef struct {
  const void* x; const void* x2; void* out;
  const float* gamma; const float* beta; float* partials;
  int32_t N, HW, C1, C2, groups;
  float eps;
  int32_t silu, dtype;
  int32_t ngroups;
  int32_t n_end[4];
  const float* gamma_g[4];
  const float* beta_g[4];
// ... 137 lines not shown
int es_ctx_set_alphas_cumprod_f64(es_ctx* c, const double* alphas_cumprod, int n);
int es_unipc_coef_table(const double* alphas_cumprod, int n_alphas, const float* timesteps, int n, float* out);
int es_ctx_plan_size(const es_ctx* c, int which);
es_plan* es_ctx_plan(es_ctx* c, int which);
int es_ctx_load(const char* path, int device, es_ctx** out);
int es_ctx_save(const es_ctx* c, const char* path);
typedef struct {
  const char* key;
  const void* data;
  int64_t shape[4];
  int32_t ndim;
  int32_t dtype;
} es_tensor;
typedef struct { const es_tensor* tensors; int32_t count; } es_state_dict;
enum { ES_NET_CONTROLNET = 0,
       ES_NET_CONTROL_LORA_VAE = 1,
       ES_NET_CONTROL_LORA = 2 };
typedef struct {
  es_state_dict unet, vae, fusion;
  es_state_dict controlnet[6];
  int32_t controlnet_kind[6];
  int32_t n_controlnets;
  int32_t net_of_cond[6];
} es_weights;
typedef struct {
  int32_t in_channels, out_channels;
  int32_t n_blocks, block_out_channels[4], down_has_attn[4];
  int32_t layers_per_block, num_heads, cross_attention_dim, norm_num_groups;
  float norm_eps;
  int32_t n_cond_embed, cond_embed_channels[4], conditioning_channels;
  int32_t text_tokens;
  int32_t vae_n_blocks, vae_block_out_channels[4], vae_layers_per_block, vae_latent_channels, vae_norm_num_groups;
  float vae_norm_eps, vae_scaling_factor;
} es_model_config;
int es_load_weights(const es_weights* w, const es_model_config* cfg, const es_ctx_geometry* g, int device, es_ctx** out);
int es_plan_gemm_choice(long long M, int rows_padded, int kpad, int geglu, const int* bns, int n_bns, int allow_split,
                        int* bn, int* splitk, int* stages);
int es_linear_xs_eligible(long long M, int ksize, int kpad, int cin, int ctail, int cout, int geglu);
typedef struct {
  long long M, hw;
  long long w_numel, src_numel;
  int32_t ksize, stride, upsample, C1, C2;
  int32_t rows_padded, kpad, cin, ctail, cout, geglu, has_ln;
  int32_t act;
  int32_t has_temb, has_residual;
  int32_t residual_dense;
  int32_t unit_scale;
  int32_t n_tails, x_rep, wide;
  int32_t dtype, gn_groups;
  int32_t ngroups;
  int32_t n_counts, group_n[4];
  int32_t groups_agree;
  int32_t force_splitk, stages;
} es_launch_query;
typedef struct {
  int32_t xs_enabled, xs_residual, xs_min_m;
  int32_t big_tile, big_tile_256, small_tile, eight_waves;
  int32_t deep_ring;
  int32_t gn_handover;
  int32_t wide_stream;
  int32_t gn_fold;
  int32_t force_bn, force_waves, force_stages;
  int32_t xcd_order;
} es_launch_knobs;
enum { ES_ROUTE_CONV_GEMM = 0, ES_ROUTE_LINEAR_XS = 1 };
typedef struct {
  int32_t route;
  int32_t bn, splitk, stages, waves, xcd_m_fastest;
  int32_t gn_partials;
  int32_t wide;
} es_launch_choice;
int es_launch_choose(const es_launch_query* q, const es_launch_knobs* k, es_launch_choice* out);
int es_launch_route(const es_launch_query* q, const es_launch_knobs* k);
int es_launch_gn_fold(const es_launch_query* q, int groups, const es_launch_knobs* k);
int es_launch_gn_handover(long long hw, int c, int groups, const es_launch_knobs* k);
int es_launch_wide_stream(int dtype, const es_launch_knobs* k);
int es_conv_gemm8p_form_ok(int act, int cout, int has_temb, long long out_hw, int has_residual);
int es_ctx_graph_hazard(void);
int es_plan_set_dry(int on);

int es_ctx_launch_plan(es_ctx* c, int which, const float* guidance_scale, void* stream);
int es_ddim_coef_table(const float* alphas_cumprod, int n_alphas, const float* timesteps, int n, float* out);
int es_denoise_step(es_ctx* c, const void* sample, float t, const void* ehs, const void* const* cond_embeds,
                    const float* scales, void* out_noise, void* stream);
int es_denoise_loop(es_ctx* c, float* latents_inout, const void* ehs, float guidance_scale, const float* timesteps,
                    int n_steps, void* stream);
int es_vae_decode(es_ctx* c, const float* latents, float* out_img, void* stream);
int es_prepare_conds(es_ctx* c, const float* const* images, const float* const* noise, void* stream);

typedef struct {
  const uint8_t* data;
  int32_t height, width;
  int32_t channels;
  int64_t row_stride;
} es_image_u8;
int es_image_fit(int height, int width, int R, int32_t out[4]);
int es_image_resize_coeffs(int in, int out, int32_t* xmin, int32_t* ntaps, int32_t* k, int cap);
size_t es_image_resize_workspace_bytes(const es_image_u8* imgs, int count, int R);
int es_image_resize_u8(const es_image_u8* imgs, int count, uint8_t* out, int R, void* workspace, size_t workspace_bytes, void* stream);
int es_image_u8_to_f32(const uint8_t* in, float* out_nchw, int count, int H, int W, int normalize, void* stream);
int es_image_f32_to_u8(const float* in_nchw, uint8_t* out_hwc, int B, int H, int W, void* stream);
int es_prepare_conds_u8(es_ctx* c, const es_image_u8* images, const int32_t* normalize, const float* const* noise,
                        void* workspace, size_t workspace_bytes, void* stream);
int es_vae_decode_u8(es_ctx* c, const float* latents, uint8_t* out_hwc, void* stream);

typedef struct { uint64_t seed, offset; } es_philox;
typedef struct {
  uint64_t seed;
  uint64_t offset;
  int64_t numel;
  int32_t blocks;
  float scale;
  int32_t round_dtype;
  int64_t N, C, HW, Cstride;
} es_randn_desc;
int es_philox4x32_10(const uint32_t ctr[4], const uint32_t key[2], uint32_t out[4]);
int es_philox_block_cap(int device);
int es_philox_blocks(int64_t numel, int block_cap);
int64_t es_philox_advance(int64_t numel, int blocks);
int es_randn(float* out, const es_randn_desc* d, void* stream);
int es_randn_host(float* out, const es_randn_desc* d);
int es_ctx_draw_latents(es_ctx* c, es_philox* gens, int n_gens, float sigma, int round_dtype, float* latents_out, void* stream);
int es_ctx_draw_cond_noise(es_ctx* c, es_philox* gen, int round_dtype, void* stream);

int es_attention_causal(const es_attn_desc* d, void* stream);
int es_text_embed(const int32_t* ids, const float* tok, const float* pos, void* out, int rows, int S, int hidden, int vocab, int dtype,
                  void* stream);
typedef struct {
  int32_t vocab_size, hidden, heads, layers, intermediate, max_positions;
// ... 14 lines not shown
```

Measured before the change: 2.235 images/s.

## Fold nearest-upsample plus 3x3 conv into four sub-pixel 2x2 convolutions

Adds a sub-pixel decomposition for upsampler convs: each output parity class (a,b) is computed by a 2x2 conv over the low-resolution input, using weights pre-summed from the 3x3 kernel. The four classes run as one grouped GEMM, and the epilogue scatters rows into the interleaved high-resolution output. This lowers the reduction depth from 9*C to 4*C per output pixel and reads the source at its original resolution instead of the upsampled one. In exchange it stores four folded weight sets, adds index arithmetic in the epilogue, excludes the big 320 tile for this path, and changes rounding slightly because the folded weights are summed before conversion to f16.

```diff
diff --git a/edgestyle_amd/csrc/builder.hip b/edgestyle_amd/csrc/builder.hip
--- a/edgestyle_amd/csrc/builder.hip
+++ b/edgestyle_amd/csrc/builder.hip
@@ -20,6 +20,7 @@
 
 extern "C" void es_set_error(const char* msg);
 extern "C" int es_plan_set_dry(int on);
+extern unsigned long long es_operand_limit_v;
 
 namespace {
 
@@ -251,6 +252,7 @@
   bool geglu = false;
   float ln_eps = 1e-5f;
   const uint16_t* host_w = nullptr;
+  const PW* sub = nullptr;
   long long w_numel() const { return (long long)rows_padded * kpad; }
 };
 using PWs = std::vector<const PW*>;
@@ -373,7 +375,7 @@
   memset(o, 0, sizeof(*o));
   if (launch_takes_xs(q, k)) { o->route = ES_ROUTE_LINEAR_XS; return true; }
   const bool aligned = q.C1 % BK == 0 && q.C2 % BK == 0;
-  const bool big_ok = k.big_tile && aligned && !q.geglu && !q.has_ln && groups_tile_256(q);
+  const bool big_ok = k.big_tile && aligned && !q.geglu && !q.has_ln && groups_tile_256(q) && !q.subpixel;
   const bool small_ok = k.small_tile && aligned && !q.geglu && k.force_waves != 8;
   const bool ln256_ok = k.big_tile_256 && (q.geglu || q.has_ln) && q.ksize == 1 && q.stride == 1 && !q.upsample && !q.C2 && !q.n_tails && !q.has_temb &&
                         q.x_rep == 1 && q.C1 % BK == 0 && q.rows_padded % 256 == 0 && q.cout % 8 == 0 && !(q.geglu && q.has_residual) && !q.wide &&
@@ -404,6 +406,15 @@
   const int cstore = geglu ? q.cout / 2 : q.cout;
   o->gn_partials = q.gn_groups > 0 && gn_handover(q.hw, cstore, q.gn_groups, k) && !geglu && !q.has_ln && q.cout / q.gn_groups <= (bn == 320 ? 160 : bn);
   o->wide = q.wide && q.has_residual && wide_stream(q.dtype, k) && cstore % 8 == 0 && !geglu;
+  return true;
+}
+bool launch_subpixel(const es_launch_query& q, const es_launch_knobs& k) {
+  if (!k.subpixel || !q.upsample || q.ksize != 3 || q.stride != 1 || q.C2 || q.C1 % BK || q.cin != q.C1 || q.ctail || q.n_tails || q.geglu || q.has_ln) return false;
+  if (q.has_temb || q.has_residual || q.act != ES_ACT_NONE || !q.unit_scale || q.x_rep != 1 || q.ngroups > 1 || q.gn_groups || q.kpad != 9 * q.C1) return false;
+  if (q.M % 4 || (q.M / 4) % BM || q.hw % 4) return false;
+  if (k.force_bn == 320 || k.force_bn == 256 || k.force_waves == 8) return false;
+  const unsigned long long lim = es_operand_limit_v;
+  if ((unsigned long long)q.M * q.cout * 2 >= lim || (unsigned long long)(q.M / 4) * q.C1 * 2 >= lim || q.M * (q.rows_padded / 8) >= (1ll << 31)) return false;
   return true;
 }
 bool launch_gn_fold(const es_launch_query& q, int groups, const es_launch_knobs& k) {
@@ -423,6 +434,7 @@
   k.xs_enabled = k.big_tile = k.small_tile = k.eight_waves = k.deep_ring = 1; k.xs_min_m = XS_MIN_M; k.xcd_order = -1;
   k.xs_residual = env("ES_XS_RESIDUAL", "1") == "1"; k.big_tile_256 = env("ES_BIG_TILE_256", "1")[0] != '0'; k.gn_fold = env("ES_GN_FOLD", "1") == "1";
   k.gn_handover = ho == "all" ? 2 : ho == "1"; k.wide_stream = ws == "auto" ? -1 : ws == "1";
+  k.subpixel = env("ES_SUBPIXEL", "1")[0] != '0';
   return b;
 }
 
@@ -513,6 +525,46 @@
     }
     return &p;
   }
+  const PW* pack_subpixel(const std::vector<float>& w, int cout, int cin, const std::vector<float>* bias) {
+    if ((long long)w.size() != (long long)cout * cin * 9 || cin % BK) fail("builder: the sub-pixel fold needs 3x3 weights over 64-aligned channels");
+    const int bn = choose_bn(cout), rows = round_up(cout, bn), kpad = 4 * cin;
+    pws.emplace_back();
+    PW& p = pws.back();
+    p.cout = cout; p.cin = cin; p.ksize = 2; p.bn = bn; p.rows_padded = rows; p.kpad = kpad;
+    const size_t gsz = (size_t)rows * kpad;
+    p.w = persistent(4 * gsz * 2);
+    uint16_t* dst = (uint16_t*)staged(p.w, 4 * gsz * 2);
+    p.host_w = dst;
+    parallel_for(cout, [&](long long r0, long long r1) {
+      for (long long row = r0; row < r1; ++row)
+        for (int g = 0; g < 4; ++g) {
+          const int ab[2] = {g >> 1, g & 1};
+          uint16_t* d = dst + g * gsz + (size_t)row * kpad;
+          for (int t = 0; t < 4; ++t) {
+            const int rs[2] = {t >> 1, t & 1};
+            int lo[2], hi[2];
+            for (int e = 0; e < 2; ++e) {
+              if (ab[e] == 0) { lo[e] = rs[e] ? 1 : 0; hi[e] = rs[e] ? 2 : 0; }
+              else            { lo[e] = rs[e] ? 2 : 0; hi[e] = rs[e] ? 2 : 1; }
+            }
+            for (int ci = 0; ci < cin; ++ci) {
+              const float* s = w.data() + ((size_t)row * cin + ci) * 9;
+              double acc = 0.0;
+              for (int ky = lo[0]; ky <= hi[0]; ++ky)
+                for (int kx = lo[1]; kx <= hi[1]; ++kx) acc += (double)s[ky * 3 + kx];
+              d[t * cin + ci] = enc((float)acc);
+            }
+          }
+        }
+    });
+    if (bias) {
+      if ((int)bias->size() != cout) fail("builder: bias size does not match the weight");
+      p.bias = persistent((size_t)rows * 4);
+      float* bd = (float*)staged(p.bias, (size_t)rows * 4);
+      for (int r = 0; r < cout; ++r) bd[r] = (*bias)[r];
+    }
+    return &p;
+  }
   const PW* pack_ln(const std::vector<float>& w, int rows, int C, const std::vector<float>* bias, const std::vector<float>& gamma, const std::vector<float>& beta,
                     float eps, bool geglu) {
     std::vector<float> wg((size_t)rows * C), fb((size_t)rows);
@@ -563,6 +615,20 @@
     if (bt) b = W.vec(p + ".bias", cout);
     const PW* pw = pack(w, cout, cin, k, bt ? &b : nullptr, geglu, cin_pad, cout_pad);
     if (!key.empty()) pack_cache[key] = pw;
+    return pw;
+  }
+  const PW* conv_up(const Weights& W, const std::string& p) {
+    PW* pw = const_cast<PW*>(conv(W, p));
+    if (!pw->sub && pw->ksize == 3 && pw->cin % BK == 0 && !pw->korder) {
+      const es_tensor* wt = W.get(p + ".weight");
+      const int cout = (int)wt->shape[0], cin = (int)wt->shape[1];
+      if (cin == pw->cin) {
+        std::vector<float> w = W.matrix(p), b;
+        const bool has_b = W.find(p + ".bias") != nullptr;
+        if (has_b) b = W.vec(p + ".bias", cout);
+        pw->sub = pack_subpixel(w, cout, cin, has_b ? &b : nullptr);
+      }
+    }
     return pw;
   }
   void stack(const Weights& W, const std::vector<std::string>& ps, bool bias, std::vector<float>& w, std::vector<float>& b, int& rows, int& cols) {
@@ -665,6 +731,35 @@
     return q;
   }
 
+  T conv_gemm_subpixel(const T& x, const PW* ps, const T& out) {
+    const int N = x.n, H = x.h, Wd = x.w, C1 = x.c;
+    const long long hw = (long long)H * Wd, M = 4 * N * hw;
+    es_launch_query q;
+    memset(&q, 0, sizeof(q));
+    q.M = M; q.hw = hw; q.w_numel = ps->w_numel(); q.src_numel = x.numel() * 4; q.ksize = 2; q.stride = 1; q.C1 = C1;
+    q.rows_padded = ps->rows_padded; q.kpad = ps->kpad; q.cin = ps->cin; q.cout = ps->cout; q.residual_dense = 1; q.unit_scale = 1; q.x_rep = 4; q.dtype = dt;
+    q.ngroups = 4; q.n_counts = 4; q.groups_agree = 1; q.subpixel = 1;
+    for (int g = 0; g < 4; ++g) q.group_n[g] = N;
+    es_launch_choice ch;
+    if (!launch_choose(q, env.knobs, &ch)) fail("plan_gemm: rows_padded fits no N tile");
+    es_gemm_desc d;
+    memset(&d, 0, sizeof(d));
+    const size_t gbytes = (size_t)ps->w_numel() * 2;
+    d.x = x.ptr(); d.w = (const void*)ps->w; d.bias = (const float*)ps->bias; d.out = out.ptr();
+    d.N = 4 * N; d.Hsrc = H; d.Wsrc = Wd; d.C1 = C1; d.Hout = H; d.Wout = Wd; d.Cout = ps->cout;
+    d.rows_padded = ps->rows_padded; d.Kpad = ps->kpad; d.ksize = 2; d.stride = 1; d.pad = 1;
+    d.act = ES_ACT_NONE; d.splitk = ch.splitk; d.bn = ch.bn; d.dtype = dt; d.out_scale = 1.f; d.stages = ch.stages;
+    d.waves = ch.waves; d.xcd_m_fastest = ch.xcd_m_fastest; d.x_nmod = N; d.subpixel = 1;
+    if (ch.splitk > 1) d.workspace = (float*)workspace((unsigned long long)ch.splitk * M * ps->rows_padded * 4);
+    d.ngroups = 4;
+    for (int g = 0; g < 4; ++g) {
+      d.mt_end[g] = (int)((g + 1) * (N * hw / BM));
+      d.w_g[g] = (const void*)(ps->w + g * gbytes); d.bias_g[g] = (const float*)ps->bias;
+    }
+    ok(es_conv_gemm(&d, nullptr), "es_conv_gemm");
+    return out;
+  }
+
   T conv_gemm(const T& x, const PWs& pl, const CA& a = CA()) {
     const PW* pw = pl[0];
     const bool grouped = pl.size() > 1;
@@ -687,6 +782,7 @@
     const long long M = (long long)N * Hout * Wout, hw = (long long)Hout * Wout;
     const es_launch_query q = launch_query(pl, M, hw, a, C1, C2, x.numel() * a.x_rep + (a.x2 ? a.x2.numel() : 0),
                                            a.residual && a.residual.contig() && a.residual.numel() == M * cstore);
+    if (a.upsample && pw->sub && !grouped && !a.out_h && !a.out_w && pad == 1 && launch_subpixel(q, env.knobs)) return conv_gemm_subpixel(x, pw->sub, out);
     es_launch_choice ch;
     if (!launch_choose(q, env.knobs, &ch)) fail("plan_gemm: rows_padded fits no N tile");
     if (ch.route == ES_ROUTE_LINEAR_XS) {
@@ -1008,7 +1104,7 @@
         if (c.has_attn[c.nb - 1 - i]) { tr.emplace_back(B, W, "up_blocks." + std::to_string(i) + ".attentions." + std::to_string(j), c.heads, c.groups); ti = (int)tr.size() - 1; }
         up.back().emplace_back(rs, ti);
       }
-      upsample.push_back(i != c.nb - 1 ? B.conv(W, "up_blocks." + std::to_string(i) + ".upsamplers.0.conv") : nullptr);
+      upsample.push_back(i != c.nb - 1 ? B.conv_up(W, "up_blocks." + std::to_string(i) + ".upsamplers.0.conv") : nullptr);
     }
     W.shaped("conv_out.weight", {c.out_ch, c.ch[0], 3, 3});
     norm_out = B.norm(W, "conv_norm_out", c.ch[0]);
@@ -1099,7 +1195,7 @@
     for (int i = 0; i < n; ++i) {
       std::vector<Resnet> rs;
       for (int j = 0; j < c.lpb + 1; ++j) rs.emplace_back(B, W, "decoder.up_blocks." + std::to_string(i) + ".resnets." + std::to_string(j), c.groups, c.eps, -1);
-      d_up.emplace_back(rs, i != n - 1 ? B.conv(W, "decoder.up_blocks." + std::to_string(i) + ".upsamplers.0.conv") : nullptr);
+      d_up.emplace_back(rs, i != n - 1 ? B.conv_up(W, "decoder.up_blocks." + std::to_string(i) + ".upsamplers.0.conv") : nullptr);
     }
     d_norm = B.norm(W, "decoder.conv_norm_out", c.ch[0]);
     d_out = B.conv(W, "decoder.conv_out");
@@ -1546,6 +1642,7 @@
 extern "C" int es_launch_gn_fold(const es_launch_query* q, int groups, const es_launch_knobs* k) { return q && k && launch_gn_fold(*q, groups, *k); }
 extern "C" int es_launch_gn_handover(long long hw, int c, int groups, const es_launch_knobs* k) { return k && gn_handover(hw, c, groups, *k); }
 extern "C" int es_launch_wide_stream(int dtype, const es_launch_knobs* k) { return k && wide_stream(dtype, *k); }
+extern "C" int es_launch_subpixel(const es_launch_query* q, const es_launch_knobs* k) { return q && k && launch_subpixel(*q, *k); }
 
 extern "C" int es_load_weights(const es_weights* wts, const es_model_config* mc, const es_ctx_geometry* g, int device, es_ctx** out) {
   if (!wts || !mc || !g || !out) { es_set_error("es_load_weights: null argument"); return -1; }
diff --git a/edgestyle_amd/csrc/gemm_conv.hip b/edgestyle_amd/csrc/gemm_conv.hip
--- a/edgestyle_amd/csrc/gemm_conv.hip
+++ b/edgestyle_amd/csrc/gemm_conv.hip
@@ -32,12 +32,13 @@
   for (int r = 0; r < n; ++r) o[r] = from_f32<T>(v[r]);
 }
 
-template <int XI>
+template <int XI, bool K2 = false >
 ES_DEVICE void row_offsets_fn(unsigned (&voff)[XI], const int (&iy0)[XI], const int (&ix0)[XI], const int (&nb)[XI],
                               const int tp, const int cs, const int chan, const int ksize, const int KK, const int pad,
                               const int Hin, const int Win, const int upsample, const int Wsrc) {
   int ky = 0, kx = 0;
   if (ksize == 3) { ky = (tp * 11) >> 5; kx = tp - ky * 3; }
+  if constexpr (K2) { if (ksize == 2) { ky = tp >> 1; kx = tp & 1; } }
   if (tp >= KK) { ky = pad; kx = pad; }
 #pragma unroll
   for (int i = 0; i < XI; ++i) {
@@ -50,7 +51,8 @@
 
 template <typename T, int BM, int BN, bool ALIGNED, int STAGES, int FM = 4 ,
           bool LN = false ,
-          bool KO = false >
+          bool KO = false ,
+          bool SP = false >
 __global__ __launch_bounds__(BM * 8 / FM, (STAGES == 2 && BM == 128) ? (FM == 2 ? 4 : 2) : 1) void conv_gemm_kernel(
     const es_gemm_desc p, const int M, const int nk, const void* const tail1, const void* const tail2, const int tailC1,
     const int tailC2) {
@@ -124,6 +126,14 @@
   const int HWout = p.Hout * p.Wout;
 
   constexpr unsigned OOB = 0xFFFFFF00u;
+  int grp = 0;
+  if (p.ngroups > 1) {
+    const int t128 = (tile_m * BM) / 128;
+    grp = (t128 >= p.mt_end[0]) + (t128 >= p.mt_end[1]) + (t128 >= p.mt_end[2]);
+  }
+  constexpr bool sp = SP;
+  static_assert(!SP || (ALIGNED && !LN && !KO), "the sub-pixel form: aligned, tap-major, no LayerNorm fold");
+  const int sp_a = sp ? grp >> 1 : 0, sp_b = sp ? grp & 1 : 0;
   int iy0[XI], ix0[XI], nb[XI];
   const bool small_m = M < (1 << 24);
   const float inv_hw = __builtin_amdgcn_rcpf((float)HWout), inv_w = __builtin_amdgcn_rcpf((float)p.Wout);
@@ -145,9 +155,10 @@
         const int rem = m - n * HWout;
         oy = rem / p.Wout; ox = rem - oy * p.Wout;
       }
-      iy0[i] = oy * p.stride - p.pad;
-      ix0[i] = ox * p.stride - p.pad;
-      if (p.x_nmod) n -= (n / p.x_nmod) * p.x_nmod;
+      iy0[i] = oy * p.stride - p.pad + sp_a;
+      ix0[i] = ox * p.stride - p.pad + sp_b;
+      if (sp) n -= grp * p.x_nmod;
+      else if (p.x_nmod) n -= (n / p.x_nmod) * p.x_nmod;
       nb[i] = n * p.Hsrc * p.Wsrc;
     }
   }
@@ -169,11 +180,6 @@
       tmask[i] = mk;
       pix0[i] = nb[i] + (ay >> p.upsample) * p.Wsrc + (ax >> p.upsample);
     }
-  }
-  int grp = 0;
-  if (p.ngroups > 1) {
-    const int t128 = (tile_m * BM) / 128;
-    grp = (t128 >= p.mt_end[0]) + (t128 >= p.mt_end[1]) + (t128 >= p.mt_end[2]);
   }
   const void* wsel = p.ngroups > 1 ? p.w_g[grp] : p.w;
   const float* bsel = p.ngroups > 1 ? p.bias_g[grp] : p.bias;
@@ -218,7 +224,7 @@
   const int ks_tail = (KK * Ctot) / BKT;
   const int pk_ksize = p.ksize, pk_pad = p.pad, pk_up = p.upsample, pk_wsrc = p.Wsrc;
 #define row_offsets(tp, cs, chan) \
-  row_offsets_fn<XI>(voff, iy0, ix0, nb, (tp), (cs), (chan), pk_ksize, KK, pk_pad, Hin, Win, pk_up, pk_wsrc)
+  row_offsets_fn<XI, SP>(voff, iy0, ix0, nb, (tp), (cs), (chan), pk_ksize, KK, pk_pad, Hin, Win, pk_up, pk_wsrc)
   auto issue_tile = [&](int ks, int stage) __attribute__((always_inline)) {
     char* xs = smem + stage * (XT + WT);
     char* ws = xs + XT;
@@ -447,6 +453,19 @@
   if (p.out_scale_dev) scale *= *p.out_scale_dev;
   char* et = smem;
   T* outp = (T*)p.out;
+  auto out_row = [&](int m) __attribute__((always_inline)) {
+    if (!sp) return m;
+    const int Ws = p.Wout, Hs = p.Hout;
+    const int mm = m - grp * (M >> 2);
+    int n, i;
+    if (small_m) { n = fast_div(mm, HWout, __builtin_amdgcn_rcpf((float)HWout)); }
+    else n = mm / HWout;
+    const int rem = mm - n * HWout;
+    if (small_m) { i = fast_div(rem, Ws, __builtin_amdgcn_rcpf((float)Ws)); }
+    else i = rem / Ws;
+    const int j = rem - i * Ws;
+    return ((n * 2 * Hs + 2 * i + sp_a) * 2 * Ws + 2 * j + sp_b);
+  };
   const T* resp = (const T*)p.residual;
   constexpr int RPF = (BM * (BN / 8) + NT - 1) / NT;
   u32x4 rpre[RPF];
@@ -595,7 +614,7 @@
           const int m = tile_m * BM + row, c = c_tile + ch * 8;
           if (idx < BM * CH && m < M && c < Cstore) {
             auto v = as_vec8<T>(*(const u32x4*)(et + row * EROW + ch * 16));
-            const size_t o = (size_t)m * Cstore + c;
+            const size_t o = (size_t)out_row(m) * Cstore + c;
             if constexpr (MODE >= 2) {
               const auto rv = as_vec8<T>(rpre[k]);
               typename Traits<T>::vec8 lv, lo;
@@ -633,7 +652,7 @@
         if (m < M && c < Cstore) {
           float x = to_f32(*(const T*)(et + row * EROW + cc * 2));
           if (resp) x += to_f32(resp[(size_t)m * Cstore + c]);
-          outp[(size_t)m * Cstore + c] = from_f32<T>(x);
+          outp[(size_t)out_row(m) * Cstore + c] = from_f32<T>(x);
         }
       }
     }
@@ -714,7 +733,17 @@
     x = to_f32(from_f32<T>(x * scale));
     v[r] = x + rv[r];
   }
-  T* o = (T*)p.out + (size_t)m * p.Cout + c0;
+  int mo = m;
+  if (p.subpixel) {
+    const int Mg = M >> 2, hw = p.Hout * p.Wout;
+    const int g = (m >= Mg) + (m >= 2 * Mg) + (m >= 3 * Mg);
+    const int mm = m - g * Mg;
+    const int ns = div_any(mm, hw, 1.0f / (float)hw, small);
+    const int rem = mm - ns * hw;
+    const int i = div_any(rem, p.Wout, 1.0f / (float)p.Wout, small), j = rem - i * p.Wout;
+    mo = (ns * 2 * p.Hout + 2 * i + (g >> 1)) * 2 * p.Wout + 2 * j + (g & 1);
+  }
+  T* o = (T*)p.out + (size_t)mo * p.Cout + c0;
   if (full && p.out_lo) {
     typename Traits<T>::vec8 pk, lo;
     if (p.residual_lo) {
@@ -841,14 +870,17 @@
   dim3 grid(((M + bm - 1) / bm) * tn * d.splitk);
   int stages = d.stages;
   if (stages == 0) stages = 2;
+                    \
 #define ES_LAUNCH_F(BMV, BNV, AL, ST, FMV)                                                                  \
   do {                                                                                                      \
-    if (AL && d.korder) ES_LAUNCH_K(BMV, BNV, AL, ST, FMV, AL);                                             \
-    else ES_LAUNCH_K(BMV, BNV, AL, ST, FMV, false);                                                         \
+    constexpr bool SPOK = AL && (FMV == 4 || BMV == 64);                                                    \
+    if (SPOK && d.subpixel) ES_LAUNCH_K(BMV, BNV, AL, ST, FMV, false, SPOK);                                \
+    else if (AL && d.korder) ES_LAUNCH_K(BMV, BNV, AL, ST, FMV, AL, false);                                 \
+    else ES_LAUNCH_K(BMV, BNV, AL, ST, FMV, false, false);                                                  \
   } while (0)
-#define ES_LAUNCH_K(BMV, BNV, AL, ST, FMV, KOV)                                                             \
+#define ES_LAUNCH_K(BMV, BNV, AL, ST, FMV, KOV, SPV)                                                        \
   do {                                                                                                      \
-    auto kfn = conv_gemm_kernel<T, BMV, BNV, AL, ST, FMV, false, KOV>;                                      \
+    auto kfn = conv_gemm_kernel<T, BMV, BNV, AL, ST, FMV, false, KOV, SPV>;                                 \
     const size_t lds = (size_t)ST * (BMV + BNV) * BK * 2;                                                   \
     static bool attr_set = false;                                                                           \
     if (!attr_set) {                                                                                        \
@@ -1022,7 +1054,20 @@
     const char* why = nullptr;
     if (launch_in_chunks(*d, nullptr, &why, true)) { es_set_error(why); return -1; }
   }
-  if (d->ksize != 1 && d->ksize != 3) { es_set_error("es_conv_gemm: ksize must be 1 or 3"); return -1; }
+  if (d->ksize != 1 && d->ksize != 3 && !(d->ksize == 2 && d->subpixel)) { es_set_error("es_conv_gemm: ksize must be 1 or 3 (2: the sub-pixel form only)"); return -1; }
+  if (d->subpixel) {
+    if (d->temb || d->residual || d->residual_lo || d->out_lo || d->t1 || d->t2 || d->act != ES_ACT_NONE || d->ln_colsum || d->gn_part) {
+      es_set_error("es_conv_gemm: the sub-pixel form takes a bias only: no residual, time embedding, activation, tail sources, LayerNorm fold or gn_part"); return -1; }
+    bool geo = d->subpixel == 1 && d->ksize == 2 && d->stride == 1 && d->pad == 1 && !d->upsample && !d->x2 && !d->C2 && d->C1 % BK == 0 && !d->korder &&
+               d->Hout == d->Hsrc && d->Wout == d->Wsrc && d->ngroups == 4 && d->x_nmod > 0 && d->N == 4 * d->x_nmod && d->Kpad == 4 * d->C1;
+    const long long mg = (long long)d->x_nmod * d->Hsrc * d->Wsrc;
+    for (int g = 0; geo && g < 4; ++g) geo = (long long)d->mt_end[g] * 128 == (g + 1) * mg;
+    if (!geo) {
+      es_set_error("es_conv_gemm: the sub-pixel form needs ksize 2, stride 1, pad 1, no upsample flag, one 64-aligned source, tap-major K = 4 * C1, "
+                   "Hout x Wout = Hsrc x Wsrc, N = 4 * x_nmod and four equal groups of whole 128-pixel tiles"); return -1; }
+    if (d->bn == 320 || d->bn == 256 || d->waves == 8) { es_set_error("es_conv_gemm: the sub-pixel form runs on the 64- and 128-pixel tiles (bn 64 | 128 | 160, 4 waves)"); return -1; }
+    if (chunked) { es_set_error("es_conv_gemm: the sub-pixel form needs every operand below 2 GiB (32-bit buffer offsets)"); return -1; }
+  }
   if (d->t1 && (d->stride != 1 || d->upsample || d->C1 % BK || d->C2 % BK || d->Ct1 % BK || d->Ct2 % BK || d->Ct1 < BK ||
                 (d->Ct2 && !d->t2) || d->ln_colsum || d->Hout != d->Hsrc || d->Wout != d->Wsrc ||
                 false)) {
diff --git a/edgestyle_amd/engine.py b/edgestyle_amd/engine.py
--- a/edgestyle_amd/engine.py
+++ b/edgestyle_amd/engine.py
@@ -42,6 +42,13 @@
         pw = ops.pack_weight(self.t(p + ".weight"), None if b is None else b.to(self.device), self.dtype,
                              self.device, geglu=geglu, cin_pad=cin_pad, cout_pad=cout_pad)
         _PACK_CACHE[key] = (weakref.ref(w), None if b is None else weakref.ref(b), pw)
+        return pw
+
+    def conv_up(self, p: str) -> ops.PackedWeight:
+        pw = self.conv(p)
+        if pw.sub is None and pw.ksize == 3 and pw.cin % ops.BK == 0 and not pw.korder and pw.cin == self.sd[p + ".weight"].shape[1]:
+            b = self.sd.get(p + ".bias")
+            pw.sub = ops.pack_weight_subpixel(self.t(p + ".weight"), None if b is None else b.to(self.device), self.dtype, self.device)
         return pw
 
     def conv_tail(self, p: str, pt: str) -> ops.PackedWeight:
@@ -237,7 +244,7 @@
                 a = Transformer(pk, f"up_blocks.{i}.attentions.{j}", heads, g) if cfg.up_has_attn[i] else None
                 blk.append((r, a))
             self.up.append(blk)
-            self.upsample.append(pk.conv(f"up_blocks.{i}.upsamplers.0.conv") if i != n - 1 else None)
+            self.upsample.append(pk.conv_up(f"up_blocks.{i}.upsamplers.0.conv") if i != n - 1 else None)
         self.norm_out = pk.norm("conv_norm_out")
         self.conv_out = pk.conv("conv_out")
         del self.pk
@@ -376,7 +383,7 @@
             for i in range(n):
                 rs = [Resnet(pk, f"decoder.up_blocks.{i}.resnets.{j}", g, eps, None)
                       for j in range(cfg.layers_per_block + 1)]
-                us = pk.conv(f"decoder.up_blocks.{i}.upsamplers.0.conv") if i != n - 1 else None
+                us = pk.conv_up(f"decoder.up_blocks.{i}.upsamplers.0.conv") if i != n - 1 else None
                 self.d_up.append((rs, us))
             self.d_norm = pk.norm("decoder.conv_norm_out")
             self.d_out = pk.conv("decoder.conv_out")
diff --git a/edgestyle_amd/lib.py b/edgestyle_amd/lib.py
--- a/edgestyle_amd/lib.py
+++ b/edgestyle_amd/lib.py
@@ -26,7 +26,7 @@
         ("ln_colsum", C.c_void_p), ("ln_colsum_g", C.c_void_p * 4), ("ln_eps", C.c_float),
         ("t1", C.c_void_p), ("t2", C.c_void_p), ("Ct1", C.c_int32), ("Ct2", C.c_int32),
         ("x_nmod", C.c_int32), ("korder", C.c_int32), ("residual_lo", C.c_void_p), ("out_lo", C.c_void_p),
-        ("gn_part", C.c_void_p), ("gn_groups", C.c_int32),
+        ("gn_part", C.c_void_p), ("gn_groups", C.c_int32), ("subpixel", C.c_int32),
     ]
 
 
@@ -156,12 +156,12 @@
     _fields_ = [(n, C.c_longlong) for n in ("M", "hw", "w_numel", "src_numel")] + \
         [(n, _I32) for n in ("ksize", "stride", "upsample", "C1", "C2", "rows_padded", "kpad", "cin", "ctail", "cout", "geglu", "has_ln", "act",
                              "has_temb", "has_residual", "residual_dense", "unit_scale", "n_tails", "x_rep", "wide", "dtype", "gn_groups",
-                             "ngroups", "n_counts")] + [("group_n", _I32 * 4)] + [(n, _I32) for n in ("groups_agree", "force_splitk", "stages")]
+                             "ngroups", "n_counts")] + [("group_n", _I32 * 4)] + [(n, _I32) for n in ("groups_agree", "force_splitk", "stages", "subpixel")]
 
 
 class LaunchKnobs(C.Structure):
     _fields_ = [(n, _I32) for n in ("xs_enabled", "xs_residual", "xs_min_m", "big_tile", "big_tile_256", "small_tile", "eight_waves", "deep_ring",
-                                    "gn_handover", "wide_stream", "gn_fold", "force_bn", "force_waves", "force_stages", "xcd_order")]
+                                    "gn_handover", "wide_stream", "gn_fold", "force_bn", "force_waves", "force_stages", "xcd_order", "subpixel")]
 
 
 class LaunchChoice(C.Structure):
@@ -251,6 +251,7 @@
     "es_launch_choose": (C.c_int, [C.POINTER(LaunchQuery), C.POINTER(LaunchKnobs), C.POINTER(LaunchChoice)]),
     "es_launch_route": (C.c_int, [C.POINTER(LaunchQuery), C.POINTER(LaunchKnobs)]),
     "es_launch_gn_fold": (C.c_int, [C.POINTER(LaunchQuery), _I, C.POINTER(LaunchKnobs)]),
+    "es_launch_subpixel": (C.c_int, [C.POINTER(LaunchQuery), C.POINTER(LaunchKnobs)]),
     "es_launch_gn_handover": (C.c_int, [C.c_longlong, _I, _I, C.POINTER(LaunchKnobs)]),
     "es_launch_wide_stream": (C.c_int, [_I, C.POINTER(LaunchKnobs)]),
     "es_conv_gemm8p_form_ok": (C.c_int, [_I, _I, _I, C.c_longlong, _I]),
diff --git a/edgestyle_amd/ops.py b/edgestyle_amd/ops.py
--- a/edgestyle_amd/ops.py
+++ b/edgestyle_amd/ops.py
@@ -59,7 +59,7 @@
     def replay_gemms(self, only_ksize: int = 0):
         lib = L.load()
         for d in self.descs:
-            if only_ksize and (isinstance(d, L.XsDesc) or int(d.ksize) != only_ksize):
+            if only_ksize and (isinstance(d, L.XsDesc) or (3 if d.subpixel else int(d.ksize)) != only_ksize):
                 continue
             fn = lib.es_linear_xs if isinstance(d, L.XsDesc) else lib.es_conv_gemm
             L.check(fn(C.byref(d), _stream()), "GEMM replay")
@@ -99,14 +99,15 @@
     ln_eps: float = 1e-5
     ctail: int = 0
     korder: int = 0
+    sub: Optional["PackedWeight"] = None
 
     @property
     def rows_padded(self):
-        return self.w.shape[0]
+        return self.w.shape[-2]
 
     @property
     def kpad(self):
-        return self.w.shape[1]
+        return self.w.shape[-1]
 
 
 def choose_bn(cout: int) -> int:
@@ -181,6 +182,40 @@
         bp = torch.zeros(rows, dtype=torch.float32, device=device)
         bp[:cout] = bias.to(device=device, dtype=torch.float32)
     return PackedWeight(wp, bp, cout, cin, k, bn, False, ctail=tw.shape[1], korder=korder)
+
+
+SUBPIXEL = _os.environ.get("ES_SUBPIXEL", "1") != "0"
+SUBPIXEL_TAPS = (((0,), (1, 2)), ((0, 1), (2,)))
+
+
+def subpixel_fold(weight: torch.Tensor) -> torch.Tensor:
+    w = weight.double()
+    v = torch.zeros((2, 2) + tuple(w.shape[:2]) + (2, 2), dtype=torch.float64, device=w.device)
+    for a in range(2):
+        for b in range(2):
+            for r in range(2):
+                for s_ in range(2):
+                    for ky in SUBPIXEL_TAPS[a][r]:
+                        for kx in SUBPIXEL_TAPS[b][s_]:
+                            v[a, b, :, :, r, s_] += w[:, :, ky, kx]
+    return v
+
+
+def pack_weight_subpixel(weight: torch.Tensor, bias: Optional[torch.Tensor], dtype, device) -> PackedWeight:
+    weight = weight.to(device=device, dtype=torch.float32)
+    cout, cin, k, _ = weight.shape
+    if k != 3 or cin % BK:
+        raise L.EdgeStyleHipError("pack_weight_subpixel: 3x3 weights over a multiple of 64 input channels")
+    v = subpixel_fold(weight).permute(0, 1, 2, 4, 5, 3).reshape(4, cout, 4 * cin)
+    bn = choose_bn(cout)
+    rows = (cout + bn - 1) // bn * bn
+    wp = torch.zeros(4, rows, 4 * cin, dtype=dtype, device=device)
+    wp[:, :cout] = v.float().to(dtype)
+    bp = None
+    if bias is not None:
+        bp = torch.zeros(rows, dtype=torch.float32, device=device)
+        bp[:cout] = bias.to(device=device, dtype=torch.float32)
+    return PackedWeight(wp, bp, cout, cin, 2, bn)
 
 
 def pack_weight_ln(weight: torch.Tensor, bias: Optional[torch.Tensor], gamma: torch.Tensor, beta: torch.Tensor,
@@ -340,7 +375,7 @@
     kn = dict(xs_enabled=XS_ENABLED, xs_residual=XS_RESIDUAL, xs_min_m=XS_MIN_M, big_tile=BIG_TILE, big_tile_256=BIG_TILE_256,
               small_tile=SMALL_TILE, eight_waves=EIGHT_WAVES, deep_ring=DEEP_RING and LANE == 0,
               gn_handover=(2 if GN_HANDOVER_ALL else 1) if GN_HANDOVER else 0, wide_stream={"auto": -1, "1": 1}.get(WIDE_STREAM, 0),
-              gn_fold=GN_FOLD, force_bn=FORCE_BN, force_waves=FORCE_WAVES, force_stages=FORCE_STAGES, xcd_order=XCD_ORDER)
+              gn_fold=GN_FOLD, force_bn=FORCE_BN, force_waves=FORCE_WAVES, force_stages=FORCE_STAGES, xcd_order=XCD_ORDER, subpixel=SUBPIXEL)
     return L.LaunchKnobs(**{k: int(v) for k, v in dict(kn, **over).items()})
 
 
@@ -538,6 +573,9 @@
                      upsample=upsample, C1=C1, C2=C2, act=act, has_temb=temb is not None, has_residual=residual is not None,
                      unit_scale=out_scale == 1.0 and out_scale_dev is None, n_tails=len(tails), x_rep=x_rep, wide=wide, dtype=_dt(x),
                      gn_groups=gn_groups, force_splitk=splitk or 0, stages=stages)
+    if upsample and pw.sub is not None and pws is None and out_hw is None and pad == 1 and \
+            L.load().es_launch_subpixel(C.byref(q), C.byref(launch_knobs())):
+        return _conv_gemm_subpixel(x, pw, out, splitk or 0, stages)
     ch = L.LaunchChoice()
     if L.load().es_launch_choose(C.byref(q), C.byref(launch_knobs()), C.byref(ch)) != 0:
         raise L.EdgeStyleHipError(f"plan_gemm: rows_padded {pw.rows_padded} fits no N tile")
@@ -630,6 +668,46 @@
     return out
 
 
+def _conv_gemm_subpixel(x: torch.Tensor, pw: PackedWeight, out: torch.Tensor, splitk: int, stages: int) -> torch.Tensor:
+    ps = pw.sub
+    N, H, W, C1 = x.shape
+    hw, M = H * W, 4 * N * H * W
+    q = launch_query(M, hw, ps, src_numel=x.numel() * 4, C1=C1, x_rep=4, dtype=_dt(x), force_splitk=splitk, stages=stages, subpixel=1)
+    q.ngroups, q.n_counts, q.groups_agree = 4, 4, 1
+    q.group_n[:] = [N] * 4
+    ch = L.LaunchChoice()
+    if L.load().es_launch_choose(C.byref(q), C.byref(launch_knobs()), C.byref(ch)) != 0:
+        raise L.EdgeStyleHipError(f"plan_gemm: rows_padded {ps.rows_padded} fits no N tile")
+    d = L.GemmDesc()
+    d.x, d.w, d.out = x.data_ptr(), ps.w.data_ptr(), out.data_ptr()
+    d.bias = ps.bias.data_ptr() if ps.bias is not None else None
+    d.N, d.Hsrc, d.Wsrc, d.C1 = 4 * N, H, W, C1
+    d.Hout, d.Wout, d.Cout = H, W, ps.cout
+    d.rows_padded, d.Kpad = ps.rows_padded, ps.kpad
+    d.ksize, d.stride, d.pad = 2, 1, 1
+    d.act, d.splitk, d.bn, d.dtype, d.out_scale = L.ACT_NONE, ch.splitk, ch.bn, _dt(x), 1.0
+    d.stages, d.waves, d.xcd_m_fastest = ch.stages, ch.waves, ch.xcd_m_fastest
+    d.x_nmod, d.subpixel = N, 1
+    if ch.splitk > 1:
+        d.workspace = _get_workspace(ch.splitk * M * ps.rows_padded * 4, x.device).data_ptr()
+    d.ngroups = 4
+    for g in range(4):
+        d.mt_end[g] = (g + 1) * (N * hw // BM)
+        d.w_g[g] = ps.w[g].data_ptr()
+        d.bias_g[g] = d.bias
+    if PROFILE is not None:
+        d.prof = PROFILE.next((2.0 * M * pw.cout * 9 * C1, 3, (M, pw.cout, 9 * C1, 1, ch.splitk, ch.bn),
+                               dict(N=N, H=H, W=W, C1=C1, C2=0, cout=pw.cout, k=3, stride=1, pad=1, upsample=True, geglu=False,
+                                    splitk=ch.splitk, Hout=2 * H, Wout=2 * W, residual=False, temb=False, bn=ch.bn, stages=int(d.stages),
+                                    group_n=None, ctail=0, subpixel=True, algorithmic_bytes=_algorithmic_bytes(x, None, pw, None, out, None))))
+        dd = L.GemmDesc()
+        C.memmove(C.byref(dd), C.byref(d), C.sizeof(L.GemmDesc))
+        dd.prof = None
+        PROFILE.descs.append(dd)
+    L.check(L.load().es_conv_gemm(C.byref(d), _stream()), "es_conv_gemm")
+    return out
+
+
 def _algorithmic_bytes(x, x2, pw, pws, out, residual) -> int:
     n = x.numel() * x.element_size() + (x2.numel() * x2.element_size() if x2 is not None else 0)
     n += sum(q.w.numel() * q.w.element_size() for q in (pws if pws is not None else [pw]))
diff --git a/include/edgestyle_hip.h b/include/edgestyle_hip.h
--- a/include/edgestyle_hip.h
+++ b/include/edgestyle_hip.h
@@ -56,6 +56,7 @@
   void* out_lo;
   float* gn_part;
   int32_t gn_groups;
+  int32_t subpixel;
 } es_gemm_desc;
 int es_conv_gemm(const es_gemm_desc* d, void* stream);
 unsigned long long es_set_operand_limit(unsigned long long bytes);
@@ -299,6 +300,7 @@
   int32_t n_counts, group_n[4];
   int32_t groups_agree;
   int32_t force_splitk, stages;
+  int32_t subpixel;
 } es_launch_query;
 typedef struct {
   int32_t xs_enabled, xs_residual, xs_min_m;
@@ -309,6 +311,7 @@
   int32_t gn_fold;
   int32_t force_bn, force_waves, force_stages;
   int32_t xcd_order;
+  int32_t subpixel;
 } es_launch_knobs;
 enum { ES_ROUTE_CONV_GEMM = 0, ES_ROUTE_LINEAR_XS = 1 };
 typedef struct {
@@ -322,6 +325,7 @@
 int es_launch_gn_fold(const es_launch_query* q, int groups, const es_launch_knobs* k);
 int es_launch_gn_handover(long long hw, int c, int groups, const es_launch_knobs* k);
 int es_launch_wide_stream(int dtype, const es_launch_knobs* k);
+int es_launch_subpixel(const es_launch_query* q, const es_launch_knobs* k);
 int es_conv_gemm8p_form_ok(int act, int cout, int has_temb, long long out_hw, int has_residual);
 int es_ctx_graph_hazard(void);
 int es_plan_set_dry(int on);
```

Result: no change. 2.252 images/s (median of 6 runs) (+0.7%).
